# JiapengWu/TeMP

Measured on AMD Instinct MI355X. Metric: edges/sec (fwd+bwd) RGCN+GRU seq_len=15, higher is better.
Workload: dtype f32

## Files before the change

include/temp_amd.h:

```cpp
#ifndef TEMP_AMD_H
#define TEMP_AMD_H

#include <stddef.h>
#include <stdint.h>

#ifdef __cplusplus
extern "C" {
#endif

#define TEMP_ABI_VERSION 2

enum {
  TEMP_OK = 0,
  TEMP_E_BADARG = 1,
  TEMP_E_UNSUPPORTED = 2,
  TEMP_E_WORKSPACE = 3,
  TEMP_E_LAUNCH = 4
};

enum { TEMP_ACT_NONE = 0, TEMP_ACT_RELU = 1 };
enum { TEMP_GRU_TORCH = 0,
       TEMP_GRU_TYPE1 = 1 };

int temp_abi_version(void);
// ... 31 lines not shown
  int32_t n_seg;
  int32_t n_edges;
  const int32_t* a;
  const int32_t* b;
  int32_t n_chunks;
  const int32_t* chunk_seg;
  const int32_t* chunk_beg;
  const int32_t* chunk_end;
  const int32_t* chunk_slot;
  int32_t n_partial;
  int32_t n_fix;
  const int32_t* fix_seg;
  const int32_t* fix_slot;
  const int32_t* fix_cnt;
} TempEdgeView;

typedef struct TempMembers {
  int32_t n_members;
  int32_t max_nodes;
  int32_t max_edges;
  int32_t max_chunks[3];
  const int32_t* node_off;
  const int32_t* edge_off;
  const int32_t* chunk_off;
  const int32_t* fix_off;
} TempMembers;

typedef struct TempGraph {
  int32_t n_nodes;
  int32_t n_edges;
  const float* nnorm;
  const int32_t* in_deg;
  const int32_t* out_deg;
  TempEdgeView by_dst;
  TempEdgeView by_src;
  TempEdgeView by_rel;
  TempMembers members;
} TempGraph;

size_t temp_rgcn_fwd_workspace(const TempGraph* g, int d_out);
int temp_rgcn_fwd(const TempGraph* g, const float* h, const int32_t* h_ids ,
                  int d_in, int d_out, int num_bases, int n_rel_rows,
                  const float* weight, const float* loop_w, const float* bias , int act,
                  float* out, void* workspace, size_t workspace_bytes, const TempDropout* drop, void* stream);

size_t temp_rgcn_bwd_workspace(const TempGraph* g, int d_in, int d_out, int num_bases, int n_rel_rows);
int temp_rgcn_bwd(const TempGraph* g, const float* h, const float* out, const float* d_out_grad,
                  int d_in, int d_out, int num_bases, int n_rel_rows,
                  const float* weight, const float* loop_w, int has_bias, int act,
                  float* d_h, float* d_weight, float* d_loop_w, float* d_bias ,
                  void* workspace, size_t workspace_bytes, const TempDropout* drop, void* stream);

int temp_rgcn_bwd_dh(const TempGraph* g, const float* out , const float* d_out_grad, int d_in, int d_out, int num_bases,
                     int n_rel_rows, const float* weight, const float* loop_w, int act, float* d_h, float* dz_out ,
                     float* dzm_out , void* workspace, size_t workspace_bytes, const TempDropout* drop, void* stream);
int temp_rgcn_bwd_weights(const TempGraph* g, const float* h, const float* dz, const float* dzm , int d_in, int d_out, int num_bases,
                          int n_rel_rows, int has_bias, float* d_weight, float* d_loop_w, float* d_bias , void* workspace,
                          size_t workspace_bytes, void* stream);

size_t temp_rgcn_table_fwd_workspace(const TempGraph* g, int n_table, int d_out);
int temp_rgcn_table_fwd(const TempGraph* g, const float* table, const int32_t* ids, int n_table, int d_in, int d_out, int num_bases,
                        int n_rel_rows, const float* weight, const float* loop_w, const float* bias, int act, float* out, void* workspace,
                        size_t workspace_bytes, const TempDropout* drop, void* stream);
size_t temp_rgcn_table_bwd_workspace(const TempGraph* g, int n_table, int d_in, int d_out, int num_bases);
int temp_rgcn_table_bwd(const TempGraph* g, const float* table, const int32_t* ids, const int32_t* inv_ptr, const int32_t* inv_order, int n_table,
                        const float* out, const float* d_out_grad, int d_in, int d_out, int num_bases, int n_rel_rows, const float* weight,
                        const float* loop_w, int has_bias, int act, float* d_table, float* d_weight, float* d_loop_w, float* d_bias,
                        void* workspace, size_t workspace_bytes, const TempDropout* drop, void* stream);

int temp_rgcn_isolated_fwd(int n, int d, const float* e, const float* loop_w, const float* bias ,
                           int act, float* out, const TempDropout* drop, void* stream);
size_t temp_rgcn_isolated_bwd_workspace(int n, int d);
int temp_rgcn_isolated_bwd(int n, int d, const float* e, const float* out, const float* d_out_grad,
                           const float* loop_w, int has_bias, int act,
                           float* d_e, float* d_loop_w, float* d_bias ,
                           void* workspace, size_t workspace_bytes, const TempDropout* drop, void* stream);

int temp_gru_fwd(int n, int d, int variant,
                 const float* x, const float* prev, const int32_t* prev_idx , const float* dt,
                 float lambda, const float* decay_wb ,
                 const float* w_ih, const float* w_hh, const float* b_ih, const float* b_hh,
                 float* h_out, float* saved, void* stream);

size_t temp_gru_bwd_workspace(int n, int d, int variant);
int temp_gru_bwd(int n, int d, int variant,
                 const float* x, const float* prev, const int32_t* prev_idx , const float* dt,
                 float lambda, const float* decay_wb ,
                 const float* w_ih, const float* w_hh,
                 const float* saved, const float* d_h_out,
                 float* d_x, float* d_prev, float* d_w_ih, float* d_w_hh, float* d_b_ih, float* d_b_hh,
                 float* d_decay_wb ,
                 void* workspace, size_t workspace_bytes, void* stream);

int temp_decay_rows(int n, int d, const float* x, const float* dt, float lambda, float* out, void* stream);

int temp_gru_input_gates(int n, int d, int variant, const float* x, const float* w_ih, const float* b_ih, float* gi, void* stream);
int temp_gru_input_gates_multi(int count, const int* ns, int d, int variant, const float* const* xs, const float* const* w_ihs,
                               const float* const* b_ihs, float* const* gis, void* stream);
int temp_gru_input_gates_gather_multi(int count, const int* ns, int d, int variant, const float* const* xs, const int32_t* const* x_idx,
                                      const float* const* w_ihs, const float* const* b_ihs, float* const* gis, void* stream);
int temp_gru_cell_fwd(int n, int d, int variant, const float* gi, const float* prev, const int32_t* prev_idx ,
                      const float* dt, float lambda, const float* w_hh, const float* b_hh,
                      float* h_out, float* saved, size_t saved_plane, void* stream);
int temp_gru_cell_bwd(int n, int d, int variant, const float* saved, size_t saved_plane,
                      const float* dh_up , const float* d_prev_next , const int32_t* next_idx ,
                      const float* dt, float lambda, const float* w_hh,
                      float* dgi, float* dgh, float* decv, float* d_prev, void* stream);
typedef struct TempGruCellFwd {
  int32_t n; const float* gi; const float* prev ;
  const int32_t* prev_idx ; const float* dt;
  const float* w_hh; const float* b_hh; float* h_out; float* saved ;
} TempGruCellFwd;
typedef struct TempGruCellBwd {
  int32_t n; const float* saved; const float* dh_up ; const float* d_prev_next ;
  const int32_t* next_idx ; const float* dt; const float* w_hh;
  float* dgi; float* dgh; float* decv; float* d_prev;
  int32_t no_prev;
} TempGruCellBwd;
int temp_gru_cell_fwd_multi(int count, const TempGruCellFwd* cells, int d, int variant, float lambda, size_t saved_plane, void* stream);
int temp_gru_cell_bwd_multi(int count, const TempGruCellBwd* cells, int d, int variant, float lambda, size_t saved_plane, void* stream);
size_t temp_gru_weight_grads_workspace(int n, int d, int variant);
int temp_gru_weight_grads(int n, int d, int variant, const float* x, const float* hdec, const float* dgi, const float* dgh,
                          const float* w_ih, float* d_x , float* d_w_ih, float* d_w_hh, float* d_b_ih, float* d_b_hh,
                          void* workspace, size_t workspace_bytes, void* stream);
size_t temp_gru_weight_grads_multi_workspace(int count, const int* ns, int d, int variant);
int temp_gru_weight_grads_multi(int count, const int* ns, int d, int variant, const float* const* xs, const float* const* hdecs,
                                const float* const* dgis, const float* const* dghs, const float* const* w_ihs, float* const* d_xs,
                                float* d_w, float* d_b, void* workspace, size_t workspace_bytes, void* stream);

size_t temp_gru_grads_g4_workspace(int count, const int* ns, int d);
int temp_gru_grads_g4(int count, const int* ns, int d, const float* const* xs, const float* const* hdecs, const float* const* g4s,
                      const float* const* w_ihs, float* const* d_xs, float* d_w, float* d_b, void* workspace, size_t workspace_bytes,
                      void* stream);
int temp_gru_grads_g4_keys(int count, const int* ns, int d, const float* const* xs, const float* const* hdecs, const float* const* g4s,
                           const float* const* w_ihs, float* const* d_xs, float* d_w, float* d_b, const uint32_t* const* g4_row_keys,
                           const uint32_t* const* g4_col_keys, const uint32_t* const* x_col_keys ,
                           void* workspace, size_t workspace_bytes, void* stream);

#define TEMP_CHAIN_HAS_PREV (1 << 30)
#define TEMP_CHAIN_TRACKS 32
#define TEMP_CHAIN_MAX_RNN 4
#define TEMP_CHAIN_MAX_UP 8
typedef struct TempGruChain {
  int32_t d, variant, n_panels, n_steps;
  int32_t max_steps;
  const int32_t* panel; const int32_t* rows; const int32_t* sinfo;
  const float* dt;
  float lambda;
  size_t saved_plane;
  int32_t n_rnn;
  const float* packed[TEMP_CHAIN_MAX_RNN];
  const float* b_hh[TEMP_CHAIN_MAX_RNN];
  const int32_t* gi_index;
} TempGruChain;
int temp_gru_chain_supported(int d);
size_t temp_gru_chain_pack_floats(int d);
int temp_gru_chain_pack(int d, const float* w_hh, float* packed, void* stream);
int temp_gru_chain_pack_multi(int count, int d, const float* const* w_hh, float* const* packed, void* stream);
int temp_gru_chain_fwd(const TempGruChain* c, const float* gi, float* h_out, float* saved, void* stream);
int temp_gru_chain_bwd(const TempGruChain* c, const float* saved, int n_up, const float* const* up ,
                       float* dgi, float* dgh, void* stream);
int temp_gru_chain_bwd_g4(const TempGruChain* c, const float* saved, int n_up, const float* const* up ,
                          float* g4, void* stream);
int temp_gru_chain_keys_supported(int d);
int temp_gru_chain_bwd_g4_keys(const TempGruChain* c, const float* saved, int n_up, const float* const* up, float* g4,
                               uint32_t* row_keys, uint32_t* col_keys, void* stream);

int temp_gather_rows(int n, int d, const float* table, const int32_t* idx, float* out, void* stream);
size_t temp_keys_cols_size(int d);
int temp_absmax_keys(int n, int d, const float* x, int ldx, uint32_t* row_keys, uint32_t* col_keys, void* stream);
int temp_gather_rows_keys(int n, int d, const float* table, const int32_t* idx, float* out, uint32_t* row_keys, uint32_t* col_keys, void* stream);
int temp_linear_keys(int M, int N, int K, const float* A, int lda, const uint32_t* a_keys, const float* B, int ldb, int trans_b, float* C, int ldc,
                     void* stream);
int temp_gru_input_gates_gather_multi_keys(int count, const int* ns, int d, int variant, const float* const* xs, const int32_t* const* x_idx,
                                           const uint32_t* const* x_keys, const float* const* w_ihs, const float* const* b_ihs, float* const* gis,
                                           void* stream);
int temp_scatter_add_rows(int n, int d, const float* src, const int32_t* idx, float* table, void* stream);
size_t temp_segment_sum_rows_workspace(int n_seg, int n_rows, int d);
int temp_segment_sum_rows(int n_seg, int n_rows, int d, const int32_t* seg_ptr, const int32_t* order, const float* src, float* out,
                          void* workspace, size_t workspace_bytes, void* stream);
int temp_segment_sum_rows_relu(int n_seg, int n_rows, int d, const int32_t* seg_ptr, const int32_t* order, const float* src, const float* relu_of,
                               float* out, void* workspace, size_t workspace_bytes, void* stream);

int temp_linear(int M, int N, int K, const float* A, int lda, const float* B, int ldb, int trans_b, float* C, int ldc, void* stream);
int temp_linear_t(int M, int N, int K, const float* A, int lda, const float* B, int ldb, int trans_b, float* Ct, int ldct, void* stream);
typedef struct TempLinearProblem { int M; const float* A; const float* B; float* C; } TempLinearProblem;
int temp_linear_multi(int count, const TempLinearProblem* probs, int N, int K, int lda, int ldb, int trans_b, int ldc, void* stream);
size_t temp_linear_tn_workspace(int M, int Ka, int Nb);
int temp_linear_tn(int M, int Ka, int Nb, const float* A, int lda, const float* B, int ldb, float* out, int ldo,
                   void* workspace, size_t workspace_bytes, void* stream);
size_t temp_linear_tn_multi_workspace(int count, int max_m, int Ka, int Nb);
int temp_linear_tn_multi(int count, const TempLinearProblem* probs, int Ka, int Nb, int lda, int ldb, int ldc, void* workspace,
                         size_t workspace_bytes, void* stream);

int temp_gather_ce_fwd(int P, int C, int N, const float* scores, const int32_t* cand, float* loss_rows, float* lse_rows, void* stream);
int temp_gather_ce_bwd(int P, int C, int N, const float* scores, const int32_t* cand, const float* lse_rows, const float* scale,
                       float inv_rows, const float* row_scale , float* d_scores, void* stream);

#define TEMP_SCORE_DISTMULT 0
#define TEMP_SCORE_COMPLEX 1
int temp_bilinear_query_fwd(int P, int d, int kind, const float* ent_rows, const int32_t* known_idx, const float* rel, const int32_t* rel_idx,
                            const int32_t* is_tail, float* q, void* stream);
int temp_bilinear_query_bwd(int P, int d, int kind, const float* ent_rows, const int32_t* known_idx, const float* rel, const int32_t* rel_idx,
                            const int32_t* is_tail, const float* d_q, float* d_known_rows, float* d_rel_rows, void* stream);

#define TEMP_ASSEMBLE_PIECE 4096
typedef struct TempCopyDesc { const int32_t* src; const int32_t* aux; int32_t dst_off; int32_t len; int32_t add; int32_t mode; } TempCopyDesc;
int temp_assemble_views(int n_pieces, const int32_t* piece_desc, const int32_t* piece_start, const TempCopyDesc* descs, const int32_t* table,
                        int32_t* out, void* stream);

typedef struct TempSubsampleJob {
  int32_t n_nodes, n_edges, keep;
  uint64_t seed;
  const int32_t* parent; int32_t* child; const int32_t* eid;
  int32_t off_a[3], off_b[3], off_chunk_beg[3], off_chunk_end[3], off_chunk_seg[3], n_chunks[3];
  int32_t off_in_deg, off_out_deg, off_nnorm;
  uint8_t* keep_mask; void* scratch;
} TempSubsampleJob;
int temp_subsample_views(int n_jobs, const TempSubsampleJob* jobs, void* stream);

int temp_corrupt_sample(int R, int K, int N, uint64_t seed, const int32_t* truth, const int32_t* lo, const int32_t* hi, const int32_t* ids,
                        int32_t* cand, void* stream);

int temp_filtered_rank(int P, int N, int ld, const float* scores, const int32_t* target, const int32_t* filt_ptr,
                       const int32_t* filt_ids, int32_t* ranks, void* stream);

typedef struct TempAttn {
  int32_t n, D, heads, T;
  const float* q;  int32_t ldq;
  const float* kh; const float* vh; int32_t ldh;
  const float* kc; const float* vc; int32_t ldc;
  const int32_t* idx;
  const float* decay;
} TempAttn;
int temp_sa_attn_fwd(const TempAttn* p, float* out, float* score, float* lse, void* stream);
int temp_sa_attn_bwd(const TempAttn* p, const float* out, const float* score, const float* lse, const float* d_out,
                     float* d_q, int ld_dq, float* d_kh, float* d_vh, int ld_dh, float* d_kc, float* d_vc, int ld_dc,
                     float* d_decay, int n_table, const int32_t* inv_ptr, const int32_t* inv_ref, float* ds_ws, void* stream);

int temp_copy_probe(const void* src, void* dst, size_t bytes, void* stream);

int temp_trace_begin(int capacity);
int temp_trace_end(int* kernel_ids , float* ms , int capacity, int* n_out );
const char* temp_trace_kernel_name(int kernel_id);

#ifdef __cplusplus
}
#endif
#endif
```

temp_amd/_lib.py:

```python
import ctypes
import threading
import os

_HERE = os.path.dirname(os.path.abspath(__file__))
LIB_PATH = os.path.join(_HERE, "libtemp_amd.so")

c_i32p = ctypes.POINTER(ctypes.c_int32)
c_f32p = ctypes.POINTER(ctypes.c_float)
c_vp = ctypes.c_void_p

ACT_NONE, ACT_RELU = 0, 1
GRU_TORCH, GRU_TYPE1 = 0, 1
CHUNK = 64
CHUNK_REL = 128


class TempEdgeView(ctypes.Structure):
    _fields_ = [("n_seg", ctypes.c_int32), ("n_edges", ctypes.c_int32), ("a", c_vp), ("b", c_vp),
                ("n_chunks", ctypes.c_int32), ("chunk_seg", c_vp), ("chunk_beg", c_vp), ("chunk_end", c_vp),
                ("chunk_slot", c_vp), ("n_partial", ctypes.c_int32), ("n_fix", ctypes.c_int32),
                ("fix_seg", c_vp), ("fix_slot", c_vp), ("fix_cnt", c_vp)]


class TempMembers(ctypes.Structure):
    _fields_ = [("n_members", ctypes.c_int32), ("max_nodes", ctypes.c_int32), ("max_edges", ctypes.c_int32),
                ("max_chunks", ctypes.c_int32 * 3), ("node_off", c_vp), ("edge_off", c_vp), ("chunk_off", c_vp), ("fix_off", c_vp)]


class TempGraph(ctypes.Structure):
    _fields_ = [("n_nodes", ctypes.c_int32), ("n_edges", ctypes.c_int32), ("nnorm", c_vp), ("in_deg", c_vp),
                ("out_deg", c_vp), ("by_dst", TempEdgeView), ("by_src", TempEdgeView), ("by_rel", TempEdgeView),
                ("members", TempMembers)]


ABI_VERSION = 2
OPT_MFMA_BF16X3, OPT_TN_SPLIT, OPT_RGCN_SCALAR, OPT_GEMM_STREAM, OPT_GRU_STREAM, OPT_RGCN_TILE, OPT_DEBUG, OPT_OVERLAP, OPT_GEMM_RESIDENT, OPT_MFMA_F16X2 = range(10)


class TempGruCellFwd(ctypes.Structure):
    _fields_ = [("n", ctypes.c_int32), ("gi", c_vp), ("prev", c_vp), ("prev_idx", c_vp), ("dt", c_vp), ("w_hh", c_vp),
                ("b_hh", c_vp), ("h_out", c_vp), ("saved", c_vp)]


class TempGruCellBwd(ctypes.Structure):
    _fields_ = [("n", ctypes.c_int32), ("saved", c_vp), ("dh_up", c_vp), ("d_prev_next", c_vp), ("next_idx", c_vp), ("dt", c_vp),
                ("w_hh", c_vp), ("dgi", c_vp), ("dgh", c_vp), ("decv", c_vp), ("d_prev", c_vp), ("no_prev", ctypes.c_int32)]


CHAIN_HAS_PREV = 1 << 30
CHAIN_TRACKS = 32
CHAIN_MAX_RNN = 4
CHAIN_MAX_UP = 8
CHAIN_MAX_STEPS = 64


class TempGruChain(ctypes.Structure):
    _fields_ = [("d", ctypes.c_int32), ("variant", ctypes.c_int32), ("n_panels", ctypes.c_int32), ("n_steps", ctypes.c_int32),
                ("max_steps", ctypes.c_int32), ("panel", c_vp), ("rows", c_vp), ("sinfo", c_vp), ("dt", c_vp), ("lambda_", ctypes.c_float),
                ("saved_plane", ctypes.c_size_t), ("n_rnn", ctypes.c_int32), ("packed", c_vp * CHAIN_MAX_RNN), ("b_hh", c_vp * CHAIN_MAX_RNN),
                ("gi_index", c_vp)]


class TempSubsampleJob(ctypes.Structure):
    _fields_ = [("n_nodes", ctypes.c_int32), ("n_edges", ctypes.c_int32), ("keep", ctypes.c_int32), ("seed", ctypes.c_uint64),
                ("parent", c_vp), ("child", c_vp), ("eid", c_vp),
                ("off_a", ctypes.c_int32 * 3), ("off_b", ctypes.c_int32 * 3), ("off_chunk_beg", ctypes.c_int32 * 3),
                ("off_chunk_end", ctypes.c_int32 * 3), ("off_chunk_seg", ctypes.c_int32 * 3), ("n_chunks", ctypes.c_int32 * 3),
                ("off_in_deg", ctypes.c_int32), ("off_out_deg", ctypes.c_int32), ("off_nnorm", ctypes.c_int32),
                ("keep_mask", c_vp), ("scratch", c_vp)]


class TempDropout(ctypes.Structure):
    _fields_ = [("p", ctypes.c_float), ("seed", ctypes.c_uint64)]


class TempAttn(ctypes.Structure):
    _fields_ = [("n", ctypes.c_int32), ("D", ctypes.c_int32), ("heads", ctypes.c_int32), ("T", ctypes.c_int32),
                ("q", c_vp), ("ldq", ctypes.c_int32), ("kh", c_vp), ("vh", c_vp), ("ldh", ctypes.c_int32),
                ("kc", c_vp), ("vc", c_vp), ("ldc", ctypes.c_int32), ("idx", c_vp), ("decay", c_vp)]


class TempLinearProblem(ctypes.Structure):
    _fields_ = [("M", ctypes.c_int32), ("A", c_vp), ("B", c_vp), ("C", c_vp)]


ASSEMBLE_PIECE = 4096
SCORE_KINDS = {"distmult": 0, "complex": 1}

_G = ctypes.POINTER(TempGraph)
_I, _F, _SZ = ctypes.c_int, ctypes.c_float, ctypes.c_size_t
SYMBOLS = {
    "temp_abi_version": (_I, []),
    "temp_error_string": (ctypes.c_char_p, [_I]),
    "temp_set_option": (_I, [_I, _I]),
    "temp_get_option": (_I, [_I]),
    "temp_scratch_refused": (ctypes.c_longlong, []),
    "temp_f16_launches": (ctypes.c_longlong, []),
    "temp_tile_launches": (ctypes.c_longlong, []),
    "temp_set_debug_buffer": (None, [c_vp, _SZ]),
    "temp_rgcn_fwd_workspace": (_SZ, [_G, _I]),
    "temp_rgcn_fwd": (_I, [_G, c_vp, c_vp, _I, _I, _I, _I, c_vp, c_vp, c_vp, _I, c_vp, c_vp, _SZ, c_vp, c_vp]),
    "temp_rgcn_bwd_workspace": (_SZ, [_G, _I, _I, _I, _I]),
    "temp_rgcn_bwd": (_I, [_G, c_vp, c_vp, c_vp, _I, _I, _I, _I, c_vp, c_vp, _I, _I, c_vp, c_vp, c_vp, c_vp, c_vp, _SZ, c_vp, c_vp]),
    "temp_rgcn_bwd_dh": (_I, [_G, c_vp, c_vp, _I, _I, _I, _I, c_vp, c_vp, _I, c_vp, c_vp, c_vp, c_vp, _SZ, c_vp, c_vp]),
    "temp_rgcn_bwd_weights": (_I, [_G, c_vp, c_vp, c_vp, _I, _I, _I, _I, _I, c_vp, c_vp, c_vp, c_vp, _SZ, c_vp]),
    "temp_rgcn_table_fwd_workspace": (_SZ, [_G, _I, _I]),
    "temp_rgcn_table_fwd": (_I, [_G, c_vp, c_vp, _I, _I, _I, _I, _I, c_vp, c_vp, c_vp, _I, c_vp, c_vp, _SZ, c_vp, c_vp]),
    "temp_rgcn_table_bwd_workspace": (_SZ, [_G, _I, _I, _I, _I]),
    "temp_rgcn_table_bwd": (_I, [_G, c_vp, c_vp, c_vp, c_vp, _I, c_vp, c_vp, _I, _I, _I, _I, c_vp, c_vp, _I, _I, c_vp, c_vp, c_vp, c_vp,
                                 c_vp, _SZ, c_vp, c_vp]),
    "temp_rgcn_isolated_fwd": (_I, [_I, _I, c_vp, c_vp, c_vp, _I, c_vp, c_vp, c_vp]),
    "temp_rgcn_isolated_bwd_workspace": (_SZ, [_I, _I]),
    "temp_rgcn_isolated_bwd": (_I, [_I, _I, c_vp, c_vp, c_vp, c_vp, _I, _I, c_vp, c_vp, c_vp, c_vp, _SZ, c_vp, c_vp]),
    "temp_gru_fwd": (_I, [_I, _I, _I, c_vp, c_vp, c_vp, c_vp, _F, c_vp, c_vp, c_vp, c_vp, c_vp, c_vp, c_vp, c_vp]),
    "temp_gru_bwd_workspace": (_SZ, [_I, _I, _I]),
    "temp_gru_bwd": (_I, [_I, _I, _I, c_vp, c_vp, c_vp, c_vp, _F, c_vp, c_vp, c_vp, c_vp, c_vp,
                          c_vp, c_vp, c_vp, c_vp, c_vp, c_vp, c_vp, c_vp, _SZ, c_vp]),
    "temp_decay_rows": (_I, [_I, _I, c_vp, c_vp, _F, c_vp, c_vp]),
    "temp_gru_input_gates": (_I, [_I, _I, _I, c_vp, c_vp, c_vp, c_vp, c_vp]),
    "temp_gru_input_gates_multi": (_I, [_I, c_vp, _I, _I, c_vp, c_vp, c_vp, c_vp, c_vp]),
    "temp_gru_input_gates_gather_multi": (_I, [_I, c_vp, _I, _I, c_vp, c_vp, c_vp, c_vp, c_vp, c_vp]),
    "temp_gru_cell_fwd": (_I, [_I, _I, _I, c_vp, c_vp, c_vp, c_vp, _F, c_vp, c_vp, c_vp, c_vp, _SZ, c_vp]),
    "temp_gru_cell_bwd": (_I, [_I, _I, _I, c_vp, _SZ, c_vp, c_vp, c_vp, c_vp, _F, c_vp, c_vp, c_vp, c_vp, c_vp, c_vp]),
    "temp_gru_cell_fwd_multi": (_I, [_I, ctypes.POINTER(TempGruCellFwd), _I, _I, _F, _SZ, c_vp]),
    "temp_gru_cell_bwd_multi": (_I, [_I, ctypes.POINTER(TempGruCellBwd), _I, _I, _F, _SZ, c_vp]),
    "temp_gru_weight_grads_workspace": (_SZ, [_I, _I, _I]),
    "temp_gru_weight_grads": (_I, [_I, _I, _I, c_vp, c_vp, c_vp, c_vp, c_vp, c_vp, c_vp, c_vp, c_vp, c_vp, c_vp, _SZ, c_vp]),
    "temp_gru_weight_grads_multi_workspace": (ctypes.c_size_t, [_I, c_vp, _I, _I]),
    "temp_gru_weight_grads_multi": (_I, [_I, c_vp, _I, _I, c_vp, c_vp, c_vp, c_vp, c_vp, c_vp, c_vp, c_vp, c_vp, ctypes.c_size_t, c_vp]),
    "temp_gru_chain_supported": (_I, [_I]),
    "temp_gru_chain_pack_floats": (_SZ, [_I]),
    "temp_gru_chain_pack": (_I, [_I, c_vp, c_vp, c_vp]),
    "temp_gru_chain_pack_multi": (_I, [_I, _I, ctypes.POINTER(c_vp), ctypes.POINTER(c_vp), c_vp]),
    "temp_gru_chain_fwd": (_I, [ctypes.POINTER(TempGruChain), c_vp, c_vp, c_vp, c_vp]),
    "temp_gru_chain_bwd": (_I, [ctypes.POINTER(TempGruChain), c_vp, _I, ctypes.POINTER(c_vp), c_vp, c_vp, c_vp]),
    "temp_gru_chain_bwd_g4": (_I, [ctypes.POINTER(TempGruChain), c_vp, _I, ctypes.POINTER(c_vp), c_vp, c_vp]),
    "temp_gru_chain_keys_supported": (_I, [_I]),
    "temp_gru_chain_bwd_g4_keys": (_I, [ctypes.POINTER(TempGruChain), c_vp, _I, ctypes.POINTER(c_vp), c_vp, c_vp, c_vp, c_vp]),
    "temp_gru_grads_g4_keys": (_I, [_I, c_vp, _I, c_vp, c_vp, c_vp, c_vp, c_vp, c_vp, c_vp, c_vp, c_vp, c_vp, c_vp, ctypes.c_size_t, c_vp]),
    "temp_gru_grads_g4_workspace": (ctypes.c_size_t, [_I, c_vp, _I]),
    "temp_gru_grads_g4": (_I, [_I, c_vp, _I, c_vp, c_vp, c_vp, c_vp, c_vp, c_vp, c_vp, c_vp, ctypes.c_size_t, c_vp]),
    "temp_gather_rows": (_I, [_I, _I, c_vp, c_vp, c_vp, c_vp]),
    "temp_keys_cols_size": (_SZ, [_I]),
    "temp_absmax_keys": (_I, [_I, _I, c_vp, _I, c_vp, c_vp, c_vp]),
    "temp_gather_rows_keys": (_I, [_I, _I, c_vp, c_vp, c_vp, c_vp, c_vp, c_vp]),
    "temp_linear_keys": (_I, [_I, _I, _I, c_vp, _I, c_vp, c_vp, _I, _I, c_vp, _I, c_vp]),
    "temp_gru_input_gates_gather_multi_keys": (_I, [_I, c_vp, _I, _I, c_vp, c_vp, c_vp, c_vp, c_vp, c_vp, c_vp]),
    "temp_scatter_add_rows": (_I, [_I, _I, c_vp, c_vp, c_vp, c_vp]),
    "temp_segment_sum_rows_workspace": (_SZ, [_I, _I, _I]),
    "temp_segment_sum_rows": (_I, [_I, _I, _I, c_vp, c_vp, c_vp, c_vp, c_vp, _SZ, c_vp]),
    "temp_segment_sum_rows_relu": (_I, [_I, _I, _I, c_vp, c_vp, c_vp, c_vp, c_vp, c_vp, _SZ, c_vp]),
    "temp_linear": (_I, [_I, _I, _I, c_vp, _I, c_vp, _I, _I, c_vp, _I, c_vp]),
    "temp_linear_t": (_I, [_I, _I, _I, c_vp, _I, c_vp, _I, _I, c_vp, _I, c_vp]),
    "temp_linear_multi": (_I, [_I, ctypes.POINTER(TempLinearProblem), _I, _I, _I, _I, _I, _I, c_vp]),
    "temp_linear_tn_workspace": (_SZ, [_I, _I, _I]),
    "temp_linear_tn_multi_workspace": (_SZ, [_I, _I, _I, _I]),
    "temp_linear_tn_multi": (_I, [_I, ctypes.POINTER(TempLinearProblem), _I, _I, _I, _I, _I, c_vp, _SZ, c_vp]),
    "temp_linear_tn": (_I, [_I, _I, _I, c_vp, _I, c_vp, _I, c_vp, _I, c_vp, _SZ, c_vp]),
    "temp_gather_ce_fwd": (_I, [_I, _I, _I, c_vp, c_vp, c_vp, c_vp, c_vp]),
    "temp_gather_ce_bwd": (_I, [_I, _I, _I, c_vp, c_vp, c_vp, c_vp, _F, c_vp, c_vp, c_vp]),
    "temp_bilinear_query_fwd": (_I, [_I, _I, _I, c_vp, c_vp, c_vp, c_vp, c_vp, c_vp, c_vp]),
    "temp_bilinear_query_bwd": (_I, [_I, _I, _I, c_vp, c_vp, c_vp, c_vp, c_vp, c_vp, c_vp, c_vp, c_vp]),
    "temp_assemble_views": (_I, [_I, c_vp, c_vp, c_vp, c_vp, c_vp, c_vp]),
    "temp_subsample_views": (_I, [_I, ctypes.POINTER(TempSubsampleJob), c_vp]),
    "temp_corrupt_sample": (_I, [_I, _I, _I, ctypes.c_uint64, c_vp, c_vp, c_vp, c_vp, c_vp, c_vp]),
    "temp_filtered_rank": (_I, [_I, _I, _I, c_vp, c_vp, c_vp, c_vp, c_vp, c_vp]),
    "temp_sa_attn_fwd": (_I, [ctypes.POINTER(TempAttn), c_vp, c_vp, c_vp, c_vp]),
    "temp_sa_attn_bwd": (_I, [ctypes.POINTER(TempAttn), c_vp, c_vp, c_vp, c_vp, c_vp, _I, c_vp, c_vp, _I, c_vp, c_vp, _I, c_vp, _I, c_vp, c_vp, c_vp, c_vp]),
    "temp_copy_probe": (_I, [c_vp, c_vp, _SZ, c_vp]),
    "temp_trace_begin": (_I, [_I]),
    "temp_trace_end": (_I, [c_i32p, c_f32p, _I, c_i32p]),
    "temp_trace_kernel_name": (ctypes.c_char_p, [_I]),
}

_lib = None


class TempAmdError(RuntimeError):
    pass


def load():
    global _lib
    if _lib is not None:
        return _lib
    if not os.path.exists(LIB_PATH):
        raise TempAmdError("libtemp_amd.so not found at %s -- run `python -m temp_amd.build` "
                           "(hipcc --offload-arch=gfx950); there is no CPU fallback" % LIB_PATH)
    lib = ctypes.CDLL(LIB_PATH) if os.environ.get("TEMP_PYDLL", "1") == "0" else ctypes.PyDLL(LIB_PATH)
    for name, (res, args) in SYMBOLS.items():
        fn = getattr(lib, name)
        fn.restype = res
        fn.argtypes = args
    if lib.temp_abi_version() != ABI_VERSION:
        raise TempAmdError("libtemp_amd.so ABI version %d != %d (stale .so or stale Python package)" % (lib.temp_abi_version(), ABI_VERSION))
    _lib = lib
    return lib


def check(rc, what):
    if rc != 0:
        msg = load().temp_error_string(rc).decode()
        raise TempAmdError("%s failed: %s (code %d)" % (what, msg, rc))


class _CreateLock:

    def __init__(self):
        self._l = threading.RLock()

    def __enter__(self):
        if not self._l.acquire(blocking=False):
            held = getattr(_coop, "held", False)
            if held:
                _py_token.release()
            self._l.acquire()
            if held:
                _py_token.acquire()
        return self

    def __exit__(self, *exc):
        self._l.release()
        return False


create_lock = _CreateLock()


def publish(device):
    import torch as _torch
    device = _torch.device(device)
    if device.type == "cuda":
        _torch.cuda.current_stream(device).synchronize()


_coop = threading.local()
_py_token = threading.Lock()


def coop_begin(gate):
    _coop.gate = gate
    _py_token.acquire()
    _coop.held = True


def coop_end():
    if getattr(_coop, "held", False):
        _coop.held = False
        _py_token.release()
    _coop.gate = None


def pause_point():
    g = getattr(_coop, "gate", None)
    if g is not None and not g.is_set():
        held = getattr(_coop, "held", False)
        if held:
            _py_token.release()
        g.wait()
        if held:
            _py_token.acquire()


def outside_token(fn):
    def call(*args):
        if getattr(_coop, "held", False):
            _py_token.release()
            try:
                return fn(*args)
            finally:
                _py_token.acquire()
        return fn(*args)
    return call


_STAGE_BYTES = 32 << 20
_stage = threading.local()


def to_device(host, device):
    import numpy as _np
    import torch as _torch
    t = _torch.from_numpy(_np.ascontiguousarray(host)) if isinstance(host, _np.ndarray) else host
    device = _torch.device(device)
    nbytes = t.numel() * t.element_size()
    if device.type != "cuda" or nbytes == 0 or t.is_cuda or nbytes > _STAGE_BYTES // 4 or not t.is_contiguous():
        return t.to(device)
# ... 31 lines not shown
```

temp_amd/backend.py:

```python
import ctypes

import torch

from . import _lib

_backend = None


def set_backend(b):
    global _backend
    _backend = b


def get_backend():
    global _backend
    if _backend is None:
        _backend = HipBackend()
    return _backend


def _ptr(t):
    return ctypes.c_void_p(t.data_ptr()) if t is not None else None


# ... 137 lines not shown
        e, out, g, loop_w = _f32(e, "e"), _f32(out, "out"), _f32(d_out_grad, "d_out"), _f32(loop_w, "loop_weight")
        n, d = e.shape
        d_e = torch.empty_like(e)
        d_loop = torch.empty_like(loop_w)
        d_bias = torch.empty(d, dtype=torch.float32, device=e.device) if has_bias else None
        ws = self._ws(self.lib.temp_rgcn_isolated_bwd_workspace(n, d), e.device)
        rc = self.lib.temp_rgcn_isolated_bwd(n, d, _ptr(e), _ptr(out), _ptr(g), _ptr(loop_w), int(has_bias), act, _ptr(d_e),
                                             _ptr(d_loop), _ptr(d_bias), _ptr(ws), ws.numel(), _drop(drop), _stream())
        _lib.check(rc, "temp_rgcn_isolated_bwd")
        return d_e, d_loop, d_bias

    def gru_fwd(self, x, prev, prev_idx, dt, lam, decay_wb, w_ih, w_hh, b_ih, b_hh, variant):
        x, prev, dt = _f32(x, "x"), _f32(prev, "prev"), _f32(dt, "dt")
        w_ih, w_hh, b_ih, b_hh = _f32(w_ih, "w_ih"), _f32(w_hh, "w_hh"), _f32(b_ih, "b_ih"), _f32(b_hh, "b_hh")
        decay_wb, prev_idx = _f32(decay_wb, "decay_wb"), _i32(prev_idx, "prev_idx")
        n, d = x.shape
        h_out = torch.empty_like(x)
        saved = torch.empty(5, n, d, dtype=torch.float32, device=x.device)
        rc = self.lib.temp_gru_fwd(n, d, variant, _ptr(x), _ptr(prev), _ptr(prev_idx), _ptr(dt), float(lam), _ptr(decay_wb),
                                   _ptr(w_ih), _ptr(w_hh), _ptr(b_ih), _ptr(b_hh), _ptr(h_out), _ptr(saved), _stream())
        _lib.check(rc, "temp_gru_fwd")
        return h_out, saved

    def gru_bwd(self, x, prev, prev_idx, dt, lam, decay_wb, w_ih, w_hh, saved, d_h, variant):
        x, prev, dt, d_h = _f32(x, "x"), _f32(prev, "prev"), _f32(dt, "dt"), _f32(d_h, "d_h")
        w_ih, w_hh, saved = _f32(w_ih, "w_ih"), _f32(w_hh, "w_hh"), _f32(saved, "saved")
        decay_wb, prev_idx = _f32(decay_wb, "decay_wb"), _i32(prev_idx, "prev_idx")
        n, d = x.shape
        dev = x.device
        d_x = torch.empty_like(x)
        d_prev = torch.empty_like(x)
        d_w_ih, d_w_hh = torch.empty_like(w_ih), torch.empty_like(w_hh)
        d_b_ih = torch.empty(w_ih.shape[0], dtype=torch.float32, device=dev)
        d_b_hh = torch.empty(w_hh.shape[0], dtype=torch.float32, device=dev)
        d_wb = torch.empty(2, dtype=torch.float32, device=dev) if decay_wb is not None else None
        ws = self._ws(self.lib.temp_gru_bwd_workspace(n, d, variant), dev)
        rc = self.lib.temp_gru_bwd(n, d, variant, _ptr(x), _ptr(prev), _ptr(prev_idx), _ptr(dt), float(lam), _ptr(decay_wb),
                                   _ptr(w_ih), _ptr(w_hh), _ptr(saved), _ptr(d_h), _ptr(d_x), _ptr(d_prev), _ptr(d_w_ih),
                                   _ptr(d_w_hh), _ptr(d_b_ih), _ptr(d_b_hh), _ptr(d_wb), _ptr(ws), ws.numel(), _stream())
        _lib.check(rc, "temp_gru_bwd")
        return d_x, d_prev, d_w_ih, d_w_hh, d_b_ih, d_b_hh, d_wb

    def gru_input_gates(self, x, w_ih, b_ih, variant, out):
        x, w_ih, b_ih = _f32(x, "x"), _f32(w_ih, "w_ih"), _f32(b_ih, "b_ih")
        assert out.is_contiguous() and out.shape == (x.shape[0], w_ih.shape[0])
        rc = self.lib.temp_gru_input_gates(x.shape[0], x.shape[1], variant, _ptr(x), _ptr(w_ih), _ptr(b_ih), _ptr(out), _stream())
        _lib.check(rc, "temp_gru_input_gates")

    def gru_input_gates_multi(self, xs, w_ihs, b_ihs, variant, outs, x_idx=None, x_keys=None):
        k = len(xs)
        xs = [_f32(x, "x") for x in xs]
        w_ihs, b_ihs = [_f32(w, "w_ih") for w in w_ihs], [_f32(b, "b_ih") for b in b_ihs]
        d = xs[0].shape[1]
        idx = [None] * k if x_idx is None else [None if t is None else _i32(t, "x_idx") for t in x_idx]
        rows = [x.shape[0] if t is None else t.shape[0] for x, t in zip(xs, idx)]
        for x, w, o, n in zip(xs, w_ihs, outs, rows):
            assert x.shape[1] == d and o.is_contiguous() and o.shape == (n, w.shape[0]) and w.shape == w_ihs[0].shape
        arr = lambda ts: (ctypes.c_void_p * k)(*[t.data_ptr() for t in ts])
        ns = (ctypes.c_int * k)(*rows)
        if x_idx is None and x_keys is None:
            rc = self.lib.temp_gru_input_gates_multi(k, ns, d, variant, arr(xs), arr(w_ihs), arr(b_ihs), arr(outs), _stream())
            _lib.check(rc, "temp_gru_input_gates_multi")
            return
        ia = (ctypes.c_void_p * k)(*[None if t is None else t.data_ptr() for t in idx])
        if x_keys is not None:
            for x, t in zip(xs, x_keys):
                assert t.dtype == torch.int32 and t.is_contiguous() and t.numel() == x.shape[0]
            ka = (ctypes.c_void_p * k)(*[t.data_ptr() for t in x_keys])
            rc = self.lib.temp_gru_input_gates_gather_multi_keys(k, ns, d, variant, arr(xs), ia if x_idx is not None else None, ka, arr(w_ihs),
                                                                 arr(b_ihs), arr(outs), _stream())
            _lib.check(rc, "temp_gru_input_gates_gather_multi_keys")
            return
        rc = self.lib.temp_gru_input_gates_gather_multi(k, ns, d, variant, arr(xs), ia, arr(w_ihs), arr(b_ihs), arr(outs), _stream())
        _lib.check(rc, "temp_gru_input_gates_gather_multi")

    def gru_cell_fwd(self, gi, prev, prev_idx, dt, lam, w_hh, b_hh, variant, h_out, saved_all, row0):
        n, d = h_out.shape
        plane = saved_all.shape[1] * d
        sp = ctypes.c_void_p(saved_all.data_ptr() + 4 * row0 * d)
        rc = self.lib.temp_gru_cell_fwd(n, d, variant, _ptr(gi), _ptr(_f32(prev, "prev")), _ptr(_i32(prev_idx, "prev_idx")),
                                        _ptr(_f32(dt, "dt")), float(lam), _ptr(_f32(w_hh, "w_hh")), _ptr(_f32(b_hh, "b_hh")),
                                        _ptr(h_out), sp, plane, _stream())
        _lib.check(rc, "temp_gru_cell_fwd")

    def gru_cell_bwd(self, saved_all, row0, n, dh_up, d_prev_next, next_idx, dt, lam, w_hh, variant, dgi, dgh, decv, d_prev):
        d = saved_all.shape[2]
        plane = saved_all.shape[1] * d
        sp = ctypes.c_void_p(saved_all.data_ptr() + 4 * row0 * d)
        rc = self.lib.temp_gru_cell_bwd(n, d, variant, sp, plane, _ptr(dh_up), _ptr(d_prev_next), _ptr(_i32(next_idx, "next_idx")),
                                        _ptr(_f32(dt, "dt")), float(lam), _ptr(_f32(w_hh, "w_hh")), _ptr(dgi), _ptr(dgh), _ptr(decv),
                                        _ptr(d_prev), _stream())
        _lib.check(rc, "temp_gru_cell_bwd")

    def gru_cell_fwd_multi(self, cells, lam, variant, saved_all):
        d = saved_all.shape[2]
        arr = (_lib.TempGruCellFwd * len(cells))()
        keep = []
        for a, c in zip(arr, cells):
            prev, pidx, dt = _f32(c["prev"], "prev"), _i32(c["prev_idx"], "prev_idx"), _f32(c["dt"], "dt")
            w_hh, b_hh = _f32(c["w_hh"], "w_hh"), _f32(c["b_hh"], "b_hh")
            keep += [prev, pidx, dt, w_hh, b_hh]
            a.n = c["h_out"].shape[0]
            a.gi, a.prev = c["gi"].data_ptr(), (prev.data_ptr() if prev is not None else None)
            a.prev_idx, a.dt = (pidx.data_ptr() if pidx is not None else None), dt.data_ptr()
            a.w_hh, a.b_hh, a.h_out = w_hh.data_ptr(), b_hh.data_ptr(), c["h_out"].data_ptr()
            a.saved = saved_all.data_ptr() + 4 * c["row0"] * d
        rc = self.lib.temp_gru_cell_fwd_multi(len(cells), arr, d, variant, float(lam), saved_all.shape[1] * d, _stream())
        _lib.check(rc, "temp_gru_cell_fwd_multi")

    def gru_cell_bwd_multi(self, cells, lam, variant, saved_all):
        d = saved_all.shape[2]
        arr = (_lib.TempGruCellBwd * len(cells))()
        keep = []
        opt = lambda t: t.data_ptr() if t is not None else None
        for a, c in zip(arr, cells):
            dt, w_hh, nidx = _f32(c["dt"], "dt"), _f32(c["w_hh"], "w_hh"), _i32(c["next_idx"], "next_idx")
            keep += [dt, w_hh, nidx]
            a.n = c["n"]
            a.saved = saved_all.data_ptr() + 4 * c["row0"] * d
            a.dh_up, a.d_prev_next, a.next_idx = opt(c["dh_up"]), opt(c["d_prev_next"]), opt(nidx)
            a.dt, a.w_hh = dt.data_ptr(), w_hh.data_ptr()
            a.dgi, a.dgh, a.decv, a.d_prev = c["dgi"].data_ptr(), c["dgh"].data_ptr(), c["decv"].data_ptr(), c["d_prev"].data_ptr()
            a.no_prev = 1 if c.get("no_prev") else 0
        rc = self.lib.temp_gru_cell_bwd_multi(len(cells), arr, d, variant, float(lam), saved_all.shape[1] * d, _stream())
        _lib.check(rc, "temp_gru_cell_bwd_multi")

    def subsample_views(self, jobs):
        arr = (_lib.TempSubsampleJob * len(jobs))()
        for a, j in zip(arr, jobs):
            a.n_nodes, a.n_edges, a.keep, a.seed = j["n_nodes"], j["n_edges"], j["keep"], int(j["seed"]) & 0xFFFFFFFFFFFFFFFF
            a.parent, a.child = _i32(j["parent"], "parent").data_ptr(), _i32(j["child"], "child").data_ptr()
            a.eid = _i32(j["eid"], "eid").data_ptr() if j["n_edges"] else None
            for fld in ("off_a", "off_b", "off_chunk_beg", "off_chunk_end", "off_chunk_seg", "n_chunks"):
                for v in range(3):
                    getattr(a, fld)[v] = int(j[fld][v])
            a.off_in_deg, a.off_out_deg, a.off_nnorm = int(j["off_in_deg"]), int(j["off_out_deg"]), int(j["off_nnorm"])
            a.keep_mask = j["keep_mask"].data_ptr() if j.get("keep_mask") is not None else None
            a.scratch = j["scratch"].data_ptr()
        _lib.check(self.lib.temp_subsample_views(len(jobs), arr, _stream()), "temp_subsample_views")

    def decay_rows(self, x, dt, lam):
        x, dt = _f32(x, "x"), _f32(dt, "dt")
        out = torch.empty_like(x)
        _lib.check(self.lib.temp_decay_rows(x.shape[0], x.shape[1], _ptr(x), _ptr(dt), float(lam), _ptr(out), _stream()), "temp_decay_rows")
        return out

    def gru_chain_supported(self, d):
        return bool(self.lib.temp_gru_chain_supported(int(d)))

    def gru_chain_pack(self, w_hh):
        w_hh = _f32(w_hh, "w_hh")
        d = w_hh.shape[1]
        out = torch.empty(self.lib.temp_gru_chain_pack_floats(d), dtype=torch.float32, device=w_hh.device)
        _lib.check(self.lib.temp_gru_chain_pack(d, _ptr(w_hh), _ptr(out), _stream()), "temp_gru_chain_pack")
        return out

    def gru_chain_pack_multi(self, w_hhs):
        w_hhs = [_f32(w, "w_hh") for w in w_hhs]
        d = w_hhs[0].shape[1]
        n = self.lib.temp_gru_chain_pack_floats(d)
        buf = torch.empty(len(w_hhs), n, dtype=torch.float32, device=w_hhs[0].device)
        src = (ctypes.c_void_p * len(w_hhs))(*[w.data_ptr() for w in w_hhs])
        dst = (ctypes.c_void_p * len(w_hhs))(*[buf[i].data_ptr() for i in range(len(w_hhs))])
        _lib.check(self.lib.temp_gru_chain_pack_multi(len(w_hhs), d, src, dst, _stream()), "temp_gru_chain_pack_multi")
        return [buf[i] for i in range(len(w_hhs))]

    def _chain_desc(self, tabs, d, variant, lam, plane, packs, b_hhs):
        c = _lib.TempGruChain()
        c.d, c.variant, c.n_panels, c.n_steps, c.max_steps = d, variant, tabs["n_panels"], tabs["n_steps"], tabs["max_steps"]
        c.panel, c.rows, c.sinfo, c.dt = (_i32(tabs[k], k).data_ptr() for k in ("panel", "rows", "sinfo", "dt_bits"))
        c.lambda_, c.saved_plane, c.n_rnn = float(lam), plane, len(packs)
        keep = []
        for i, (pk, b) in enumerate(zip(packs, b_hhs)):
            pk, b = _f32(pk, "packed"), _f32(b, "b_hh")
            keep += [pk, b]
            c.packed[i], c.b_hh[i] = pk.data_ptr(), b.data_ptr()
        return c, keep

    def gru_chain_fwd(self, tabs, gi, lam, variant, packs, b_hhs, h_out, saved_all, gi_index=None):
        d = saved_all.shape[2]
        c, keep = self._chain_desc(tabs, d, variant, lam, saved_all.shape[1] * d, packs, b_hhs)
        if gi_index is not None:
            assert gi_index.shape[0] == saved_all.shape[1]
            c.gi_index = _i32(gi_index, "gi_index").data_ptr()
        rc = self.lib.temp_gru_chain_fwd(ctypes.byref(c), _ptr(_f32(gi, "gi")), _ptr(h_out), _ptr(saved_all), _stream())
        _lib.check(rc, "temp_gru_chain_fwd")

    def gru_chain_bwd(self, tabs, saved_all, ups, lam, variant, packs, b_hhs, dgi, dgh):
        d = saved_all.shape[2]
        c, keep = self._chain_desc(tabs, d, variant, lam, saved_all.shape[1] * d, packs, b_hhs)
        ups = [_f32(u, "upstream") if u is not None else None for u in ups]
        arr = (ctypes.c_void_p * max(len(ups), 1))(*[u.data_ptr() if u is not None else None for u in ups])
        rc = self.lib.temp_gru_chain_bwd(ctypes.byref(c), _ptr(saved_all), len(ups), arr, _ptr(dgi), _ptr(dgh), _stream())
        _lib.check(rc, "temp_gru_chain_bwd")

    def gru_chain_keys_supported(self, d):
        return bool(self.lib.temp_gru_chain_keys_supported(int(d)))

    def gru_chain_bwd_g4(self, tabs, saved_all, ups, lam, variant, packs, b_hhs, g4, keys=None):
        d = saved_all.shape[2]
        c, keep = self._chain_desc(tabs, d, variant, lam, saved_all.shape[1] * d, packs, b_hhs)
        ups = [_f32(u, "upstream") if u is not None else None for u in ups]
        arr = (ctypes.c_void_p * max(len(ups), 1))(*[u.data_ptr() if u is not None else None for u in ups])
        if keys is not None:
            row_keys, col_keys = keys
            assert row_keys.dtype == torch.int32 and col_keys.dtype == torch.int32 and col_keys.is_contiguous()
            assert row_keys.numel() == saved_all.shape[1] and col_keys.numel() == (len(packs) + tabs["n_panels"]) * 4 * d
            rc = self.lib.temp_gru_chain_bwd_g4_keys(ctypes.byref(c), _ptr(saved_all), len(ups), arr, _ptr(g4), _ptr(row_keys), _ptr(col_keys),
                                                     _stream())
            _lib.check(rc, "temp_gru_chain_bwd_g4_keys")
            return
        rc = self.lib.temp_gru_chain_bwd_g4(ctypes.byref(c), _ptr(saved_all), len(ups), arr, _ptr(g4), _stream())
        _lib.check(rc, "temp_gru_chain_bwd_g4")

    def gru_grads_g4_supported(self, ns, d, variant):
        k = len(ns)
        if k < 1 or k > 4 or variant != _lib.GRU_TORCH:
            return False
        return self.lib.temp_gru_grads_g4_workspace(k, (ctypes.c_int * k)(*[int(n) for n in ns]), int(d)) > 0

    def gru_grads_g4(self, xs, hdecs, g4s, w_ihs, d_xs, row_keys=None, col_keys=None, x_col_keys=None):
        k = len(xs)
        d = xs[0].shape[1]
        dev = xs[0].device
        ns = (ctypes.c_int * k)(*[x.shape[0] for x in xs])
        nb = self.lib.temp_gru_grads_g4_workspace(k, ns, d)
        if nb == 0:
            raise ValueError("temp_gru_grads_g4: unsupported shape (check gru_grads_g4_supported first)")
        keep = [[_f32(t, "operand") for t in ts] for ts in (xs, hdecs, w_ihs)]
        for g in g4s:
            assert g.dtype == torch.float32 and g.is_contiguous() and g.shape[1] == 4 * d
        arr = lambda ts: (ctypes.c_void_p * k)(*[t.data_ptr() for t in ts])
        dx = (ctypes.c_void_p * k)(*[None if t is None else t.data_ptr() for t in d_xs])
        d_w = torch.empty(2 * k, 3 * d, d, dtype=torch.float32, device=dev)
        d_b = torch.empty(2 * k, 3 * d, dtype=torch.float32, device=dev)
        ws = self._ws(nb, dev)
        if row_keys is not None and col_keys is not None:
            for rk, ck, x in zip(row_keys, col_keys, xs):
                assert rk.dtype == torch.int32 and ck.dtype == torch.int32 and rk.is_contiguous() and ck.is_contiguous()
                assert rk.numel() == x.shape[0] and ck.numel() == 4 * d
            xk = None
            if x_col_keys is not None:
                for t in x_col_keys:
                    assert t.dtype == torch.int32 and t.is_contiguous() and t.numel() == d
                xk = arr(x_col_keys)
            rc = self.lib.temp_gru_grads_g4_keys(k, ns, d, arr(keep[0]), arr(keep[1]), arr(g4s), arr(keep[2]), dx, _ptr(d_w), _ptr(d_b),
                                                 arr(row_keys), arr(col_keys), xk, _ptr(ws), ws.numel(), _stream())
            _lib.check(rc, "temp_gru_grads_g4_keys")
            return [(d_w[2 * i], d_w[2 * i + 1], d_b[2 * i], d_b[2 * i + 1]) for i in range(k)]
        rc = self.lib.temp_gru_grads_g4(k, ns, d, arr(keep[0]), arr(keep[1]), arr(g4s), arr(keep[2]), dx, _ptr(d_w), _ptr(d_b), _ptr(ws),
                                        ws.numel(), _stream())
        _lib.check(rc, "temp_gru_grads_g4")
        return [(d_w[2 * i], d_w[2 * i + 1], d_b[2 * i], d_b[2 * i + 1]) for i in range(k)]

    def gru_weight_grads(self, x, hdec, dgi, dgh, w_ih, variant, d_x):
        n, d = x.shape
        w_ih = _f32(w_ih, "w_ih")
        dev = x.device
        d_w_ih = torch.empty_like(w_ih)
        d_w_hh = torch.empty(3 * d, d, dtype=torch.float32, device=dev)
        d_b_ih = torch.empty(w_ih.shape[0], dtype=torch.float32, device=dev)
        d_b_hh = torch.empty(3 * d, dtype=torch.float32, device=dev)
        ws = self._ws(self.lib.temp_gru_weight_grads_workspace(n, d, variant), dev)
        rc = self.lib.temp_gru_weight_grads(n, d, variant, _ptr(x), _ptr(hdec), _ptr(dgi), _ptr(dgh), _ptr(w_ih), _ptr(d_x),
                                            _ptr(d_w_ih), _ptr(d_w_hh), _ptr(d_b_ih), _ptr(d_b_hh), _ptr(ws), ws.numel(), _stream())
        _lib.check(rc, "temp_gru_weight_grads")
        return d_w_ih, d_w_hh, d_b_ih, d_b_hh

    def gru_weight_grads_multi(self, xs, hdecs, dgis, dghs, w_ihs, variant, d_xs):
        k = len(xs)
        if k < 1 or k > 4 or variant != _lib.GRU_TORCH or any(h is None for h in hdecs):
            return None
        d = xs[0].shape[1]
        dev = xs[0].device
        ns = (ctypes.c_int * k)(*[x.shape[0] for x in xs])
        nb = self.lib.temp_gru_weight_grads_multi_workspace(k, ns, d, variant)
        if nb == 0:
            return None
        keep = [[_f32(t, "operand") for t in ts] for ts in (xs, hdecs, dgis, dghs, w_ihs)]
        arr = lambda ts: (ctypes.c_void_p * k)(*[t.data_ptr() for t in ts])
        dx = (ctypes.c_void_p * k)(*[None if t is None else t.data_ptr() for t in d_xs])
        d_w = torch.empty(2 * k, 3 * d, d, dtype=torch.float32, device=dev)
        d_b = torch.empty(2 * k, 3 * d, dtype=torch.float32, device=dev)
        ws = self._ws(nb, dev)
        rc = self.lib.temp_gru_weight_grads_multi(k, ns, d, variant, arr(keep[0]), arr(keep[1]), arr(keep[2]), arr(keep[3]), arr(keep[4]), dx,
                                                  _ptr(d_w), _ptr(d_b), _ptr(ws), ws.numel(), _stream())
        if rc == 2:
            return None
        _lib.check(rc, "temp_gru_weight_grads_multi")
        return [(d_w[2 * i], d_w[2 * i + 1], d_b[2 * i], d_b[2 * i + 1]) for i in range(k)]

    def linear(self, a, b, trans_b, out=None, a_keys=None):
        a, b = _f32(a, "a"), _f32(b, "b")
        M, K = a.shape
        N = b.shape[0] if trans_b else b.shape[1]
        c = out if out is not None else torch.empty(M, N, dtype=torch.float32, device=a.device)
        assert c.shape == (M, N) and c.is_contiguous() and c.dtype == torch.float32
        if a_keys is not None:
            assert a_keys.dtype == torch.int32 and a_keys.is_contiguous() and a_keys.numel() == M
            rc = self.lib.temp_linear_keys(M, N, K, _ptr(a), K, _ptr(a_keys), _ptr(b), b.shape[1], int(trans_b), _ptr(c), N, _stream())
            _lib.check(rc, "temp_linear_keys")
            return c
        rc = self.lib.temp_linear(M, N, K, _ptr(a), K, _ptr(b), b.shape[1], int(trans_b), _ptr(c), N, _stream())
        _lib.check(rc, "temp_linear")
        return c

    def absmax_keys(self, x, rows=True, cols=True):
        x = _f32(x, "x")
        n, d = x.shape
        rk = torch.empty(n, dtype=torch.int32, device=x.device) if rows else None
        ck = torch.empty(self.lib.temp_keys_cols_size(d), dtype=torch.int32, device=x.device) if cols else None
        _lib.check(self.lib.temp_absmax_keys(n, d, _ptr(x), d, _ptr(rk), _ptr(ck), _stream()), "temp_absmax_keys")
        return rk, (ck[:d] if cols else None)

    def linear_t(self, a, b, trans_b, out_t):
        a, b = _f32(a, "a"), _f32(b, "b")
        M, K = a.shape
        N = b.shape[0] if trans_b else b.shape[1]
        if out_t.shape != (N, M) or not out_t.is_contiguous() or out_t.dtype != torch.float32:
            raise ValueError("linear_t: out_t must be a contiguous float32 (N, M) matrix")
        rc = self.lib.temp_linear_t(M, N, K, _ptr(a), K, _ptr(b), b.shape[1], int(trans_b), _ptr(out_t), M, _stream())
        _lib.check(rc, "temp_linear_t")
        return out_t

    def linear_multi(self, a_list, b_list, trans_b, out):
        K = a_list[0].shape[1]
        N = out.shape[1]
        arr = (_lib.TempLinearProblem * len(a_list))()
        row, keep = 0, []
        for i, (a, b) in enumerate(zip(a_list, b_list)):
            a, b = _f32(a, "a"), _f32(b, "b")
            keep.append((a, b))
            if a.shape[1] != K or b.shape != ((N, K) if trans_b else (K, N)):
                raise ValueError("linear_multi: problems must share N, K and the layout of b")
            arr[i].M, arr[i].A, arr[i].B = a.shape[0], a.data_ptr(), b.data_ptr()
            arr[i].C = out.data_ptr() + row * N * 4
            row += a.shape[0]
        if row != out.shape[0] or not out.is_contiguous():
            raise ValueError("linear_multi: out must be a contiguous (sum M_i, N) matrix")
# ... 202 lines not shown
```

temp_amd/csrc/gru_chain.hip:

```cpp
#include "common.hpp"
#include "gru_math.hpp"
#include "gemm_bx.hpp"

namespace temp {

#define CH_SLOTS TEMP_CHAIN_TRACKS
#define CH_HAS_PREV TEMP_CHAIN_HAS_PREV
#define CH_ROW_MASK (TEMP_CHAIN_HAS_PREV - 1)
#define CH_LDS_LIMIT (160 * 1024)

struct ChainRnn { const float4* wf; const float4* wb; const float* b_hh; const unsigned* kf; const unsigned* kb; };
struct ChainArgs {
  int D, n_panels, max_steps, dbg;
  int n_rnn_keys;
  const int32_t* panel; const int32_t* rows; const int32_t* sinfo;
  const float* dt;
  const int32_t* gi_index;
  float lambda;
  size_t plane;
  ChainRnn rnn[TEMP_CHAIN_MAX_RNN];
};
struct ChainUps { const float* p[TEMP_CHAIN_MAX_UP]; };

struct ChainGeom {
  int NT, NQ;
  int NTb, NQb;
  int lda, ldh;
  int ldA, ldz;
};
__host__ __device__ inline ChainGeom chain_geom(int D) {
  ChainGeom g;
  g.NT = (3 * D + 31) >> 5; g.NQ = ((D + 15) >> 4) << 1;
  g.NTb = (D + 31) >> 5; g.NQb = ((3 * D + 31) >> 5) << 2;
  g.lda = g.NT * 32 + 4; g.ldh = g.NQ * 8 + 4;
  g.ldA = g.NQb * 8 + 4; g.ldz = g.NTb * 32 + 4;
  return g;
}
#define CH_MAX_STEPS 64
inline size_t chain_lds_fwd(int D, int ms) { ChainGeom g = chain_geom(D); return ((size_t)CH_SLOTS * g.lda + 2 * CH_SLOTS * g.ldh + (2 * CH_SLOTS + 1) * (size_t)ms) * 4; }
inline size_t chain_lds_bwd(int D, int ms) { ChainGeom g = chain_geom(D); return ((size_t)CH_SLOTS * g.ldA + 2 * CH_SLOTS * g.ldz + (2 * CH_SLOTS + 3) * (size_t)ms) * 4; }

}
#include "gru_chain_hx.hpp"
namespace temp {

__global__ void __launch_bounds__(256) k_gru_chain_pack(int D, const float* __restrict__ W, float4* __restrict__ out) {
  const ChainGeom g = chain_geom(D);
  const int nf = g.NT * g.NQ * 64, nb = g.NTb * g.NQb * 64;
  for (int i = blockIdx.x * blockDim.x + threadIdx.x; i < nf + nb; i += gridDim.x * blockDim.x) {
    const bool fwd = i < nf;
    const int j = fwd ? i : i - nf;
    const int lane = j & 63, rest = j >> 6;
    const int nq = fwd ? g.NQ : g.NQb;
    const int tile = rest / nq, q = rest - tile * nq;
    const int n = tile * 32 + (lane & 31), k = 8 * q + 4 * (lane >> 5);
    float v[4];
#pragma unroll
    for (int e = 0; e < 4; ++e) {
      if (fwd) v[e] = (n < 3 * D && k + e < D) ? W[(size_t)n * D + k + e] : 0.f;
      else v[e] = (n < D && k + e < 3 * D) ? W[(size_t)(k + e) * D + n] : 0.f;
    }
    out[i] = make_float4(v[0], v[1], v[2], v[3]);
  }
}

template <int VARIANT, int TPW, int MW, int BX>
__global__ void __launch_bounds__(256 + 64 * MW) k_gru_chain_fwd(ChainArgs a, const float* __restrict__ gi, float* __restrict__ H,
                                                                  float* __restrict__ saved) {
  extern __shared__ __attribute__((aligned(16))) float lds[];
  constexpr int PASSES = CH_SLOTS / MW;
  const int D = a.D, D4 = D >> 2;
  const int G = (VARIANT == TEMP_GRU_TORCH) ? 3 * D : D;
  const ChainGeom g = chain_geom(D);
  const int NT = g.NT, NQ = g.NQ, lda = g.lda, ldh = g.ldh;
  float* accb = lds;
  float* hb = accb + CH_SLOTS * lda;
  int* tabb = (int*)(hb + 2 * CH_SLOTS * ldh);
  float* decb = (float*)(tabb + CH_SLOTS * a.max_steps);
  int* flagb = (int*)(decb + CH_SLOTS * a.max_steps);
  const int tid = threadIdx.x, wave = tid >> 6, lane = tid & 63;
  const size_t plane = a.plane;

  for (int p = blockIdx.x; p < a.n_panels; p += gridDim.x) {
    const int rnn_id = a.panel[4 * p], s0 = a.panel[4 * p + 1], ns = a.panel[4 * p + 2];
    const ChainRnn R = a.rnn[rnn_id];
    for (int i = tid; i < 2 * CH_SLOTS * ldh; i += blockDim.x) hb[i] = 0.f;
    for (int i = tid; i < ns * CH_SLOTS; i += blockDim.x) {
      const int e = a.rows[(size_t)s0 * CH_SLOTS + i];
      tabb[i] = e;
      decb[i] = e >= 0 ? expf(-a.dt[e & CH_ROW_MASK] * a.lambda) : 0.f;
    }
    if (tid < ns) flagb[tid] = a.sinfo[4 * (size_t)(s0 + tid)];
    __syncthreads();

    if (wave < 4) {
      const int li = lane & 31, hh = lane >> 5;
      bool tval[TPW];
      int tidx[TPW];
#pragma unroll
      for (int j = 0; j < TPW; ++j) { tidx[j] = wave + 4 * j; tval[j] = tidx[j] < NT; if (!tval[j]) tidx[j] = NT - 1; }
      f32x16 acc[TPW];
#pragma unroll
      for (int j = 0; j < TPW; ++j)
#pragma unroll
        for (int r = 0; r < 16; ++r) acc[j][r] = 0.f;
      if constexpr (BX) {
        const bx_u32x4* wp = reinterpret_cast<const bx_u32x4*>(R.wf);
        const int NS = NQ >> 1;
        bx_u32x4 wh[TPW] = {}, wm[TPW] = {}, wl[TPW] = {};
        const bool dup_loads = (a.dbg & 128) != 0;
        auto wload = [&](bx_u32x4 (&w)[TPW], int sl, int pl) {
#pragma unroll
          for (int j = 0; j < TPW; ++j)
            if (tval[j] || dup_loads) w[j] = wp[((size_t)(sl * NT + tidx[j]) * 3 + pl) * 64 + lane];
        };
        const int rot = (a.dbg & 64) ? 0 : (int)(blockIdx.x >> 3) % NS;
        wload(wh, rot, 0); wload(wm, rot, 1); wload(wl, rot, 2);
        for (int s = 0; s < ns; ++s) {
          const int cur = s & 1;
          const int flags = flagb[s];
          if (flags & 1) {
            const int e = tabb[s * CH_SLOTS + li];
            const float decm = (e >= 0 && (e & CH_HAS_PREV)) ? decb[s * CH_SLOTS + li] : 0.f;
            const float* hrow = hb + (size_t)cur * CH_SLOTS * ldh + li * ldh + 8 * hh;
            bx_u32x4 AH, AM, AL, NH, NM, NL;
            {
              const float4 r0 = scale4(ld4(hrow + 16 * rot), decm), r1 = scale4(ld4(hrow + 16 * rot + 4), decm);
              unsigned h_, m_, l_;
              bx_split_pair(r0.x, r0.y, h_, m_, l_); AH[0] = h_; AM[0] = m_; AL[0] = l_;
              bx_split_pair(r0.z, r0.w, h_, m_, l_); AH[1] = h_; AM[1] = m_; AL[1] = l_;
              bx_split_pair(r1.x, r1.y, h_, m_, l_); AH[2] = h_; AM[2] = m_; AL[2] = l_;
              bx_split_pair(r1.z, r1.w, h_, m_, l_); AH[3] = h_; AM[3] = m_; AL[3] = l_;
            }
            for (int j = 0, sl = rot; j < NS; ++j) {
              const int sn = sl + 1 < NS ? sl + 1 : 0;
              const float4 n0 = scale4(ld4(hrow + 16 * sn), decm), n1 = scale4(ld4(hrow + 16 * sn + 4), decm);
              const bx_bf16x8 ah = bx_frag(AH), am = bx_frag(AM), al = bx_frag(AL);
              unsigned h_, m_, l_;
              __builtin_amdgcn_sched_barrier(0);
#pragma unroll
              for (int j = 0; j < TPW; ++j) acc[j] = __builtin_amdgcn_mfma_f32_32x32x16_bf16(bx_frag(wl[j]), ah, acc[j], 0, 0, 0);
              __builtin_amdgcn_sched_barrier(0);
              wload(wl, sn, 2);
              bx_split_pair(n0.x, n0.y, h_, m_, l_); NH[0] = h_; NM[0] = m_; NL[0] = l_;
              __builtin_amdgcn_sched_barrier(0);
#pragma unroll
              for (int j = 0; j < TPW; ++j) acc[j] = __builtin_amdgcn_mfma_f32_32x32x16_bf16(bx_frag(wm[j]), am, acc[j], 0, 0, 0);
              __builtin_amdgcn_sched_barrier(0);
              bx_split_pair(n0.z, n0.w, h_, m_, l_); NH[1] = h_; NM[1] = m_; NL[1] = l_;
              __builtin_amdgcn_sched_barrier(0);
#pragma unroll
              for (int j = 0; j < TPW; ++j) acc[j] = __builtin_amdgcn_mfma_f32_32x32x16_bf16(bx_frag(wm[j]), ah, acc[j], 0, 0, 0);
              __builtin_amdgcn_sched_barrier(0);
              wload(wm, sn, 1);
              bx_split_pair(n1.x, n1.y, h_, m_, l_); NH[2] = h_; NM[2] = m_; NL[2] = l_;
              __builtin_amdgcn_sched_barrier(0);
#pragma unroll
              for (int j = 0; j < TPW; ++j) acc[j] = __builtin_amdgcn_mfma_f32_32x32x16_bf16(bx_frag(wh[j]), al, acc[j], 0, 0, 0);
              __builtin_amdgcn_sched_barrier(0);
              bx_split_pair(n1.z, n1.w, h_, m_, l_); NH[3] = h_; NM[3] = m_; NL[3] = l_;
              __builtin_amdgcn_sched_barrier(0);
#pragma unroll
              for (int j = 0; j < TPW; ++j) acc[j] = __builtin_amdgcn_mfma_f32_32x32x16_bf16(bx_frag(wh[j]), am, acc[j], 0, 0, 0);
#pragma unroll
              for (int j = 0; j < TPW; ++j) acc[j] = __builtin_amdgcn_mfma_f32_32x32x16_bf16(bx_frag(wh[j]), ah, acc[j], 0, 0, 0);
              __builtin_amdgcn_sched_barrier(0);
// ... 256 lines not shown
            }
          const float dec = decb[s * CH_SLOTS + li];
#pragma unroll
          for (int j = 0; j < TPWB; ++j) {
            if (!tval[j]) continue;
#pragma unroll
            for (int qq = 0; qq < 4; ++qq) {
              const int c = tidx[j] * 32 + 8 * qq + 4 * hh;
              const float4 gz = ld4(gzb + (size_t)li * ldz + c);
              st4(dpb + (size_t)li * ldz + c, make_float4((acc[j][4 * qq] + gz.x) * dec, (acc[j][4 * qq + 1] + gz.y) * dec,
                                                           (acc[j][4 * qq + 2] + gz.z) * dec, (acc[j][4 * qq + 3] + gz.w) * dec));
              acc[j][4 * qq] = 0.f; acc[j][4 * qq + 1] = 0.f; acc[j][4 * qq + 2] = 0.f; acc[j][4 * qq + 3] = 0.f;
            }
          }
          }
          __syncthreads();
        }
      } else {
      float4 w0[TPWB], w1[TPWB], w2[TPWB], w3[TPWB];
      auto wload = [&](float4 (&w)[TPWB], int q) {
#pragma unroll
        for (int j = 0; j < TPWB; ++j) w[j] = R.wb[((size_t)tidx[j] * NQb + q) * 64 + lane];
      };
      wload(w0, 0); wload(w1, 1); wload(w2, 2);
      for (int s = ns - 1; s >= 0; --s) {
        const int cur = s & 1;
        const int flags = flagb[s];
        __syncthreads();
        if (flags & 1) {
          const float* arow = ab + (size_t)li * ldA + 4 * hh;
          auto stage = [&](const float4 (&w)[TPWB], const float4 d4) {
#pragma unroll
            for (int j = 0; j < TPWB; ++j) acc[j] = __builtin_amdgcn_mfma_f32_32x32x2f32(w[j].x, d4.x, acc[j], 0, 0, 0);
#pragma unroll
            for (int j = 0; j < TPWB; ++j) acc[j] = __builtin_amdgcn_mfma_f32_32x32x2f32(w[j].y, d4.y, acc[j], 0, 0, 0);
#pragma unroll
            for (int j = 0; j < TPWB; ++j) acc[j] = __builtin_amdgcn_mfma_f32_32x32x2f32(w[j].z, d4.z, acc[j], 0, 0, 0);
#pragma unroll
            for (int j = 0; j < TPWB; ++j) acc[j] = __builtin_amdgcn_mfma_f32_32x32x2f32(w[j].w, d4.w, acc[j], 0, 0, 0);
          };
          float4 dA = ld4(arow), dB;
          for (int q = 0; q < NQb; q += 4) {
            const int qa = q + 4 < NQb ? q + 4 : 0, qb = q + 5 < NQb ? q + 5 : 1, qc = q + 6 < NQb ? q + 6 : 2;
            wload(w3, q + 3);
            dB = ld4(arow + 8 * (q + 1));
            __builtin_amdgcn_sched_barrier(0);
            stage(w0, dA);
            __builtin_amdgcn_sched_barrier(0);
            wload(w0, qa);
            dA = ld4(arow + 8 * (q + 2));
            __builtin_amdgcn_sched_barrier(0);
            stage(w1, dB);
            __builtin_amdgcn_sched_barrier(0);
            wload(w1, qb);
            dB = ld4(arow + 8 * (q + 3));
            __builtin_amdgcn_sched_barrier(0);
            stage(w2, dA);
            __builtin_amdgcn_sched_barrier(0);
            wload(w2, qc);
            dA = ld4(arow + 8 * (q + 4 < NQb ? q + 4 : 0));
            __builtin_amdgcn_sched_barrier(0);
            stage(w3, dB);
            __builtin_amdgcn_sched_barrier(0);
          }
          const float dec = decb[s * CH_SLOTS + li];
#pragma unroll
          for (int j = 0; j < TPWB; ++j) {
            if (!tval[j]) continue;
#pragma unroll
            for (int qq = 0; qq < 4; ++qq) {
              const int c = tidx[j] * 32 + 8 * qq + 4 * hh;
              const float4 gz = ld4(gzb + (size_t)li * ldz + c);
              st4(dpb + (size_t)li * ldz + c, make_float4((acc[j][4 * qq] + gz.x) * dec, (acc[j][4 * qq + 1] + gz.y) * dec,
                                                           (acc[j][4 * qq + 2] + gz.z) * dec, (acc[j][4 * qq + 3] + gz.w) * dec));
              acc[j][4 * qq] = 0.f; acc[j][4 * qq + 1] = 0.f; acc[j][4 * qq + 2] = 0.f; acc[j][4 * qq + 3] = 0.f;
            }
          }
        }
        __syncthreads();
      }
      }
    } else {
      const int mw = wave - 4, c4 = lane, col = 4 * c4;
      const bool cact = c4 < D4;
      int erow[PASSES];
      bool nxt[PASSES];
      float4 sr[PASSES], sz[PASSES], sn[PASSES], shn[PASSES], shd[PASSES];
      auto prefetch = [&](int s) {
#pragma unroll
        for (int ps = 0; ps < PASSES; ++ps) {
          const int slot = ps * MW + mw;
          const int e = tabb[s * CH_SLOTS + slot];
          erow[ps] = e;
          int en = -1;
          if (s + 1 < ns) en = tabb[(s + 1) * CH_SLOTS + slot];
          nxt[ps] = en >= 0 && (en & CH_HAS_PREV);
          const bool ok = e >= 0 && cact;
          const size_t row = ok ? (size_t)(e & CH_ROW_MASK) : 0;
          const float* src = saved + row * D + (ok ? col : 0);
          sr[ps] = ld4(src); sz[ps] = ld4(src + plane); sn[ps] = ld4(src + 2 * plane); shn[ps] = ld4(src + 3 * plane);
          shd[ps] = ld4(src + 4 * plane);
        }
      };
      prefetch(ns - 1);
      for (int s = ns - 1; s >= 0; --s) {
        const int cur = s & 1;
        const int up_sel = upb[2 * s], up_row0 = upb[2 * s + 1];
        const float* upp = up_sel >= 0 ? ups.p[up_sel] : nullptr;
#pragma unroll
        for (int ps = 0; ps < PASSES; ++ps) {
          const int slot = ps * MW + mw;
          const int e = erow[ps];
          if (!cact) continue;
          if (e < 0) continue;
          const size_t row = (size_t)(e & CH_ROW_MASK);
          float4 gd = upp ? ld4(upp + (row - (size_t)up_row0) * D + col) : zero4();
          if (nxt[ps]) gd = add4(gd, ld4(dpb + (size_t)slot * ldz + col));
          const float4 rg = sr[ps], zg = sz[ps], ng = sn[ps], hn = shn[ps], hd = shd[ps];
          float4 dr_pre, dz_pre, dn_pre, dhn, gz;
#define TEMP_GATE(c)                                          \
          {                                                   \
            const float dn = gd.c * (1.f - zg.c);             \
            const float dz = gd.c * (hd.c - ng.c);            \
            dn_pre.c = dn * (1.f - ng.c * ng.c);              \
            dr_pre.c = dn_pre.c * hn.c * rg.c * (1.f - rg.c); \
            dz_pre.c = dz * zg.c * (1.f - zg.c);              \
            dhn.c = dn_pre.c * rg.c;                          \
            gz.c = gd.c * zg.c;                               \
          }
          TEMP_GATE(x) TEMP_GATE(y) TEMP_GATE(z) TEMP_GATE(w)
#undef TEMP_GATE
          float* arow = ab + (size_t)slot * ldA + col;
          st4(arow, dr_pre); st4(arow + D, dz_pre); st4(arow + 2 * D, dhn);
          st4(gzb + (size_t)slot * ldz + col, gz);
          if constexpr (G4) {
            const size_t b4 = row * 4 * D + col;
            st4(dgi + b4, dr_pre); st4(dgi + b4 + D, dz_pre); st4(dgi + b4 + 2 * D, dn_pre); st4(dgi + b4 + 3 * D, dhn);
          } else {
          const size_t b3 = row * 3 * D + col;
          if (VARIANT == TEMP_GRU_TORCH) { st4(dgi + b3, dr_pre); st4(dgi + b3 + D, dz_pre); st4(dgi + b3 + 2 * D, dn_pre); }
          else st4(dgi + row * D + col, dn_pre);
          st4(dgh + b3, dr_pre); st4(dgh + b3 + D, dz_pre); st4(dgh + b3 + 2 * D, dhn);
          }
        }
        __syncthreads();
        if (s > 0) prefetch(s - 1);
        __syncthreads();
      }
    }
    __syncthreads();
  }
}

static int chain_check(const TempGruChain* c) {
  if (!c || c->d <= 0 || c->n_panels < 0 || c->n_steps < 0 || c->n_rnn <= 0 || c->n_rnn > TEMP_CHAIN_MAX_RNN) return TEMP_E_BADARG;
  if (c->variant != TEMP_GRU_TORCH && c->variant != TEMP_GRU_TYPE1) return TEMP_E_BADARG;
  if (c->n_panels > 0 && (!c->panel || !c->rows || !c->sinfo || !c->dt)) return TEMP_E_BADARG;
  for (int i = 0; i < c->n_rnn; ++i) if (!c->packed[i] || !c->b_hh[i]) return TEMP_E_BADARG;
  if (c->max_steps <= 0 || c->max_steps > CH_MAX_STEPS) return TEMP_E_BADARG;
  if (!temp_gru_chain_supported(c->d)) return TEMP_E_UNSUPPORTED;
  return TEMP_OK;
}

static bool chain_bx(int d) { return bx_enabled() && d % 8 == 0; }
static bool chain_hx(int d) {
  if (!chain_bx(d) || !hx_enabled()) return false;
  const ChainGeomHx g = chain_geom_hx(d);
  return chain_lds_fwd_hx(d, CH_MAX_STEPS) <= CH_LDS_LIMIT && chain_lds_bwd_hx(d, CH_MAX_STEPS) <= CH_LDS_LIMIT && g.NT <= 20 && g.NTb <= 8;
}

static ChainArgs chain_args(const TempGruChain* c) {
  ChainArgs a = {};
  const ChainGeom g = chain_geom(c->d);
  a.D = c->d; a.n_panels = c->n_panels; a.max_steps = c->max_steps; a.panel = c->panel; a.rows = c->rows; a.sinfo = c->sinfo; a.dt = c->dt;
  a.n_rnn_keys = c->n_rnn; a.lambda = c->lambda; a.plane = c->saved_plane; a.gi_index = c->gi_index; a.dbg = option(TEMP_OPT_DEBUG) >> 8;
  for (int i = 0; i < c->n_rnn; ++i) {
    a.rnn[i].wf = (const float4*)c->packed[i];
    a.rnn[i].wb = (const float4*)c->packed[i] + (chain_bx(c->d) ? (size_t)(g.NQ >> 1) * g.NT * 192 : (size_t)g.NT * g.NQ * 64);
    a.rnn[i].b_hh = c->b_hh[i];
    a.rnn[i].kf = a.rnn[i].kb = nullptr;
    if (chain_hx(c->d)) {
      const ChainGeomHx gx = chain_geom_hx(c->d);
      a.rnn[i].wb = (const float4*)c->packed[i] + chain_hx_fwd_items(c->d);
      a.rnn[i].kf = (const unsigned*)((const float4*)c->packed[i] + chain_hx_fwd_items(c->d) + chain_hx_bwd_items(c->d));
      a.rnn[i].kb = a.rnn[i].kf + gx.NT * 32;
    }
  }
  return a;
}

template <class K>
static int chain_lds_attr(K kernel, size_t bytes, bool* done) {
  if (*done) return TEMP_OK;
  if (hipFuncSetAttribute((const void*)kernel, hipFuncAttributeMaxDynamicSharedMemorySize, CH_LDS_LIMIT) != hipSuccess) return TEMP_E_LAUNCH;
  (void)bytes;
  *done = true;
  return TEMP_OK;
}

template <int VARIANT, int TPW>
static int launch_chain_fwd(const ChainArgs& a, const float* gi, float* h, float* saved, hipStream_t st) {
  static bool attr = false;
  static bool attr_bx = false;
  static bool attr_hx = false;
  if (chain_hx(a.D)) {
    const size_t lds_hx = chain_lds_fwd_hx(a.D, a.max_steps);
    constexpr int TPW8 = (TPW * 4 + 7) / 8 < 1 ? 1 : (TPW * 4 + 7) / 8;
    const int cfg = (a.dbg >> 4) & 3;
    if (cfg == 1) {
      auto kernel = k_gru_chain_fwd_hx<VARIANT, TPW, 4, 4>;
      int rc = chain_lds_attr(kernel, lds_hx, &attr_hx);
      if (rc) return rc;
      TEMP_LAUNCH(K_GRU_CHAIN_FWD, kernel, dim3(a.n_panels), dim3(512), lds_hx, st, a, gi, h, saved);
    } else if (cfg == 2) {
      static bool attr_48 = false;
      auto kernel = k_gru_chain_fwd_hx<VARIANT, TPW, 8, 4>;
      int rc = chain_lds_attr(kernel, lds_hx, &attr_48);
      if (rc) return rc;
      TEMP_LAUNCH(K_GRU_CHAIN_FWD, kernel, dim3(a.n_panels), dim3(768), lds_hx, st, a, gi, h, saved);
    } else if (cfg == 3) {
      static bool attr_882 = false;
      auto kernel = k_gru_chain_fwd_hx<VARIANT, TPW8, 8, 8, 1>;
      int rc = chain_lds_attr(kernel, lds_hx, &attr_882);
      if (rc) return rc;
      TEMP_LAUNCH(K_GRU_CHAIN_FWD, kernel, dim3(a.n_panels), dim3(1024), lds_hx, st, a, gi, h, saved);
    } else {
      static bool attr_88 = false;
      auto kernel = k_gru_chain_fwd_hx<VARIANT, TPW8, 8, 8>;
      int rc = chain_lds_attr(kernel, lds_hx, &attr_88);
      if (rc) return rc;
      TEMP_LAUNCH(K_GRU_CHAIN_FWD, kernel, dim3(a.n_panels), dim3(1024), lds_hx, st, a, gi, h, saved);
    }
    hx_count();
    return launch_status();
  }
  const size_t lds = chain_lds_fwd(a.D, a.max_steps);
  if (chain_bx(a.D)) {
    auto kernel = k_gru_chain_fwd<VARIANT, TPW, 4, 1>;
    int rc = chain_lds_attr(kernel, lds, &attr_bx);
    if (rc) return rc;
    TEMP_LAUNCH(K_GRU_CHAIN_FWD, kernel, dim3(a.n_panels), dim3(512), lds, st, a, gi, h, saved);
    return launch_status();
  }
  auto kernel = k_gru_chain_fwd<VARIANT, TPW, 4, 0>;
  int rc = chain_lds_attr(kernel, lds, &attr);
  if (rc) return rc;
  TEMP_LAUNCH(K_GRU_CHAIN_FWD, kernel, dim3(a.n_panels), dim3(512), lds, st, a, gi, h, saved);
  return launch_status();
}

template <int VARIANT, int TPWB, int G4 = 0>
static int launch_chain_bwd(const ChainArgs& a, const ChainUps& ups, const float* saved, float* dgi, float* dgh, hipStream_t st,
                            unsigned* row_keys = nullptr, unsigned* col_keys = nullptr) {
  static bool attr = false;
  static bool attr_bx = false;
  static bool attr_hx = false;
  if (chain_hx(a.D)) {
    const size_t lds_hx = chain_lds_bwd_hx(a.D, a.max_steps);
    constexpr int TPWB8 = (TPWB * 4 + 7) / 8 < 1 ? 1 : (TPWB * 4 + 7) / 8;
    const int cfg = (a.dbg >> 4) & 3;
    if (cfg == 3) {
      static bool attr_5 = false;
      auto kernel = k_gru_chain_bwd_hx<VARIANT, TPWB, 8, G4, 4, 5>;
      int rc = chain_lds_attr(kernel, lds_hx, &attr_5);
      if (rc) return rc;
      TEMP_LAUNCH(K_GRU_CHAIN_BWD, kernel, dim3(a.n_panels), dim3(768), lds_hx, st, a, ups, saved, dgi, dgh, row_keys, col_keys);
    } else if (cfg != 2) {
      auto kernel = k_gru_chain_bwd_hx<VARIANT, TPWB, 8, G4, 4, 4>;
      int rc = chain_lds_attr(kernel, lds_hx, &attr_hx);
      if (rc) return rc;
      TEMP_LAUNCH(K_GRU_CHAIN_BWD, kernel, dim3(a.n_panels), dim3(768), lds_hx, st, a, ups, saved, dgi, dgh, row_keys, col_keys);
    } else {
      static bool attr_88 = false;
      auto kernel = k_gru_chain_bwd_hx<VARIANT, TPWB8, 8, G4, 8, 8>;
      int rc = chain_lds_attr(kernel, lds_hx, &attr_88);
      if (rc) return rc;
      TEMP_LAUNCH(K_GRU_CHAIN_BWD, kernel, dim3(a.n_panels), dim3(1024), lds_hx, st, a, ups, saved, dgi, dgh, row_keys, col_keys);
    }
    hx_count();
    if (col_keys) TEMP_LAUNCH(K_GRU_CHAIN_PACK, k_keys_reduce, dim3(ceil_div(4 * a.D, 32), a.n_rnn_keys), dim3(1024), 0, st, a.n_panels, 4 * a.D, col_keys + (size_t)a.n_rnn_keys * 4 * a.D, col_keys, a.panel, 4);
    return launch_status();
  }
  if (row_keys || col_keys) return TEMP_E_UNSUPPORTED;
  const size_t lds = chain_lds_bwd(a.D, a.max_steps);
  if (chain_bx(a.D)) {
    auto kernel = k_gru_chain_bwd<VARIANT, TPWB, 8, 1, G4>;
    int rc = chain_lds_attr(kernel, lds, &attr_bx);
    if (rc) return rc;
    TEMP_LAUNCH(K_GRU_CHAIN_BWD, kernel, dim3(a.n_panels), dim3(768), lds, st, a, ups, saved, dgi, dgh);
    return launch_status();
  }
  auto kernel = k_gru_chain_bwd<VARIANT, TPWB, 8, 0, G4>;
  int rc = chain_lds_attr(kernel, lds, &attr);
  if (rc) return rc;
  TEMP_LAUNCH(K_GRU_CHAIN_BWD, kernel, dim3(a.n_panels), dim3(768), lds, st, a, ups, saved, dgi, dgh);
  return launch_status();
}

}

using namespace temp;

extern "C" {

int temp_gru_chain_supported(int d) {
  if (d <= 0 || d % 4) return 0;
  return chain_lds_fwd(d, CH_MAX_STEPS) <= CH_LDS_LIMIT && chain_lds_bwd(d, CH_MAX_STEPS) <= CH_LDS_LIMIT && chain_geom(d).NT <= 24 && chain_geom(d).NTb <= 8;
}

size_t temp_gru_chain_pack_floats(int d) {
  if (d <= 0) return 0;
  const ChainGeom g = chain_geom(d);
  const size_t f32 = ((size_t)g.NT * g.NQ + (size_t)g.NTb * g.NQb) * 64 * 4;
  const size_t bx = ((size_t)(g.NQ >> 1) * g.NT + (size_t)(g.NQb >> 1) * g.NTb) * 192 * 4;
  const size_t hx = chain_hx_pack_floats(d);
  const size_t m = f32 > bx ? f32 : bx;
  return m > hx ? m : hx;
}

int temp_gru_chain_pack(int d, const float* w_hh, float* packed, void* stream) {
  if (d <= 0 || !w_hh || !packed) return TEMP_E_BADARG;
  if (d % 4) return TEMP_E_UNSUPPORTED;
  const ChainGeom g = chain_geom(d);
  if (chain_hx(d)) return temp_gru_chain_pack_multi(1, d, &w_hh, &packed, stream);
  if (chain_bx(d)) {
    const int nsf = g.NQ >> 1, nsb = g.NQb >> 1;
    bx_u32x4* pf = reinterpret_cast<bx_u32x4*>(packed);
    bx_u32x4* pb = pf + (size_t)nsf * g.NT * 192;
    TEMP_LAUNCH(K_GRU_CHAIN_PACK, (k_bx_pack<1>), dim3(ceil_div((long long)nsf * g.NT, 4)), dim3(256), 0, (hipStream_t)stream, d, 3 * d, g.NT, nsf,
                w_hh, d, pf);
    TEMP_LAUNCH(K_GRU_CHAIN_PACK, (k_bx_pack<0>), dim3(ceil_div((long long)nsb * g.NTb, 4)), dim3(256), 0, (hipStream_t)stream, 3 * d, d, g.NTb, nsb,
                w_hh, d, pb);
    return launch_status();
  }
  const size_t n4 = ((size_t)g.NT * g.NQ + (size_t)g.NTb * g.NQb) * 64;
  int gx = ceil_div((long long)n4, 256);
  if (gx > 1024) gx = 1024;
  TEMP_LAUNCH(K_GRU_CHAIN_PACK, k_gru_chain_pack, dim3(gx), dim3(256), 0, (hipStream_t)stream, d, w_hh, (float4*)packed);
  return launch_status();
}

int temp_gru_chain_pack_multi(int count, int d, const float* const* w_hh, float* const* packed, void* stream) {
  if (count <= 0 || count > TEMP_CHAIN_MAX_RNN || d <= 0 || !w_hh || !packed) return TEMP_E_BADARG;
  for (int i = 0; i < count; ++i) if (!w_hh[i] || !packed[i]) return TEMP_E_BADARG;
  if (d % 4) return TEMP_E_UNSUPPORTED;
  if (chain_hx(d)) {
    const ChainGeomHx gx = chain_geom_hx(d);
    HxPackJobs jobs = {};
    for (int i = 0; i < count; ++i) {
      hx_u32x4* pf = reinterpret_cast<hx_u32x4*>(packed[i]);
      hx_u32x4* pb = pf + chain_hx_fwd_items(d);
      unsigned* kf = reinterpret_cast<unsigned*>(pb + chain_hx_bwd_items(d));
      if (jobs.count + 2 > HX_PACK_JOBS) { hx_pack_launch(jobs, K_GRU_CHAIN_PACK, (hipStream_t)stream); jobs = HxPackJobs{}; }
      hx_pack_jobs_add(jobs, w_hh[i], pf, kf, d, 3 * d, d, 1);
      hx_pack_jobs_add(jobs, w_hh[i], pb, kf + gx.NT * 32, 3 * d, d, d, 0, gx.NSb);
    }
    hx_pack_launch(jobs, K_GRU_CHAIN_PACK, (hipStream_t)stream);
    return launch_status();
  }
  if (!chain_bx(d) || 2 * count > BX_PACK_JOBS) {
    for (int i = 0; i < count; ++i) { const int rc = temp_gru_chain_pack(d, w_hh[i], packed[i], stream); if (rc) return rc; }
    return TEMP_OK;
  }
  const ChainGeom g = chain_geom(d);
  BxPackJobs jobs = {};
  for (int i = 0; i < count; ++i) {
    bx_u32x4* pf = reinterpret_cast<bx_u32x4*>(packed[i]);
    bx_pack_jobs_add(jobs, w_hh[i], pf, d, 3 * d, d, 1);
    bx_pack_jobs_add(jobs, w_hh[i], pf + (size_t)(g.NQ >> 1) * g.NT * 192, 3 * d, d, d, 0);
  }
  TEMP_LAUNCH(K_GRU_CHAIN_PACK, k_bx_pack_multi, dim3(ceil_div(jobs.total_units, 4)), dim3(256), 0, (hipStream_t)stream, jobs);
  return launch_status();
}

int temp_gru_chain_fwd(const TempGruChain* c, const float* gi, float* h_out, float* saved, void* stream) {
  int rc = chain_check(c);
  if (rc) return rc;
  if (c->n_panels == 0) return TEMP_OK;
  if (!gi || !h_out || !saved) return TEMP_E_BADARG;
  const ChainArgs a = chain_args(c);
  hipStream_t st = (hipStream_t)stream;
  const int tpw = ceil_div(chain_geom(c->d).NT, 4);
#define TEMP_CHAIN_FWD(V)                                                            \
  switch (tpw) {                                                                     \
    case 1: return launch_chain_fwd<V, 1>(a, gi, h_out, saved, st);                  \
    case 2: return launch_chain_fwd<V, 2>(a, gi, h_out, saved, st);                  \
    case 3: return launch_chain_fwd<V, 3>(a, gi, h_out, saved, st);                  \
    case 4: return launch_chain_fwd<V, 4>(a, gi, h_out, saved, st);                  \
    case 5: return launch_chain_fwd<V, 5>(a, gi, h_out, saved, st);                  \
    case 6: return launch_chain_fwd<V, 6>(a, gi, h_out, saved, st);                  \
    default: return TEMP_E_UNSUPPORTED;                                              \
  }
  if (c->variant == TEMP_GRU_TORCH) { TEMP_CHAIN_FWD(TEMP_GRU_TORCH) }
  TEMP_CHAIN_FWD(TEMP_GRU_TYPE1)
#undef TEMP_CHAIN_FWD
}

int temp_gru_chain_bwd_g4(const TempGruChain* c, const float* saved, int n_up, const float* const* up, float* g4, void* stream) {
  int rc = chain_check(c);
  if (rc) return rc;
  if (n_up < 0 || n_up > TEMP_CHAIN_MAX_UP || (n_up > 0 && !up)) return TEMP_E_BADARG;
  if (c->variant != TEMP_GRU_TORCH) return TEMP_E_UNSUPPORTED;
  if (c->n_panels == 0) return TEMP_OK;
  if (!saved || !g4) return TEMP_E_BADARG;
  const ChainArgs a = chain_args(c);
  ChainUps ups = {};
  for (int i = 0; i < n_up; ++i) ups.p[i] = up[i];
  hipStream_t st = (hipStream_t)stream;
  const int tpw = ceil_div(chain_geom(c->d).NTb, 4);
  if (tpw == 1) return launch_chain_bwd<TEMP_GRU_TORCH, 1, 1>(a, ups, saved, g4, nullptr, st);
  if (tpw == 2) return launch_chain_bwd<TEMP_GRU_TORCH, 2, 1>(a, ups, saved, g4, nullptr, st);
  return TEMP_E_UNSUPPORTED;
}

int temp_gru_chain_keys_supported(int d) { return d > 0 && chain_hx(d) ? 1 : 0; }

int temp_gru_chain_bwd_g4_keys(const TempGruChain* c, const float* saved, int n_up, const float* const* up, float* g4, uint32_t* row_keys,
                               uint32_t* col_keys, void* stream) {
  int rc = chain_check(c);
  if (rc) return rc;
  if (n_up < 0 || n_up > TEMP_CHAIN_MAX_UP || (n_up > 0 && !up)) return TEMP_E_BADARG;
  if (c->variant != TEMP_GRU_TORCH || !chain_hx(c->d)) return TEMP_E_UNSUPPORTED;
  if (c->n_panels == 0) return TEMP_OK;
  if (!saved || !g4) return TEMP_E_BADARG;
  const ChainArgs a = chain_args(c);
  ChainUps ups = {};
  for (int i = 0; i < n_up; ++i) ups.p[i] = up[i];
  hipStream_t st = (hipStream_t)stream;
  const int tpw = ceil_div(chain_geom(c->d).NTb, 4);
  if (tpw == 1) return launch_chain_bwd<TEMP_GRU_TORCH, 1, 1>(a, ups, saved, g4, nullptr, st, row_keys, col_keys);
  if (tpw == 2) return launch_chain_bwd<TEMP_GRU_TORCH, 2, 1>(a, ups, saved, g4, nullptr, st, row_keys, col_keys);
  return TEMP_E_UNSUPPORTED;
}

int temp_gru_chain_bwd(const TempGruChain* c, const float* saved, int n_up, const float* const* up, float* dgi, float* dgh, void* stream) {
  int rc = chain_check(c);
  if (rc) return rc;
  if (n_up < 0 || n_up > TEMP_CHAIN_MAX_UP || (n_up > 0 && !up)) return TEMP_E_BADARG;
  if (c->n_panels == 0) return TEMP_OK;
  if (!saved || !dgi || !dgh) return TEMP_E_BADARG;
  const ChainArgs a = chain_args(c);
  ChainUps ups = {};
  for (int i = 0; i < n_up; ++i) ups.p[i] = up[i];
  hipStream_t st = (hipStream_t)stream;
  const int tpw = ceil_div(chain_geom(c->d).NTb, 4);
  if (c->variant == TEMP_GRU_TORCH) {
    if (tpw == 1) return launch_chain_bwd<TEMP_GRU_TORCH, 1>(a, ups, saved, dgi, dgh, st);
    if (tpw == 2) return launch_chain_bwd<TEMP_GRU_TORCH, 2>(a, ups, saved, dgi, dgh, st);
  } else {
    if (tpw == 1) return launch_chain_bwd<TEMP_GRU_TYPE1, 1>(a, ups, saved, dgi, dgh, st);
    if (tpw == 2) return launch_chain_bwd<TEMP_GRU_TYPE1, 2>(a, ups, saved, dgi, dgh, st);
  }
  return TEMP_E_UNSUPPORTED;
}

}
```

temp_amd/csrc/gru_chain_hx.hpp:

```cpp
#pragma once
#include "hx_pack.hpp"

namespace temp {

#define CHX_STATE_SCALE 16384.f
#define CHX_STATE_INV (1.f / 16384.f)

struct ChainGeomHx {
  int NT, NS;
  int NTb, NSb;
  int lda, ldz;
  int ldp, ldpa;
  int ldh;
};
__host__ __device__ inline ChainGeomHx chain_geom_hx(int D) {
  ChainGeomHx g;
  g.NT = (3 * D + 31) >> 5; g.NS = (D + 15) >> 4;
  g.NTb = (D + 31) >> 5; g.NSb = (((3 * D + 15) >> 4) + 7) & ~7;
  g.lda = g.NT * 32 + 4; g.ldz = g.NTb * 32 + 4;
  g.ldp = g.NS * 32 + 16; g.ldpa = g.NSb * 32 + 16;
  g.ldh = g.NS * 16 + 4;
  return g;
}
inline size_t chain_lds_fwd_hx(int D, int ms) {
// ... 56 lines not shown
#pragma unroll
        for (int r = 0; r < 16; ++r) acc[j][r] = 0.f;
      const hx_u32x4* wp = reinterpret_cast<const hx_u32x4*>(R.wf);
      constexpr bool ONESET = NMW > 4 && !TWOSETS;
      constexpr bool PREF = !(NMW > 4 && TWOSETS);
      hx_u32x4 w[ONESET ? 1 : 2][2][TPW] = {};
      auto wload = [&](hx_u32x4 (&wr)[TPW], int sl, int pl) {
#pragma unroll
        for (int j = 0; j < TPW; ++j)
          if (tval[j]) wr[j] = wp[((size_t)(sl * NT + tidx[j]) * 2 + pl) * 64 + lane];
      };
      const int rot = (a.dbg & 64) ? 0 : (int)(blockIdx.x >> 3) % NS;
      wload(w[0][0], rot, 0); wload(w[0][1], rot, 1);
      if constexpr (!ONESET) { wload(w[1][0], rot + 1 < NS ? rot + 1 : 0, 0); wload(w[1][1], rot + 1 < NS ? rot + 1 : 0, 1); }
      const char* hrow = hpl + (size_t)li * ldp + 16 * hh;
      const int pl1 = CH_SLOTS * ldp;
      for (int s = 0; s < ns; ++s) {
        const int flags = flagb[s];
        if ((flags & 1) && !(a.dbg & 1)) {
          hx_u32x4 FH = *reinterpret_cast<const hx_u32x4*>(hrow + 32 * rot), FL = *reinterpret_cast<const hx_u32x4*>(hrow + pl1 + 32 * rot), NH, NL;
          int sl_cur = rot;
          auto slab = [&](auto set_c, int sl1, int sl2) {
            constexpr int SET = decltype(set_c)::value;
            if constexpr (PREF) {
              NH = *reinterpret_cast<const hx_u32x4*>(hrow + 32 * sl1);
              NL = *reinterpret_cast<const hx_u32x4*>(hrow + pl1 + 32 * sl1);
            } else {
              FH = *reinterpret_cast<const hx_u32x4*>(hrow + 32 * sl_cur);
              FL = *reinterpret_cast<const hx_u32x4*>(hrow + pl1 + 32 * sl_cur);
              sl_cur = sl1;
            }
            const hx_f16x8 ah = hx_frag(FH), al = hx_frag(FL);
            __builtin_amdgcn_sched_barrier(0);
#pragma unroll
            for (int j = 0; j < TPW; ++j) acc[j] = __builtin_amdgcn_mfma_f32_32x32x16_f16(hx_frag(w[SET][1][j]), ah, acc[j], 0, 0, 0);
            __builtin_amdgcn_sched_barrier(0);
            wload(w[SET][1], sl2, 1);
            __builtin_amdgcn_sched_barrier(0);
#pragma unroll
            for (int j = 0; j < TPW; ++j) acc[j] = __builtin_amdgcn_mfma_f32_32x32x16_f16(hx_frag(w[SET][0][j]), al, acc[j], 0, 0, 0);
#pragma unroll
            for (int j = 0; j < TPW; ++j) acc[j] = __builtin_amdgcn_mfma_f32_32x32x16_f16(hx_frag(w[SET][0][j]), ah, acc[j], 0, 0, 0);
            __builtin_amdgcn_sched_barrier(0);
            wload(w[SET][0], sl2, 0);
            if constexpr (PREF) { FH = NH; FL = NL; }
          };
          auto at = [&](int j) { const int v = rot + j; return v < NS ? v : v - NS; };
          if constexpr (ONESET) {
            for (int j = 0; j < NS; ++j) slab(std::integral_constant<int, 0>(), at(j + 1 < NS ? j + 1 : 0), at(j + 1 < NS ? j + 1 : 0));
          } else {
          int j = 0;
          for (; j + 1 < NS; j += 2) {
            slab(std::integral_constant<int, 0>(), at(j + 1), at(j + 2 < NS ? j + 2 : 0));
            slab(std::integral_constant<int, 1>(), at(j + 2 < NS ? j + 2 : 0), at(j + 3 < NS ? j + 3 : 1));
          }
          if (j < NS) slab(std::integral_constant<int, 0>(), at(0), at(0));
          }
#pragma unroll
          for (int j = 0; j < TPW; ++j) {
            if (!tval[j]) continue;
            float* dst = accb + (size_t)li * lda + tidx[j] * 32 + 4 * hh;
#pragma unroll
            for (int qq = 0; qq < 4; ++qq) {
              st4(dst + 8 * qq, make_float4(acc[j][4 * qq], acc[j][4 * qq + 1], acc[j][4 * qq + 2], acc[j][4 * qq + 3]));
              acc[j][4 * qq] = 0.f; acc[j][4 * qq + 1] = 0.f; acc[j][4 * qq + 2] = 0.f; acc[j][4 * qq + 3] = 0.f;
            }
          }
        }
        __syncthreads();
        __syncthreads();
      }
    } else {
      const int mw = wave - NMW, c4 = lane, col = 4 * c4;
      const bool cact = c4 < D4;
      const int colc = cact ? col : 0;
      const float4 bhr = ld4(R.b_hh + colc), bhz = ld4(R.b_hh + D + colc), bhn = ld4(R.b_hh + 2 * D + colc);
      int erow[PASSES];
      float4 g0[PASSES], g1[PASSES], g2[PASSES];
      auto prefetch = [&](int s) {
#pragma unroll
        for (int ps = 0; ps < PASSES; ++ps) {
          const int e = tabb[s * CH_SLOTS + ps * MW + mw];
          erow[ps] = e;
          const bool ok = e >= 0 && cact && !(a.dbg & 4);
          const int er = e & CH_ROW_MASK;
          const float* src = gi + (ok ? (size_t)(a.gi_index ? a.gi_index[er] : er) * G + col : 0);
          if (VARIANT == TEMP_GRU_TORCH) { g0[ps] = ld4(src); g1[ps] = ld4(src + (ok ? D : 0)); g2[ps] = ld4(src + (ok ? 2 * D : 0)); }
          else { g0[ps] = zero4(); g1[ps] = zero4(); g2[ps] = ld4(src); }
        }
      };
      prefetch(0);
      for (int s = 0; s < ns; ++s) {
        const int flags = flagb[s];
        __syncthreads();
#pragma unroll
        for (int ps = 0; ps < PASSES; ++ps) {
          const int slot = ps * MW + mw;
          const int e = erow[ps];
          if (e < 0 || !cact) continue;
          const size_t row = (size_t)(e & CH_ROW_MASK);
          const bool hp = (e & CH_HAS_PREV) != 0;
          float4 ar = zero4(), az = zero4(), an = zero4(), hd = zero4();
          if (hp) {
            const float* ab = accb + (size_t)slot * lda + col;
            const float dec = decb[s * CH_SLOTS + slot];
            const float4 pr = ld4(ab), pz = ld4(ab + D), pn = ld4(ab + 2 * D);
            const float4 ivr = ld4(ivt + col), ivz = ld4(ivt + D + col), ivn = ld4(ivt + 2 * D + col);
            ar = make_float4(pr.x * (ivr.x * dec), pr.y * (ivr.y * dec), pr.z * (ivr.z * dec), pr.w * (ivr.w * dec));
            az = make_float4(pz.x * (ivz.x * dec), pz.y * (ivz.y * dec), pz.z * (ivz.z * dec), pz.w * (ivz.w * dec));
            an = make_float4(pn.x * (ivn.x * dec), pn.y * (ivn.y * dec), pn.z * (ivn.z * dec), pn.w * (ivn.w * dec));
            hd = scale4(ld4(hb + (size_t)slot * ldh + col), dec);
          }
          float o_h[4], o_r[4], o_z[4], o_n[4], o_hn[4];
          const float arv[4] = {ar.x, ar.y, ar.z, ar.w}, azv[4] = {az.x, az.y, az.z, az.w}, anv[4] = {an.x, an.y, an.z, an.w};
          const float hdv[4] = {hd.x, hd.y, hd.z, hd.w};
          const float g0v[4] = {g0[ps].x, g0[ps].y, g0[ps].z, g0[ps].w}, g1v[4] = {g1[ps].x, g1[ps].y, g1[ps].z, g1[ps].w};
          const float g2v[4] = {g2[ps].x, g2[ps].y, g2[ps].z, g2[ps].w};
          const float brv[4] = {bhr.x, bhr.y, bhr.z, bhr.w}, bzv[4] = {bhz.x, bhz.y, bhz.z, bhz.w}, bnv[4] = {bhn.x, bhn.y, bhn.z, bhn.w};
#pragma unroll
          for (int k = 0; k < 4; ++k) {
            float xr = arv[k], xz = azv[k];
            if (VARIANT == TEMP_GRU_TORCH) { xr += g0v[k]; xz += g1v[k]; }
            const float rg = gate_sigmoid(xr + brv[k]);
            const float zg = gate_sigmoid(xz + bzv[k]);
            const float hn = anv[k] + bnv[k];
            const float ng = gate_tanh(g2v[k] + rg * hn);
            o_h[k] = (VARIANT == TEMP_GRU_TORCH) ? ((1.f - zg) * ng + zg * hdv[k]) : (ng + zg * (hdv[k] - ng));
            o_r[k] = rg; o_z[k] = zg; o_n[k] = ng; o_hn[k] = hn;
          }
          const float4 h4 = make_float4(o_h[0], o_h[1], o_h[2], o_h[3]);
          st4(hb + (size_t)slot * ldh + col, h4);
          hx_u32x2 SH, SL;
          hx_split4(h4, CHX_STATE_SCALE, SH, SL);
          char* hdst = hpl + (size_t)slot * ldp + 2 * col;
          *reinterpret_cast<hx_u32x2*>(hdst) = SH;
          *reinterpret_cast<hx_u32x2*>(hdst + CH_SLOTS * ldp) = SL;
          const size_t o = row * D + col;
          if (a.dbg & 2) continue;
          if (flags & 2) st4(H + o, h4);
          st4(saved + o, make_float4(o_r[0], o_r[1], o_r[2], o_r[3]));
          st4(saved + plane + o, make_float4(o_z[0], o_z[1], o_z[2], o_z[3]));
          st4(saved + 2 * plane + o, make_float4(o_n[0], o_n[1], o_n[2], o_n[3]));
          st4(saved + 3 * plane + o, make_float4(o_hn[0], o_hn[1], o_hn[2], o_hn[3]));
          st4(saved + 4 * plane + o, hd);
        }
        __syncthreads();
        if (s + 1 < ns) prefetch(s + 1);
      }
    }
    __syncthreads();
  }
}

template <int VARIANT, int TPWB, int MW, int G4, int NMW = 4, int RING = 4>
__global__ void __launch_bounds__(64 * (NMW + MW)) k_gru_chain_bwd_hx(ChainArgs a, ChainUps ups, const float* __restrict__ saved,
                                                                     float* __restrict__ dgi, float* __restrict__ dgh,
                                                                     unsigned* __restrict__ row_keys, unsigned* __restrict__ col_keys) {
  extern __shared__ __attribute__((aligned(16))) float lds[];
  constexpr int PASSES = CH_SLOTS / MW;
  const int D = a.D, D4 = D >> 2;
  const ChainGeomHx g = chain_geom_hx(D);
  const int NTb = g.NTb, NSb = g.NSb, ldpa = g.ldpa, ldz = g.ldz;
  char* apl = (char*)lds;
  float* gzb = (float*)(apl + 2 * CH_SLOTS * ldpa);
  float* dpb = gzb + CH_SLOTS * ldz;
  int* tabb = (int*)(dpb + CH_SLOTS * ldz);
  float* decb = (float*)(tabb + CH_SLOTS * a.max_steps);
  int* flagb = (int*)(decb + CH_SLOTS * a.max_steps);
  int* upb = flagb + a.max_steps;
  float* rinv = (float*)(upb + 2 * a.max_steps);
  unsigned* ckey = (unsigned*)(rinv + CH_SLOTS);
  const int tid = threadIdx.x, wave = __builtin_amdgcn_readfirstlane(tid >> 6), lane = tid & 63;
  const size_t plane = a.plane;

  for (int p = blockIdx.x; p < a.n_panels; p += gridDim.x) {
    const int rnn_id = a.panel[4 * p], s0 = a.panel[4 * p + 1], ns = a.panel[4 * p + 2];
    const ChainRnn R = a.rnn[rnn_id];
    for (int i = tid; i < 2 * CH_SLOTS * ldpa / 16; i += blockDim.x) reinterpret_cast<hx_u32x4*>(apl)[i] = hx_u32x4{0u, 0u, 0u, 0u};
    for (int i = tid; i < 4 * D; i += blockDim.x) ckey[i] = 0u;
    if (tid < ns) { upb[2 * tid] = a.sinfo[4 * (size_t)(s0 + tid) + 1]; upb[2 * tid + 1] = a.sinfo[4 * (size_t)(s0 + tid) + 2]; }
    for (int i = tid; i < ns * CH_SLOTS; i += blockDim.x) {
      const int e = a.rows[(size_t)s0 * CH_SLOTS + i];
      tabb[i] = e;
      decb[i] = e >= 0 ? expf(-a.dt[e & CH_ROW_MASK] * a.lambda) : 0.f;
    }
    if (tid < ns) flagb[tid] = a.sinfo[4 * (size_t)(s0 + tid)];
    __syncthreads();

    if (wave < NMW) {
      const int li = lane & 31, hh = lane >> 5;
      bool tval[TPWB];
      int tidx[TPWB];
#pragma unroll
      for (int j = 0; j < TPWB; ++j) { tidx[j] = wave + NMW * j; tval[j] = tidx[j] < NTb; if (!tval[j]) tidx[j] = NTb - 1; }
      f32x16 acc[TPWB];
#pragma unroll
      for (int j = 0; j < TPWB; ++j)
#pragma unroll
        for (int r = 0; r < 16; ++r) acc[j][r] = 0.f;
      const hx_u32x4* wp = reinterpret_cast<const hx_u32x4*>(R.wb);
      hx_u32x4 wh[RING][TPWB] = {}, wl[RING][TPWB] = {};
      auto wload = [&](hx_u32x4 (&w)[TPWB], int sl, int pl) {
#pragma unroll
        for (int j = 0; j < TPWB; ++j)
          if (tval[j]) w[j] = wp[((size_t)(sl * NTb + tidx[j]) * 2 + pl) * 64 + lane];
      };
      const int rot = (a.dbg & 64) ? 0 : RING * ((int)(blockIdx.x >> 3) % (NSb / RING));
#pragma unroll
      for (int q = 0; q < RING; ++q) { wload(wh[q], rot + q, 0); wload(wl[q], rot + q, 1); }
      const char* arow = apl + (size_t)li * ldpa + 16 * hh;
      const int pl1 = CH_SLOTS * ldpa;
      for (int s = ns - 1; s >= 0; --s) {
        const int flags = flagb[s];
        __syncthreads();
        if ((flags & 1) && !(a.dbg & 1)) {
          hx_u32x4 FH = *reinterpret_cast<const hx_u32x4*>(arow + 32 * rot), FL = *reinterpret_cast<const hx_u32x4*>(arow + pl1 + 32 * rot), NH, NL;
          for (int j = 0, sl = rot; j < NSb; j += RING) {
            const int base2 = sl + RING < NSb ? sl + RING : 0;
#pragma unroll
            for (int q = 0; q < RING; ++q) {
              const int sn = (q < RING - 1) ? sl + q + 1 : base2;
              NH = *reinterpret_cast<const hx_u32x4*>(arow + 32 * sn);
              NL = *reinterpret_cast<const hx_u32x4*>(arow + pl1 + 32 * sn);
              const hx_f16x8 ah = hx_frag(FH), al = hx_frag(FL);
              __builtin_amdgcn_sched_barrier(0);
#pragma unroll
              for (int t = 0; t < TPWB; ++t) acc[t] = __builtin_amdgcn_mfma_f32_32x32x16_f16(hx_frag(wl[q][t]), ah, acc[t], 0, 0, 0);
              __builtin_amdgcn_sched_barrier(0);
              wload(wl[q], base2 + q, 1);
              __builtin_amdgcn_sched_barrier(0);
#pragma unroll
              for (int t = 0; t < TPWB; ++t) acc[t] = __builtin_amdgcn_mfma_f32_32x32x16_f16(hx_frag(wh[q][t]), al, acc[t], 0, 0, 0);
#pragma unroll
              for (int t = 0; t < TPWB; ++t) acc[t] = __builtin_amdgcn_mfma_f32_32x32x16_f16(hx_frag(wh[q][t]), ah, acc[t], 0, 0, 0);
              __builtin_amdgcn_sched_barrier(0);
              wload(wh[q], base2 + q, 0);
              FH = NH; FL = NL;
            }
            sl = base2;
          }
          const float dec = decb[s * CH_SLOTS + li], ri = rinv[li];
#pragma unroll
          for (int j = 0; j < TPWB; ++j) {
            if (!tval[j]) continue;
#pragma unroll
            for (int qq = 0; qq < 4; ++qq) {
              const int c = tidx[j] * 32 + 8 * qq + 4 * hh;
              const float4 gz = ld4(gzb + (size_t)li * ldz + c);
              const float i0 = hx_inv_scale(R.kb[c]) * ri, i1 = hx_inv_scale(R.kb[c + 1]) * ri, i2 = hx_inv_scale(R.kb[c + 2]) * ri, i3 = hx_inv_scale(R.kb[c + 3]) * ri;
              st4(dpb + (size_t)li * ldz + c, make_float4((acc[j][4 * qq] * i0 + gz.x) * dec, (acc[j][4 * qq + 1] * i1 + gz.y) * dec,
                                                           (acc[j][4 * qq + 2] * i2 + gz.z) * dec, (acc[j][4 * qq + 3] * i3 + gz.w) * dec));
              acc[j][4 * qq] = 0.f; acc[j][4 * qq + 1] = 0.f; acc[j][4 * qq + 2] = 0.f; acc[j][4 * qq + 3] = 0.f;
            }
          }
        }
        __syncthreads();
      }
    } else {
      const int mw = wave - NMW, c4 = lane, col = 4 * c4;
      const bool cact = c4 < D4;
      const int colc = cact ? col : 0;
      int erow[PASSES];
      bool nxt[PASSES];
      float4 sr[PASSES], sz[PASSES], sn[PASSES], shn[PASSES], shd[PASSES];
      unsigned ck[4][4] = {};
      auto prefetch = [&](int s) {
#pragma unroll
        for (int ps = 0; ps < PASSES; ++ps) {
          const int slot = ps * MW + mw;
          const int e = tabb[s * CH_SLOTS + slot];
          erow[ps] = e;
          int en = -1;
          if (s + 1 < ns) en = tabb[(s + 1) * CH_SLOTS + slot];
          nxt[ps] = en >= 0 && (en & CH_HAS_PREV);
          const bool ok = e >= 0 && cact && !(a.dbg & 4);
          const size_t row = ok ? (size_t)(e & CH_ROW_MASK) : 0;
          const float* src = saved + row * D + (ok ? col : 0);
          sr[ps] = ld4(src); sz[ps] = ld4(src + plane); sn[ps] = ld4(src + 2 * plane); shn[ps] = ld4(src + 3 * plane);
          shd[ps] = ld4(src + 4 * plane);
        }
      };
      prefetch(ns - 1);
      for (int s = ns - 1; s >= 0; --s) {
        const int up_sel = upb[2 * s], up_row0 = upb[2 * s + 1];
        const float* upp = up_sel >= 0 ? ups.p[up_sel] : nullptr;
#pragma unroll
        for (int ps = 0; ps < PASSES; ++ps) {
          const int slot = ps * MW + mw;
          const int e = erow[ps];
          if (e < 0) continue;
          const size_t row = (size_t)(e & CH_ROW_MASK);
          float4 gd = (upp && cact) ? ld4(upp + (row - (size_t)up_row0) * D + col) : zero4();
          if (nxt[ps] && cact) gd = add4(gd, ld4(dpb + (size_t)slot * ldz + col));
          const float4 rg = sr[ps], zg = sz[ps], ng = sn[ps], hn = shn[ps], hd = shd[ps];
          float4 dr_pre, dz_pre, dn_pre, dhn, gz;
#define TEMP_GATE(c)                                          \
          {                                                   \
            const float dn = gd.c * (1.f - zg.c);             \
            const float dz = gd.c * (hd.c - ng.c);            \
            dn_pre.c = dn * (1.f - ng.c * ng.c);              \
            dr_pre.c = dn_pre.c * hn.c * rg.c * (1.f - rg.c); \
            dz_pre.c = dz * zg.c * (1.f - zg.c);              \
            dhn.c = dn_pre.c * rg.c;                          \
            gz.c = gd.c * zg.c;                               \
          }
          TEMP_GATE(x) TEMP_GATE(y) TEMP_GATE(z) TEMP_GATE(w)
// ... 64 lines not shown
```

temp_amd/csrc/hx_pack.hpp:

```cpp
#pragma once
#include "common.hpp"
#include "split_f16.hpp"

namespace temp {

#define HX_PACK_JOBS 8
struct HxPackJob { const float* B; hx_u32x4* out; unsigned* keys; int K, N, n_tiles, n_slabs, ldb, trans, unit0, kblock0; };
struct HxPackJobs { HxPackJob j[HX_PACK_JOBS]; int count, total_units, total_kblocks; };

inline size_t hx_packed_items(int N, int K) { return (size_t)ceil_div(K, 16) * ceil_div(N, 32) * 128; }

inline void hx_pack_jobs_add(HxPackJobs& jobs, const float* B, hx_u32x4* out, unsigned* keys, int K, int N, int ldb, int trans, int n_slabs = 0) {
  HxPackJob& j = jobs.j[jobs.count++];
  j.B = B; j.out = out; j.keys = keys; j.K = K; j.N = N; j.n_tiles = ceil_div(N, 32); j.n_slabs = n_slabs > 0 ? n_slabs : ceil_div(K, 16); j.ldb = ldb; j.trans = trans;
  j.unit0 = jobs.total_units; j.kblock0 = jobs.total_kblocks;
  jobs.total_units += j.n_tiles * j.n_slabs;
  jobs.total_kblocks += j.n_tiles;
}

__device__ __forceinline__ const HxPackJob& hx_job_of(const HxPackJobs& jobs, int idx, bool by_kblock, int& local) {
  int ji = 0;
#pragma unroll
  for (int i = 1; i < HX_PACK_JOBS; ++i)
    if (i < jobs.count && idx >= (by_kblock ? jobs.j[i].kblock0 : jobs.j[i].unit0)) ji = i;
  local = idx - (by_kblock ? jobs.j[ji].kblock0 : jobs.j[ji].unit0);
  return jobs.j[ji];
}

static __global__ void __launch_bounds__(1024) k_hx_keys_pack(HxPackJobs jobs) {
  __shared__ unsigned sm[32][33];
  __shared__ float scale_l[32];
  int t;
  const HxPackJob& jb = hx_job_of(jobs, blockIdx.x, true, t);
  const int K = jb.K, N = jb.N, ldb = jb.ldb;
  const float* __restrict__ B = jb.B;
  unsigned key = 0;
  int c, g;
  if (jb.trans) {
    c = threadIdx.x >> 5; g = threadIdx.x & 31;
    const int n = 32 * t + c;
    if (n < N) {
      const float* p = B + (size_t)n * ldb;
      if ((K & 3) == 0 && (ldb & 3) == 0) {
        for (int q0 = g; q0 < (K >> 2); q0 += 128) {
          float4 v[4];
#pragma unroll
          for (int i = 0; i < 4; ++i) { const int q = q0 + 32 * i; v[i] = q < (K >> 2) ? ld4(p + 4 * q) : zero4(); }
#pragma unroll
          for (int i = 0; i < 4; ++i) key = max(key, hx_abs_bits4(v[i]));
        }
      } else {
        for (int k = g; k < K; k += 32) key = max(key, hx_abs_bits(p[k]));
      }
    }
  } else {
    g = threadIdx.x >> 5; c = threadIdx.x & 31;
    const int n = 32 * t + c;
    if (n < N) {
      const float* p = B + n;
      for (int k0 = g; k0 < K; k0 += 256) {
        float v[8];
#pragma unroll
        for (int i = 0; i < 8; ++i) { const int k = k0 + 32 * i; v[i] = k < K ? p[(size_t)k * ldb] : 0.f; }
#pragma unroll
        for (int i = 0; i < 8; ++i) key = max(key, hx_abs_bits(v[i]));
      }
    }
  }
  sm[g][c] = key;
  __syncthreads();
  if (threadIdx.x < 32) {
    key = 0;
#pragma unroll
    for (int i = 0; i < 32; ++i) key = max(key, sm[i][threadIdx.x]);
    jb.keys[32 * t + threadIdx.x] = key;
    scale_l[threadIdx.x] = hx_scale(key);
  }
  __syncthreads();
  const int lane = threadIdx.x & 63, hh = lane >> 5, li = lane & 31, wave = threadIdx.x >> 6;
  const int n = 32 * t + li;
  const float sc = scale_l[li];
  for (int s0 = wave; s0 < jb.n_slabs; s0 += 16) {
    const int k = 16 * s0 + 8 * hh;
    float4 v0 = zero4(), v1 = zero4();
    if (n < N && k < K) {
      const bool full = k + 4 < K;
      if (jb.trans) {
        const float* p = B + (size_t)n * ldb + k;
        v0 = ld4(p);
        if (full) v1 = ld4(p + 4);
      } else {
        const float* p = B + (size_t)k * ldb + n;
        const size_t l = (size_t)ldb;
        v0 = make_float4(p[0], p[l], p[2 * l], p[3 * l]);
        if (full) v1 = make_float4(p[4 * l], p[5 * l], p[6 * l], p[7 * l]);
      }
    }
    hx_u32x4 H, L;
    hx_split8(v0, v1, sc, H, L);
    hx_u32x4* d = jb.out + ((size_t)s0 * jb.n_tiles + t) * 128 + lane;
    d[0] = H; d[64] = L;
  }
}

inline void hx_pack_launch(const HxPackJobs& jobs, int kid, hipStream_t st) {
  if (!jobs.count) return;
  TEMP_LAUNCH(kid, k_hx_keys_pack, dim3(jobs.total_kblocks), dim3(1024), 0, st, jobs);
}

__device__ __forceinline__ unsigned hx_wave_max(unsigned v) {
  v = max(v, (unsigned)__builtin_amdgcn_update_dpp(0, (int)v, 0xB1, 0xf, 0xf, true));
  v = max(v, (unsigned)__builtin_amdgcn_update_dpp(0, (int)v, 0x4E, 0xf, 0xf, true));
  v = max(v, (unsigned)__builtin_amdgcn_update_dpp(0, (int)v, 0x141, 0xf, 0xf, true));
  v = max(v, (unsigned)__builtin_amdgcn_update_dpp(0, (int)v, 0x140, 0xf, 0xf, true));
  const unsigned a = __builtin_amdgcn_readlane((int)v, 0), b = __builtin_amdgcn_readlane((int)v, 16);
  const unsigned c = __builtin_amdgcn_readlane((int)v, 32), d = __builtin_amdgcn_readlane((int)v, 48);
  return max(max(a, b), max(c, d));
}

static __global__ void __launch_bounds__(1024) k_keys_reduce(int n_part, int cols, const unsigned* __restrict__ part, unsigned* __restrict__ out,
                                                             const int32_t* __restrict__ owner, int owner_stride) {
  __shared__ unsigned sm[32][33];
  const int cl = threadIdx.x & 31, pg = threadIdx.x >> 5, c = blockIdx.x * 32 + cl, r = blockIdx.y;
  unsigned key = 0;
  if (c < cols) {
    for (int p0 = pg; p0 < n_part; p0 += 256) {
      unsigned v[8];
#pragma unroll
      for (int u = 0; u < 8; ++u) {
        const int p = p0 + 32 * u;
        v[u] = (p < n_part && (!owner || owner[(size_t)owner_stride * p] == r)) ? part[(size_t)p * cols + c] : 0u;
      }
#pragma unroll
      for (int u = 0; u < 8; ++u) key = max(key, v[u]);
    }
  }
  sm[pg][cl] = key;
  __syncthreads();
  if (threadIdx.x < 32 && blockIdx.x * 32 + threadIdx.x < cols) {
    key = 0;
#pragma unroll
    for (int i = 0; i < 32; ++i) key = max(key, sm[i][threadIdx.x]);
    out[(size_t)r * cols + blockIdx.x * 32 + threadIdx.x] = key;
  }
}

#define ABSMAX_BLOCKS 1024
#define ABSMAX_WAVES 16
template <bool GATHER>
__global__ void __launch_bounds__(64 * ABSMAX_WAVES) k_absmax_keys(int n_rows, int d, const float* __restrict__ X, int ldx, const int32_t* __restrict__ idx,
                                                     float* __restrict__ out, unsigned* __restrict__ row_keys, unsigned* __restrict__ col_part) {
  __shared__ hx_u32x4 sm[ABSMAX_WAVES][64];
  const int lane = threadIdx.x & 63, wave = threadIdx.x >> 6;
  const int d4 = d >> 2;
  const bool act = lane < d4;
  const int gw = blockIdx.x * ABSMAX_WAVES + wave, nw = gridDim.x * ABSMAX_WAVES;
  const float* xp = X + (act ? 4 * lane : 0);
  unsigned ck[4] = {0u, 0u, 0u, 0u};
  for (int r0 = gw; r0 < n_rows; r0 += 4 * nw) {
    float4 v[4];
    int src[4];
#pragma unroll
    for (int u = 0; u < 4; ++u) { const int r = r0 + u * nw; const int rr = r < n_rows ? r : r0; src[u] = GATHER ? idx[rr] : rr; }
#pragma unroll
    for (int u = 0; u < 4; ++u) { v[u] = ld4(xp + (size_t)(src[u] >= 0 ? src[u] : 0) * ldx); if (GATHER && src[u] < 0) v[u] = zero4(); }
#pragma unroll
    for (int u = 0; u < 4; ++u) {
      const int r = r0 + u * nw;
      const unsigned k = act ? hx_abs_bits4(v[u]) : 0u;
      if (r < n_rows) {
        if (GATHER && act) st4(out + (size_t)r * d + 4 * lane, v[u]);
        if (act) { ck[0] = max(ck[0], hx_abs_bits(v[u].x)); ck[1] = max(ck[1], hx_abs_bits(v[u].y)); ck[2] = max(ck[2], hx_abs_bits(v[u].z)); ck[3] = max(ck[3], hx_abs_bits(v[u].w)); }
        if (row_keys) { const unsigned rk = hx_wave_max(k); if (lane == 0) row_keys[r] = rk; }
      }
    }
  }
  if (!col_part) return;
  sm[wave][lane] = hx_u32x4{ck[0], ck[1], ck[2], ck[3]};
  __syncthreads();
  if (wave == 0 && act) {
    hx_u32x4 m = sm[0][lane];
#pragma unroll
    for (int w = 1; w < ABSMAX_WAVES; ++w) { const hx_u32x4 o = sm[w][lane]; m[0] = max(m[0], o[0]); m[1] = max(m[1], o[1]); m[2] = max(m[2], o[2]); m[3] = max(m[3], o[3]); }
    *reinterpret_cast<hx_u32x4*>(col_part + (size_t)blockIdx.x * d + 4 * lane) = m;
  }
}
inline int absmax_blocks(int n_rows) { const int b = ceil_div(n_rows, 8 * ABSMAX_WAVES); return b < 1 ? 1 : (b > ABSMAX_BLOCKS / 4 ? ABSMAX_BLOCKS / 4 : b); }
static inline void launch_absmax_keys(int n_rows, int d, const float* X, int ldx, unsigned* row_keys, unsigned* col_keys, unsigned* col_part, hipStream_t st) {
  const int blocks = absmax_blocks(n_rows);
  TEMP_LAUNCH(K_KEYS, (k_absmax_keys<false>), dim3(blocks), dim3(64 * ABSMAX_WAVES), 0, st, n_rows, d, X, ldx, (const int32_t*)nullptr, (float*)nullptr, row_keys, col_keys ? col_part : nullptr);
  if (col_keys) TEMP_LAUNCH(K_KEYS, k_keys_reduce, dim3(ceil_div(d, 32), 1), dim3(1024), 0, st, blocks, d, col_part, col_keys, (const int32_t*)nullptr, 0);
}

static inline void launch_gather_rows_keys(int n, int d, const float* table, const int32_t* idx, float* out, unsigned* row_keys, unsigned* col_keys,
                                           unsigned* col_part, hipStream_t st) {
  const int blocks = absmax_blocks(n);
  TEMP_LAUNCH(K_GATHER_ROWS, (k_absmax_keys<true>), dim3(blocks), dim3(64 * ABSMAX_WAVES), 0, st, n, d, table, d, idx, out, row_keys, col_keys ? col_part : nullptr);
  if (col_keys) TEMP_LAUNCH(K_GATHER_ROWS, k_keys_reduce, dim3(ceil_div(d, 32), 1), dim3(1024), 0, st, blocks, d, col_part, col_keys, (const int32_t*)nullptr, 0);
}

}
```

temp_amd/gru_chain.py:

```python
import numpy as np
import torch

from . import _hostlib, _lib
from .backend import get_backend


CHAIN_KERNELS = True
WEIGHT_GRADS_MULTI = True
KEYED_GRADS = True
GATE_GRADS_ONCE = True


class GruInstance:
    __slots__ = ("n", "x0", "h0", "rnn", "prev", "next", "prev_idx", "next_idx", "dt", "group")

    def __init__(self, n, x0, rnn, prev, prev_idx_np, dt_np, next_idx_np=None):
        self.n, self.x0, self.rnn, self.prev = int(n), int(x0), rnn, prev
        self.h0 = 0
        self.next = -1
        self.prev_idx = prev_idx_np
        self.next_idx = next_idx_np
        self.dt = dt_np
        self.group = -1


class GruProgram:
    def __init__(self, instances):
        self.inst = instances
        off = 0
        for it in instances:
            it.h0 = off
            off += it.n
        self.n_total = off
        for i, it in enumerate(instances):
            if it.prev >= 0:
                p = instances[it.prev]
                assert p.next == -1, "an instance feeds at most one successor"
                p.next = i
                if p.next_idx is None:
                    inv = np.full(p.n, -1, dtype=np.int32)
                    ok = it.prev_idx >= 0
                    inv[it.prev_idx[ok]] = np.nonzero(ok)[0].astype(np.int32)
                    p.next_idx = inv
        self.groups = []
        for i, it in enumerate(instances):
            g = self.groups[-1] if self.groups else None
            if g is not None and g["rnn"] == it.rnn and g["x1"] == it.x0 and g["h1"] == it.h0:
                g["x1"] += it.n
                g["h1"] += it.n
            else:
                self.groups.append(dict(rnn=it.rnn, x0=it.x0, x1=it.x0 + it.n, h0=it.h0, h1=it.h0 + it.n))
            it.group = len(self.groups) - 1
        depth = []
        for it in instances:
            depth.append(0 if it.prev < 0 else depth[it.prev] + 1)
        self.levels = []
        for lv in range(max(depth) + 1 if depth else 0):
            idx = [i for i, dp in enumerate(depth) if dp == lv and instances[i].n > 0]
            for k in range(0, len(idx), 4):
                self.levels.append(idx[k:k + 4])
        self.dev = None

    def chain_plan(self):
        if getattr(self, "_chain_plan", False) is not False:
            return self._chain_plan
        self._chain_plan = self._chain_plan_host()
        return self._chain_plan

    def _chain_plan_host(self):
        inst = self.inst
        if not any(it.prev >= 0 and it.n > 0 for it in inst):
            return None
        chains = []
        for head, it0 in enumerate(inst):
            if it0.prev >= 0:
                continue
            chain = [head]
            while inst[chain[-1]].next >= 0:
                chain.append(inst[chain[-1]].next)
            chains.append(chain)
        res = _hostlib.chain_tracks(chains, [it.n for it in inst], [it.h0 for it in inst], [it.rnn for it in inst],
                                    [getattr(it, "prev_idx", None) if it.prev >= 0 else None for it in inst], _lib.CHAIN_TRACKS, _lib.CHAIN_MAX_STEPS)
        if res is None:
            return None
        panel, rows, anyp, sinst = res
        return dict(panel=panel, rows=rows, any_prev=anyp, step_inst=sinst)

    def _chain_plan_numpy(self):
        inst = self.inst
        T = _lib.CHAIN_TRACKS
        panel, rows_tab, any_prev, step_inst = [], [], [], []
        s_base = 0
        plan = None
        ok = any(it.prev >= 0 and it.n > 0 for it in inst)
        for head, it0 in enumerate(inst):
            if not ok:
                break
            if it0.prev >= 0:
                continue
            chain = [head]
            while inst[chain[-1]].next >= 0:
                chain.append(inst[chain[-1]].next)
            chain = [i for i in chain]
            if any(inst[i].rnn != it0.rnn for i in chain):
                ok = False
                break
            n_tracks, prev_tr, steps = 0, None, []
            for k, i in enumerate(chain):
                it = inst[i]
                tr = np.full(it.n, -1, dtype=np.int64)
                has = np.zeros(it.n, dtype=bool)
                if k > 0 and it.n:
                    pi = np.asarray(it.prev_idx, dtype=np.int64)
                    has = pi >= 0
                    tr[has] = prev_tr[pi[has]]
                new = np.nonzero(~has)[0]
                if new.size:
                    used = np.zeros(n_tracks, dtype=bool)
                    used[tr[has]] = True
                    free = np.nonzero(~used)[0]
                    take = min(free.size, new.size)
                    tr[new[:take]] = free[:take]
                    extra = new.size - take
                    if extra:
                        tr[new[take:]] = n_tracks + np.arange(extra)
                        n_tracks += extra
                steps.append((i, tr, has))
                prev_tr = tr
            if n_tracks == 0:
                continue
            n_pan = (n_tracks + T - 1) // T
            tab = np.full((len(chain), n_pan * T), -1, dtype=np.int64)
            for k, (i, tr, has) in enumerate(steps):
                if tr.size:
                    tab[k, tr] = (inst[i].h0 + np.arange(tr.size)) | (has.astype(np.int64) << 30)
            tab = tab.reshape(len(chain), n_pan, T)
            active = (tab >= 0).any(axis=2)
            anyp = ((tab >= 0) & ((tab >> 30) & 1).astype(bool)).any(axis=2)
            act_t = active.T
            counts = act_t.sum(axis=1)
            if counts.max() > _lib.CHAIN_MAX_STEPS:
                ok = False
                break
            first = s_base + np.concatenate([[0], np.cumsum(counts)[:-1]])
            panel.append(np.stack([np.full(n_pan, it0.rnn), first, counts, np.zeros(n_pan, dtype=np.int64)], axis=1))
            rows_tab.append(tab.transpose(1, 0, 2)[act_t])
            any_prev.append(anyp.T[act_t])
            step_inst.append(np.broadcast_to(np.asarray(chain)[None, :], act_t.shape)[act_t])
            s_base += int(counts.sum())
        if ok and panel:
            pn = np.concatenate(panel)
            pn = pn[pn[:, 2] > 0]
            plan = dict(panel=pn.astype(np.int32), rows=np.concatenate(rows_tab).astype(np.int32),
                        any_prev=np.concatenate(any_prev), step_inst=np.concatenate(step_inst).astype(np.int64))
        return plan

    def chain_tables(self, device, want):
        plan = self.chain_plan()
        _lib.pause_point()
        if plan is None or (want is not None and len(want) > _lib.CHAIN_MAX_UP):
            return None
        cache = self.__dict__.setdefault("_chain_tabs", {})
        key = (str(device), want)
        tabs = cache.get(key)
        if tabs is None:
            S = plan["rows"].shape[0]
            sinfo = np.zeros((S, 4), dtype=np.int32)
            si = plan["step_inst"]
            if want is None:
                sinfo[:, 0] = plan["any_prev"].astype(np.int32) | 2
            else:
                sel = np.full(len(self.inst), -1, dtype=np.int32)
                sel[list(want)] = np.arange(len(want), dtype=np.int32)
                h0 = np.array([it.h0 for it in self.inst], dtype=np.int32)
                sinfo[:, 0] = plan["any_prev"].astype(np.int32) | np.where(sel[si] >= 0, 2, 0)
                sinfo[:, 1] = sel[si]
                sinfo[:, 2] = np.where(sel[si] >= 0, h0[si], 0)
            dt = np.zeros(self.n_total, dtype=np.float32)
            for it in self.inst:
                if it.n:
                    dt[it.h0:it.h0 + it.n] = np.asarray(it.dt, dtype=np.float32).reshape(-1)
            _lib.pause_point()
            parts = [plan["panel"].reshape(-1), plan["rows"].reshape(-1), sinfo.reshape(-1), dt.view(np.int32)]
            buf = _lib.to_device(np.concatenate(parts), device)
            cuts = np.cumsum([0] + [p.size for p in parts])
            tabs = cache[key] = dict(n_panels=int(plan["panel"].shape[0]), n_steps=int(S), max_steps=int(plan["panel"][:, 2].max()), panel=buf[cuts[0]:cuts[1]], rows=buf[cuts[1]:cuts[2]],
                                     sinfo=buf[cuts[2]:cuts[3]], dt_bits=buf[cuts[3]:cuts[4]])
        return tabs

    def gi_shared(self, device):
        src = getattr(self, "x_src", None)
        if src is None:
            return None
        c = getattr(self, "_gi_shared", None)
        if c is not None and c[0] == str(device):
            return c[1]
        src = np.asarray(src)
        reps, g0, index, total = [], [], np.zeros(self.n_total, dtype=np.int32), 0
        n_labels = int(src.max()) + 1 if src.size else 0
        for g in self.groups:
            assert g["x1"] - g["x0"] == g["h1"] - g["h0"]
            first, inv = _hostlib.unique_labels(src[g["x0"]:g["x1"]], n_labels)
            reps.append(first)
            g0.append(total)
            index[g["h0"]:g["h1"]] = total + inv.reshape(-1)
            total += first.size
        res = None
        if total * 8 <= self.n_total * 7:
            buf = _lib.to_device(np.concatenate(reps + [index]), device)
            cuts = np.cumsum([0] + [r.size for r in reps])
            res = dict(rep=[buf[cuts[i]:cuts[i + 1]] for i in range(len(reps))], g0=g0, rows=int(total), gi_index=buf[cuts[-1]:])
        self._gi_shared = (str(device), res)
        return res

    def constants(self, device, d):
        key = (str(device), int(d))
        c = getattr(self, "_const", None)
        if c is None or c[0] != key:
            n0 = max([it.n for it in self.inst if it.prev < 0] + [1])
            c = self._const = (key, torch.zeros(1, d, dtype=torch.float32, device=device), torch.full((n0,), -1, dtype=torch.int32, device=device))
        return c[1], c[2]

    def upload(self, device):
        if self.dev is not None and self.dev[0] == str(device):
            return self.dev[1]
        parts, spans, off = [], [], 0
        for it in self.inst:
            span = []
            for arr in (it.prev_idx.astype(np.int32) if it.prev >= 0 else None, it.next_idx,
                        np.ascontiguousarray(it.dt, dtype=np.float32).view(np.int32)):
                if arr is None:
                    span.append(None)
                    continue
                parts.append(arr.reshape(-1))
                span.append((off, off + arr.size))
                off += arr.size
            spans.append(span)
        buf = _lib.to_device(np.concatenate(parts) if parts else np.zeros(0, np.int32), device)
        cut = lambda sp: buf[sp[0]:sp[1]] if sp is not None else None
        t = [(cut(a), cut(b), cut(c).view(torch.float32)) for a, b, c in spans]
        self.dev = (str(device), t)
        return t


class _GruChainFn(torch.autograd.Function):
    @staticmethod
    def forward(ctx, x_all, prog, lam, variant, n_rnn, want, x_keys, *weights):
        be = get_backend()
        dev = x_all.device
        d = x_all.shape[1]
        G = weights[0].shape[0]
        N = prog.n_total
        x_all = x_all.detach().contiguous()
        W = [tuple(w.detach().contiguous() for w in weights[4 * r:4 * r + 4]) for r in range(n_rnn)]
        tabs = None
        if CHAIN_KERNELS and hasattr(be, "gru_chain_fwd") and n_rnn <= _lib.CHAIN_MAX_RNN and be.gru_chain_supported(d):
            tabs = prog.chain_tables(dev, want)
        share = prog.gi_shared(dev) if tabs is not None else None
        ctx.x_keys = x_keys if (x_keys is not None and tabs is not None) else None
        gk = (lambda: dict(x_keys=[ctx.x_keys[0][g["x0"]:g["x1"]] for g in prog.groups])) if ctx.x_keys is not None else dict
        gi_index = None
        if share is not None:
            gi_index = share["gi_index"]
            gi = torch.empty(share["rows"], G, dtype=torch.float32, device=dev)
            cut = share["g0"] + [share["rows"]]
            be.gru_input_gates_multi([x_all[g["x0"]:g["x1"]] for g in prog.groups], [W[g["rnn"]][0] for g in prog.groups],
                                     [W[g["rnn"]][2] for g in prog.groups], variant, [gi[cut[i]:cut[i + 1]] for i in range(len(prog.groups))],
                                     x_idx=share["rep"], **gk())
        else:
            gi = torch.empty(N, G, dtype=torch.float32, device=dev)
        if share is not None:
            pass
        elif len(prog.groups) > 1 and hasattr(be, "gru_input_gates_multi"):
            be.gru_input_gates_multi([x_all[g["x0"]:g["x1"]] for g in prog.groups], [W[g["rnn"]][0] for g in prog.groups],
                                     [W[g["rnn"]][2] for g in prog.groups], variant, [gi[g["h0"]:g["h1"]] for g in prog.groups], **gk())
        else:
            for g in prog.groups:
                w_ih, _, b_ih, _ = W[g["rnn"]]
                be.gru_input_gates(x_all[g["x0"]:g["x1"]], w_ih, b_ih, variant, gi[g["h0"]:g["h1"]])
        H = torch.empty(N, d, dtype=torch.float32, device=dev)
        saved = torch.empty(5, N, d, dtype=torch.float32, device=dev)
        packs = None
        if tabs is not None:
            packs = be.gru_chain_pack_multi([W[r][1] for r in range(n_rnn)]) if hasattr(be, "gru_chain_pack_multi") else \
                [be.gru_chain_pack(W[r][1]) for r in range(n_rnn)]
            be.gru_chain_fwd(tabs, gi, lam, variant, packs, [W[r][3] for r in range(n_rnn)], H, saved, gi_index=gi_index)
        else:
            tens = prog.upload(dev)
            zero, none_idx = prog.constants(dev, d)
        for level in (prog.levels if tabs is None else ()):
            cells = []
            for i in level:
                it = prog.inst[i]
                pi, _, dt = tens[i]
                _, w_hh, _, b_hh = W[it.rnn]
                if it.prev >= 0:
                    p = prog.inst[it.prev]
                    prev, pidx = H[p.h0:p.h0 + p.n], pi
                else:
                    prev, pidx = None, none_idx[:it.n]
                cells.append(dict(gi=gi[it.h0:it.h0 + it.n], prev=prev, prev_idx=pidx, dt=dt, w_hh=w_hh, b_hh=b_hh,
                                  h_out=H[it.h0:it.h0 + it.n], row0=it.h0))
            be.gru_cell_fwd_multi(cells, lam, variant, saved)
        ctx.set_materialize_grads(False)
        ctx.save_for_backward(x_all, saved, *[w for ws in W for w in ws])
        ctx.prog, ctx.lam, ctx.variant, ctx.n_rnn, ctx.G, ctx.want = prog, lam, variant, n_rnn, G, want
        ctx.tabs, ctx.packs = tabs, packs
        if want is None:
            return H
        return tuple(H[prog.inst[i].h0:prog.inst[i].h0 + prog.inst[i].n] for i in want)

    @staticmethod
    def backward(ctx, *d_outs):
        be = get_backend()
        x_all, saved = ctx.saved_tensors[:2]
        flat = ctx.saved_tensors[2:]
        W = [flat[4 * r:4 * r + 4] for r in range(ctx.n_rnn)]
        prog, lam, variant, G = ctx.prog, ctx.lam, ctx.variant, ctx.G
        dev, d, N = x_all.device, x_all.shape[1], prog.n_total
        if ctx.want is None:
            dH = d_outs[0].contiguous() if d_outs[0] is not None else torch.zeros(N, d, dtype=torch.float32, device=dev)
            up = lambda i, it: dH[it.h0:it.h0 + it.n]
        else:
            given = {i: g.contiguous() for i, g in zip(ctx.want, d_outs) if g is not None}
            up = lambda i, it: given.get(i)
        groups = list(prog.groups)
        zero_state = [all(it.prev < 0 for it in prog.inst if it.group == gi) for gi in range(len(groups))]
        disjoint = all(groups[a]["x1"] <= groups[b]["x0"] or groups[b]["x1"] <= groups[a]["x0"] for a in range(len(groups)) for b in range(a))
        one_launch = bool(groups and disjoint and not any(zero_state) and len({g["rnn"] for g in groups}) == len(groups) and WEIGHT_GRADS_MULTI)
        once = bool(one_launch and GATE_GRADS_ONCE and ctx.tabs is not None and hasattr(be, "gru_grads_g4")
                    and be.gru_grads_g4_supported([g["h1"] - g["h0"] for g in groups], d, variant))
        if once:
            g4 = torch.empty(N, 4 * d, dtype=torch.float32, device=dev)
            ups = [dH] if ctx.want is None else [given.get(i) for i in ctx.want]
            keyed = bool(KEYED_GRADS and hasattr(be, "gru_chain_keys_supported") and be.gru_chain_keys_supported(d))
            keys = (torch.empty(N, dtype=torch.int32, device=dev), torch.empty(ctx.n_rnn + ctx.tabs["n_panels"], 4 * d, dtype=torch.int32, device=dev)) if keyed else None
            be.gru_chain_bwd_g4(ctx.tabs, saved, ups, lam, variant, ctx.packs, [W[r][3] for r in range(ctx.n_rnn)], g4, **({"keys": keys} if keyed else {}))
            d_x_all = torch.empty_like(x_all)
            xsl = [slice(g["x0"], g["x1"]) for g in groups]
            hsl = [slice(g["h0"], g["h1"]) for g in groups]
            kw = dict(row_keys=[keys[0][b] for b in hsl], col_keys=[keys[1][g["rnn"]] for g in groups]) if keyed else {}
            if keyed and ctx.x_keys is not None:
                kw["x_col_keys"] = [ctx.x_keys[1]] * len(groups)
            multi = be.gru_grads_g4([x_all[a] for a in xsl], [saved[4, b] for b in hsl], [g4[b] for b in hsl], [W[g["rnn"]][0] for g in groups],
                                    [d_x_all[a] for a in xsl], **kw)
            grads = [None] * (4 * ctx.n_rnn)
            covered = np.zeros(x_all.shape[0], dtype=bool)
            for g, gw in zip(groups, multi):
                covered[g["x0"]:g["x1"]] = True
                for k in range(4):
                    grads[4 * g["rnn"] + k] = gw[k]
            if not covered.all():
                d_x_all[torch.from_numpy(~covered).to(dev)] = 0
            return (d_x_all, None, None, None, None, None, None) + tuple(grads)
        dgi = torch.empty(N, G, dtype=torch.float32, device=dev)
        dgh = torch.empty(N, 3 * d, dtype=torch.float32, device=dev)
        if ctx.tabs is not None:
            ups = [dH] if ctx.want is None else [given.get(i) for i in ctx.want]
            be.gru_chain_bwd(ctx.tabs, saved, ups, lam, variant, ctx.packs, [W[r][3] for r in range(ctx.n_rnn)], dgi, dgh)
        else:
            tens = prog.upload(dev)
            decv = torch.empty(N, dtype=torch.float32, device=dev)
            d_prev = torch.empty(N, d, dtype=torch.float32, device=dev)
        for level in (reversed(prog.levels) if ctx.tabs is None else ()):
            cells = []
            for i in level:
                it = prog.inst[i]
                _, ni, dt = tens[i]
                nxt = prog.inst[it.next] if (it.next >= 0 and prog.inst[it.next].n > 0) else None
                sl = slice(it.h0, it.h0 + it.n)
                cells.append(dict(row0=it.h0, n=it.n, dh_up=up(i, it), d_prev_next=d_prev[nxt.h0:nxt.h0 + nxt.n] if nxt is not None else None,
                                  next_idx=ni if nxt is not None else None, dt=dt, w_hh=W[it.rnn][1], dgi=dgi[sl], dgh=dgh[sl],
                                  decv=decv[sl], d_prev=d_prev[sl], no_prev=it.prev < 0))
            be.gru_cell_bwd_multi(cells, lam, variant, saved)
        d_x_all = torch.empty_like(x_all)
        written = np.zeros(x_all.shape[0], dtype=bool)
        grads = [None] * (4 * ctx.n_rnn)
        multi = None
        if one_launch and hasattr(be, "gru_weight_grads_multi"):
            xsl = [slice(g["x0"], g["x1"]) for g in groups]
            hsl = [slice(g["h0"], g["h1"]) for g in groups]
            multi = be.gru_weight_grads_multi([x_all[a] for a in xsl], [saved[4, b] for b in hsl], [dgi[b] for b in hsl], [dgh[b] for b in hsl],
                                              [W[g["rnn"]][0] for g in groups], variant, [d_x_all[a] for a in xsl])
        if multi is not None:
            for g, gw in zip(groups, multi):
                written[g["x0"]:g["x1"]] = True
                for k in range(4):
                    grads[4 * g["rnn"] + k] = gw[k]
            groups = []
        for g in groups:
            gi_ = prog.groups.index(g)
            xs, hs = slice(g["x0"], g["x1"]), slice(g["h0"], g["h1"])
            first = not written[xs].any()
            assert first or written[xs].all()
            tgt = d_x_all[xs] if first else torch.empty(g["x1"] - g["x0"], d, dtype=torch.float32, device=dev)
            gw = be.gru_weight_grads(x_all[xs], None if zero_state[gi_] else saved[4, hs], dgi[hs], dgh[hs], W[g["rnn"]][0], variant, tgt)
            if not first:
                d_x_all[xs] += tgt
            written[xs] = True
            for k in range(4):
                j = 4 * g["rnn"] + k
                grads[j] = gw[k] if grads[j] is None else grads[j] + gw[k]
        if not written.all():
            d_x_all[torch.from_numpy(~written).to(dev)] = 0
        return (d_x_all, None, None, None, None, None, None) + tuple(grads)


def chain_kernels_usable(d, n_rnn=1):
    be = get_backend()
    return bool(CHAIN_KERNELS and hasattr(be, "gru_chain_fwd") and n_rnn <= _lib.CHAIN_MAX_RNN and be.gru_chain_supported(d))


def prepare_program(prog, device, d, n_rnn, want):
    if chain_kernels_usable(d, n_rnn) and prog.chain_tables(device, tuple(want) if want is not None else None) is not None:
        _lib.pause_point()
        prog.gi_shared(device)
        return
    prog.upload(device)


def zero_state_program(n):
    return GruProgram([GruInstance(n, 0, 0, -1, np.full(n, -1, dtype=np.int32), np.zeros(n, dtype=np.float32))])


def gru_chain(x_all, prog, rnns, lam, type1=False, want=None, x_keys=None):
    ws = []
    for r in rnns:
        if type1:
            ws += [r.weight_ih, r.weight_hh, r.bias_ih, r.bias_hh]
        else:
            ws += [r.weight_ih_l0, r.weight_hh_l0, r.bias_ih_l0, r.bias_hh_l0]
    return _GruChainFn.apply(x_all, prog, float(lam), _lib.GRU_TYPE1 if type1 else _lib.GRU_TORCH, len(rnns),
                             tuple(want) if want is not None else None, x_keys, *ws)
```

Baseline: 875.4 million.

## Fuse GRU input-gate GEMM into chain forward kernel with joint W_ih/W_hh packing

Adds a fused forward chain kernel that computes the input-gate projection x·W_ih inside the recurrent chain kernel, reading x through a row index, instead of materialising the gi tensor with a separate GEMM launch first. W_ih is packed alongside W_hh in the split hx format by a joint pack job, and pack-layout tags are threaded through the chain descriptor so forward and backward pick kernels by layout. This removes one GEMM launch and the gi write/read round trip. In exchange the chain kernel does more MFMA work per step on its serial path and uses more LDS.

```diff
diff --git a/include/temp_amd.h b/include/temp_amd.h
--- a/include/temp_amd.h
+++ b/include/temp_amd.h
@@ -207,12 +207,21 @@
   const float* packed[TEMP_CHAIN_MAX_RNN];
   const float* b_hh[TEMP_CHAIN_MAX_RNN];
   const int32_t* gi_index;
+  int32_t pack_layout;
 } TempGruChain;
+enum { TEMP_CHAIN_PACK_F32 = 1, TEMP_CHAIN_PACK_BX = 2, TEMP_CHAIN_PACK_HX = 3, TEMP_CHAIN_PACK_HX_X = 4 };
+int temp_gru_chain_pack_layout(int d);
 int temp_gru_chain_supported(int d);
 size_t temp_gru_chain_pack_floats(int d);
 int temp_gru_chain_pack(int d, const float* w_hh, float* packed, void* stream);
 int temp_gru_chain_pack_multi(int count, int d, const float* const* w_hh, float* const* packed, void* stream);
 int temp_gru_chain_fwd(const TempGruChain* c, const float* gi, float* h_out, float* saved, void* stream);
+int temp_gru_chain_fwd_x_supported(int d, int variant, int max_steps);
+size_t temp_gru_chain_pack_x_floats(int d);
+int temp_gru_chain_pack_x_multi(int count, int d, const float* const* w_hh, const float* const* w_ih, float* const* packed, void* stream);
+int temp_gru_chain_fwd_x(const TempGruChain* c, const float* x, const int32_t* x_index, const float* const* b_ih, float* h_out, float* saved,
+                         void* stream);
+long long temp_gru_chain_fwd_x_launches(void);
 int temp_gru_chain_bwd(const TempGruChain* c, const float* saved, int n_up, const float* const* up ,
                        float* dgi, float* dgh, void* stream);
 int temp_gru_chain_bwd_g4(const TempGruChain* c, const float* saved, int n_up, const float* const* up ,
diff --git a/temp_amd/_lib.py b/temp_amd/_lib.py
--- a/temp_amd/_lib.py
+++ b/temp_amd/_lib.py
@@ -52,13 +52,14 @@
 CHAIN_MAX_RNN = 4
 CHAIN_MAX_UP = 8
 CHAIN_MAX_STEPS = 64
+CHAIN_PACK_F32, CHAIN_PACK_BX, CHAIN_PACK_HX, CHAIN_PACK_HX_X = 1, 2, 3, 4
 
 
 class TempGruChain(ctypes.Structure):
     _fields_ = [("d", ctypes.c_int32), ("variant", ctypes.c_int32), ("n_panels", ctypes.c_int32), ("n_steps", ctypes.c_int32),
                 ("max_steps", ctypes.c_int32), ("panel", c_vp), ("rows", c_vp), ("sinfo", c_vp), ("dt", c_vp), ("lambda_", ctypes.c_float),
                 ("saved_plane", ctypes.c_size_t), ("n_rnn", ctypes.c_int32), ("packed", c_vp * CHAIN_MAX_RNN), ("b_hh", c_vp * CHAIN_MAX_RNN),
-                ("gi_index", c_vp)]
+                ("gi_index", c_vp), ("pack_layout", ctypes.c_int32)]
 
 
 class TempSubsampleJob(ctypes.Structure):
@@ -133,6 +134,12 @@
     "temp_gru_chain_pack": (_I, [_I, c_vp, c_vp, c_vp]),
     "temp_gru_chain_pack_multi": (_I, [_I, _I, ctypes.POINTER(c_vp), ctypes.POINTER(c_vp), c_vp]),
     "temp_gru_chain_fwd": (_I, [ctypes.POINTER(TempGruChain), c_vp, c_vp, c_vp, c_vp]),
+    "temp_gru_chain_pack_layout": (_I, [_I]),
+    "temp_gru_chain_fwd_x_supported": (_I, [_I, _I, _I]),
+    "temp_gru_chain_pack_x_floats": (_SZ, [_I]),
+    "temp_gru_chain_pack_x_multi": (_I, [_I, _I, ctypes.POINTER(c_vp), ctypes.POINTER(c_vp), ctypes.POINTER(c_vp), c_vp]),
+    "temp_gru_chain_fwd_x": (_I, [ctypes.POINTER(TempGruChain), c_vp, c_vp, ctypes.POINTER(c_vp), c_vp, c_vp, c_vp]),
+    "temp_gru_chain_fwd_x_launches": (ctypes.c_longlong, []),
     "temp_gru_chain_bwd": (_I, [ctypes.POINTER(TempGruChain), c_vp, _I, ctypes.POINTER(c_vp), c_vp, c_vp, c_vp]),
     "temp_gru_chain_bwd_g4": (_I, [ctypes.POINTER(TempGruChain), c_vp, _I, ctypes.POINTER(c_vp), c_vp, c_vp]),
     "temp_gru_chain_keys_supported": (_I, [_I]),
diff --git a/temp_amd/backend.py b/temp_amd/backend.py
--- a/temp_amd/backend.py
+++ b/temp_amd/backend.py
@@ -313,7 +313,9 @@
         w_hh = _f32(w_hh, "w_hh")
         d = w_hh.shape[1]
         out = torch.empty(self.lib.temp_gru_chain_pack_floats(d), dtype=torch.float32, device=w_hh.device)
+        layout = self.lib.temp_gru_chain_pack_layout(d)
         _lib.check(self.lib.temp_gru_chain_pack(d, _ptr(w_hh), _ptr(out), _stream()), "temp_gru_chain_pack")
+        out.chain_pack_layout = layout
         return out
 
     def gru_chain_pack_multi(self, w_hhs):
@@ -323,14 +325,24 @@
         buf = torch.empty(len(w_hhs), n, dtype=torch.float32, device=w_hhs[0].device)
         src = (ctypes.c_void_p * len(w_hhs))(*[w.data_ptr() for w in w_hhs])
         dst = (ctypes.c_void_p * len(w_hhs))(*[buf[i].data_ptr() for i in range(len(w_hhs))])
+        layout = self.lib.temp_gru_chain_pack_layout(d)
         _lib.check(self.lib.temp_gru_chain_pack_multi(len(w_hhs), d, src, dst, _stream()), "temp_gru_chain_pack_multi")
-        return [buf[i] for i in range(len(w_hhs))]
+        return self._tagged([buf[i] for i in range(len(w_hhs))], layout)
+
+    @staticmethod
+    def _tagged(packs, layout):
+        for pk in packs:
+            pk.chain_pack_layout = layout
+        return packs
 
     def _chain_desc(self, tabs, d, variant, lam, plane, packs, b_hhs):
         c = _lib.TempGruChain()
         c.d, c.variant, c.n_panels, c.n_steps, c.max_steps = d, variant, tabs["n_panels"], tabs["n_steps"], tabs["max_steps"]
         c.panel, c.rows, c.sinfo, c.dt = (_i32(tabs[k], k).data_ptr() for k in ("panel", "rows", "sinfo", "dt_bits"))
         c.lambda_, c.saved_plane, c.n_rnn = float(lam), plane, len(packs)
+        layouts = {getattr(pk, "chain_pack_layout", None) for pk in packs}
+        assert len(layouts) == 1 and None not in layouts, "chain packs without one common layout tag (gru_chain_pack*)"
+        c.pack_layout = layouts.pop()
         keep = []
         for i, (pk, b) in enumerate(zip(packs, b_hhs)):
             pk, b = _f32(pk, "packed"), _f32(b, "b_hh")
@@ -346,6 +358,30 @@
             c.gi_index = _i32(gi_index, "gi_index").data_ptr()
         rc = self.lib.temp_gru_chain_fwd(ctypes.byref(c), _ptr(_f32(gi, "gi")), _ptr(h_out), _ptr(saved_all), _stream())
         _lib.check(rc, "temp_gru_chain_fwd")
+
+    def gru_chain_fwd_x_supported(self, d, variant, max_steps):
+        return bool(self.lib.temp_gru_chain_fwd_x_supported(int(d), int(variant), int(max_steps)))
+
+    def gru_chain_pack_x_multi(self, w_hhs, w_ihs):
+        w_hhs, w_ihs = [_f32(w, "w_hh") for w in w_hhs], [_f32(w, "w_ih") for w in w_ihs]
+        d = w_hhs[0].shape[1]
+        k = len(w_hhs)
+        n = self.lib.temp_gru_chain_pack_x_floats(d)
+        buf = torch.empty(k, n, dtype=torch.float32, device=w_hhs[0].device)
+        arr = lambda ts: (ctypes.c_void_p * k)(*[t.data_ptr() for t in ts])
+        _lib.check(self.lib.temp_gru_chain_pack_x_multi(k, d, arr(w_hhs), arr(w_ihs), arr([buf[i] for i in range(k)]), _stream()),
+                   "temp_gru_chain_pack_x_multi")
+        return self._tagged([buf[i] for i in range(k)], _lib.CHAIN_PACK_HX_X)
+
+    def gru_chain_fwd_x(self, tabs, x, x_index, lam, variant, packs, b_hhs, b_ihs, h_out, saved_all):
+        d = saved_all.shape[2]
+        c, keep = self._chain_desc(tabs, d, variant, lam, saved_all.shape[1] * d, packs, b_hhs)
+        x = _f32(x, "x")
+        assert x.shape[1] == d and x_index.shape[0] == saved_all.shape[1]
+        b_ihs = [_f32(b, "b_ih") for b in b_ihs]
+        barr = (ctypes.c_void_p * len(b_ihs))(*[b.data_ptr() for b in b_ihs])
+        rc = self.lib.temp_gru_chain_fwd_x(ctypes.byref(c), _ptr(x), _ptr(_i32(x_index, "x_index")), barr, _ptr(h_out), _ptr(saved_all), _stream())
+        _lib.check(rc, "temp_gru_chain_fwd_x")
 
     def gru_chain_bwd(self, tabs, saved_all, ups, lam, variant, packs, b_hhs, dgi, dgh):
         d = saved_all.shape[2]
diff --git a/temp_amd/csrc/gru_chain.hip b/temp_amd/csrc/gru_chain.hip
--- a/temp_amd/csrc/gru_chain.hip
+++ b/temp_amd/csrc/gru_chain.hip
@@ -1,3 +1,4 @@
+#include <atomic>
 #include "common.hpp"
 #include "gru_math.hpp"
 #include "gemm_bx.hpp"
@@ -12,6 +13,7 @@
 struct ChainRnn { const float4* wf; const float4* wb; const float* b_hh; const unsigned* kf; const unsigned* kb; };
 struct ChainArgs {
   int D, n_panels, max_steps, dbg;
+  int layout;
   int n_rnn_keys;
   const int32_t* panel; const int32_t* rows; const int32_t* sinfo;
   const float* dt;
@@ -574,6 +576,7 @@
   }
 }
 
+static bool chain_layout_ok(int layout, int d);
 static int chain_check(const TempGruChain* c) {
   if (!c || c->d <= 0 || c->n_panels < 0 || c->n_steps < 0 || c->n_rnn <= 0 || c->n_rnn > TEMP_CHAIN_MAX_RNN) return TEMP_E_BADARG;
   if (c->variant != TEMP_GRU_TORCH && c->variant != TEMP_GRU_TYPE1) return TEMP_E_BADARG;
@@ -581,27 +584,37 @@
   for (int i = 0; i < c->n_rnn; ++i) if (!c->packed[i] || !c->b_hh[i]) return TEMP_E_BADARG;
   if (c->max_steps <= 0 || c->max_steps > CH_MAX_STEPS) return TEMP_E_BADARG;
   if (!temp_gru_chain_supported(c->d)) return TEMP_E_UNSUPPORTED;
+  if (!chain_layout_ok(c->pack_layout, c->d)) return TEMP_E_BADARG;
   return TEMP_OK;
 }
 
 static bool chain_bx(int d) { return bx_enabled() && d % 8 == 0; }
-static bool chain_hx(int d) {
-  if (!chain_bx(d) || !hx_enabled()) return false;
+static bool chain_hx_fits(int d) {
+  if (d % 8) return false;
   const ChainGeomHx g = chain_geom_hx(d);
   return chain_lds_fwd_hx(d, CH_MAX_STEPS) <= CH_LDS_LIMIT && chain_lds_bwd_hx(d, CH_MAX_STEPS) <= CH_LDS_LIMIT && g.NT <= 20 && g.NTb <= 8;
 }
+static bool chain_hx(int d) { return chain_bx(d) && hx_enabled() && chain_hx_fits(d); }
+static int chain_pack_layout(int d) { return chain_hx(d) ? TEMP_CHAIN_PACK_HX : chain_bx(d) ? TEMP_CHAIN_PACK_BX : TEMP_CHAIN_PACK_F32; }
+static bool chain_layout_ok(int layout, int d) {
+  if (layout == TEMP_CHAIN_PACK_F32) return true;
+  if (layout == TEMP_CHAIN_PACK_BX) return d % 8 == 0;
+  return (layout == TEMP_CHAIN_PACK_HX || layout == TEMP_CHAIN_PACK_HX_X) && chain_hx_fits(d);
+}
+static bool layout_hx(int layout) { return layout == TEMP_CHAIN_PACK_HX || layout == TEMP_CHAIN_PACK_HX_X; }
 
 static ChainArgs chain_args(const TempGruChain* c) {
   ChainArgs a = {};
   const ChainGeom g = chain_geom(c->d);
   a.D = c->d; a.n_panels = c->n_panels; a.max_steps = c->max_steps; a.panel = c->panel; a.rows = c->rows; a.sinfo = c->sinfo; a.dt = c->dt;
+  a.layout = c->pack_layout;
   a.n_rnn_keys = c->n_rnn; a.lambda = c->lambda; a.plane = c->saved_plane; a.gi_index = c->gi_index; a.dbg = option(TEMP_OPT_DEBUG) >> 8;
   for (int i = 0; i < c->n_rnn; ++i) {
     a.rnn[i].wf = (const float4*)c->packed[i];
-    a.rnn[i].wb = (const float4*)c->packed[i] + (chain_bx(c->d) ? (size_t)(g.NQ >> 1) * g.NT * 192 : (size_t)g.NT * g.NQ * 64);
+    a.rnn[i].wb = (const float4*)c->packed[i] + (a.layout == TEMP_CHAIN_PACK_BX ? (size_t)(g.NQ >> 1) * g.NT * 192 : (size_t)g.NT * g.NQ * 64);
     a.rnn[i].b_hh = c->b_hh[i];
     a.rnn[i].kf = a.rnn[i].kb = nullptr;
-    if (chain_hx(c->d)) {
+    if (layout_hx(a.layout)) {
       const ChainGeomHx gx = chain_geom_hx(c->d);
       a.rnn[i].wb = (const float4*)c->packed[i] + chain_hx_fwd_items(c->d);
       a.rnn[i].kf = (const unsigned*)((const float4*)c->packed[i] + chain_hx_fwd_items(c->d) + chain_hx_bwd_items(c->d));
@@ -625,7 +638,7 @@
   static bool attr = false;
   static bool attr_bx = false;
   static bool attr_hx = false;
-  if (chain_hx(a.D)) {
+  if (layout_hx(a.layout)) {
     const size_t lds_hx = chain_lds_fwd_hx(a.D, a.max_steps);
     constexpr int TPW8 = (TPW * 4 + 7) / 8 < 1 ? 1 : (TPW * 4 + 7) / 8;
     const int cfg = (a.dbg >> 4) & 3;
@@ -657,7 +670,7 @@
     return launch_status();
   }
   const size_t lds = chain_lds_fwd(a.D, a.max_steps);
-  if (chain_bx(a.D)) {
+  if (a.layout == TEMP_CHAIN_PACK_BX) {
     auto kernel = k_gru_chain_fwd<VARIANT, TPW, 4, 1>;
     int rc = chain_lds_attr(kernel, lds, &attr_bx);
     if (rc) return rc;
@@ -670,6 +683,15 @@
   TEMP_LAUNCH(K_GRU_CHAIN_FWD, kernel, dim3(a.n_panels), dim3(512), lds, st, a, gi, h, saved);
   return launch_status();
 }
+
+#define CH_FWD_X_OFF 0x400000
+static std::atomic<long long> g_fwd_x_launches{0};
+static size_t chain_x_ih_offset(int d) { return chain_hx_pack_floats(d); }
+static bool chain_fwd_x_fits(int d, int max_steps) {
+  return chain_hx_fits(d) && d / 4 <= 64 && max_steps > 0 && max_steps <= CH_MAX_STEPS && chain_lds_fwd_x(d, max_steps) <= CH_LDS_LIMIT &&
+         (chain_geom_hx(d).NT + 7) / 8 <= 3;
+}
+static bool chain_fwd_x_ok(int d, int max_steps) { return chain_hx(d) && !(option(TEMP_OPT_DEBUG) & CH_FWD_X_OFF) && chain_fwd_x_fits(d, max_steps); }
 
 template <int VARIANT, int TPWB, int G4 = 0>
 static int launch_chain_bwd(const ChainArgs& a, const ChainUps& ups, const float* saved, float* dgi, float* dgh, hipStream_t st,
@@ -677,7 +699,7 @@
   static bool attr = false;
   static bool attr_bx = false;
   static bool attr_hx = false;
-  if (chain_hx(a.D)) {
+  if (layout_hx(a.layout)) {
     const size_t lds_hx = chain_lds_bwd_hx(a.D, a.max_steps);
     constexpr int TPWB8 = (TPWB * 4 + 7) / 8 < 1 ? 1 : (TPWB * 4 + 7) / 8;
     const int cfg = (a.dbg >> 4) & 3;
@@ -705,7 +727,7 @@
   }
   if (row_keys || col_keys) return TEMP_E_UNSUPPORTED;
   const size_t lds = chain_lds_bwd(a.D, a.max_steps);
-  if (chain_bx(a.D)) {
+  if (a.layout == TEMP_CHAIN_PACK_BX) {
     auto kernel = k_gru_chain_bwd<VARIANT, TPWB, 8, 1, G4>;
     int rc = chain_lds_attr(kernel, lds, &attr_bx);
     if (rc) return rc;
@@ -818,6 +840,75 @@
 #undef TEMP_CHAIN_FWD
 }
 
+int temp_gru_chain_fwd_x_supported(int d, int variant, int max_steps) {
+  return d > 0 && d % 8 == 0 && variant == TEMP_GRU_TORCH && chain_fwd_x_ok(d, max_steps) ? 1 : 0;
+}
+
+size_t temp_gru_chain_pack_x_floats(int d) {
+  if (d <= 0) return 0;
+  return chain_x_ih_offset(d) + chain_hx_fwd_items(d) * 4;
+}
+
+int temp_gru_chain_pack_x_multi(int count, int d, const float* const* w_hh, const float* const* w_ih, float* const* packed, void* stream) {
+  if (count <= 0 || count > TEMP_CHAIN_MAX_RNN || d <= 0 || !w_hh || !w_ih || !packed) return TEMP_E_BADARG;
+  for (int i = 0; i < count; ++i) if (!w_hh[i] || !w_ih[i] || !packed[i]) return TEMP_E_BADARG;
+  if (d % 8 || !chain_hx(d)) return TEMP_E_UNSUPPORTED;
+  const ChainGeomHx gx = chain_geom_hx(d);
+  HxPackJobs jobs = {};
+  for (int i = 0; i < count; ++i) {
+    hx_u32x4* pf = reinterpret_cast<hx_u32x4*>(packed[i]);
+    hx_u32x4* pb = pf + chain_hx_fwd_items(d);
+    unsigned* kf = reinterpret_cast<unsigned*>(pb + chain_hx_bwd_items(d));
+    hx_u32x4* pi = reinterpret_cast<hx_u32x4*>(packed[i] + chain_x_ih_offset(d));
+    if (jobs.count + 2 > HX_PACK_JOBS) { hx_pack_launch(jobs, K_GRU_CHAIN_PACK, (hipStream_t)stream); jobs = HxPackJobs{}; }
+    hx_pack_jobs_add_joint(jobs, w_hh[i], pf, w_ih[i], pi, kf, d, 3 * d, d, 1);
+    hx_pack_jobs_add(jobs, w_hh[i], pb, kf + gx.NT * 32, 3 * d, d, d, 0, gx.NSb);
+  }
+  hx_pack_launch(jobs, K_GRU_CHAIN_PACK, (hipStream_t)stream);
+  return launch_status();
+}
+
+int temp_gru_chain_fwd_x(const TempGruChain* c, const float* x, const int32_t* x_index, const float* const* b_ih, float* h_out, float* saved, void* stream) {
+  int rc = chain_check(c);
+  if (rc) return rc;
+  if (c->pack_layout != TEMP_CHAIN_PACK_HX_X) return TEMP_E_BADARG;
+  if (c->variant != TEMP_GRU_TORCH || !chain_fwd_x_fits(c->d, c->max_steps)) return TEMP_E_UNSUPPORTED;
+  if (c->n_panels == 0) return TEMP_OK;
+  if (!x || !x_index || !b_ih || !h_out || !saved) return TEMP_E_BADARG;
+  for (int i = 0; i < c->n_rnn; ++i) if (!b_ih[i]) return TEMP_E_BADARG;
+  const ChainArgs a = chain_args(c);
+  ChainX X = {};
+  X.x = x; X.x_index = x_index;
+  const ChainGeomHx gx = chain_geom_hx(c->d);
+  for (int i = 0; i < c->n_rnn; ++i) {
+    X.b_ih[i] = b_ih[i];
+    X.wi[i] = reinterpret_cast<const hx_u32x4*>(c->packed[i] + chain_x_ih_offset(c->d));
+  }
+  static bool attr = false;
+  const size_t lds = chain_lds_fwd_x(c->d, c->max_steps);
+  hipStream_t st = (hipStream_t)stream;
+  if ((gx.NT + 7) / 8 == 3) {
+    auto kernel = k_gru_chain_fwd_x<3, 8, 8>;
+    if ((rc = chain_lds_attr(kernel, lds, &attr))) return rc;
+    TEMP_LAUNCH(K_GRU_CHAIN_FWD, kernel, dim3(a.n_panels), dim3(1024), lds, st, a, X, h_out, saved);
+  } else if ((gx.NT + 7) / 8 == 2) {
+    static bool attr2 = false;
+    auto kernel = k_gru_chain_fwd_x<2, 8, 8>;
+    if ((rc = chain_lds_attr(kernel, lds, &attr2))) return rc;
+    TEMP_LAUNCH(K_GRU_CHAIN_FWD, kernel, dim3(a.n_panels), dim3(1024), lds, st, a, X, h_out, saved);
+  } else {
+    static bool attr1 = false;
+    auto kernel = k_gru_chain_fwd_x<1, 8, 8>;
+    if ((rc = chain_lds_attr(kernel, lds, &attr1))) return rc;
+    TEMP_LAUNCH(K_GRU_CHAIN_FWD, kernel, dim3(a.n_panels), dim3(1024), lds, st, a, X, h_out, saved);
+  }
+  hx_count();
+  g_fwd_x_launches.fetch_add(1, std::memory_order_relaxed);
+  return launch_status();
+}
+
+long long temp_gru_chain_fwd_x_launches(void) { return g_fwd_x_launches.load(std::memory_order_relaxed); }
+
 int temp_gru_chain_bwd_g4(const TempGruChain* c, const float* saved, int n_up, const float* const* up, float* g4, void* stream) {
   int rc = chain_check(c);
   if (rc) return rc;
@@ -835,6 +926,8 @@
   return TEMP_E_UNSUPPORTED;
 }
 
+int temp_gru_chain_pack_layout(int d) { return d > 0 ? chain_pack_layout(d) : 0; }
+
 int temp_gru_chain_keys_supported(int d) { return d > 0 && chain_hx(d) ? 1 : 0; }
 
 int temp_gru_chain_bwd_g4_keys(const TempGruChain* c, const float* saved, int n_up, const float* const* up, float* g4, uint32_t* row_keys,
@@ -842,7 +935,7 @@
   int rc = chain_check(c);
   if (rc) return rc;
   if (n_up < 0 || n_up > TEMP_CHAIN_MAX_UP || (n_up > 0 && !up)) return TEMP_E_BADARG;
-  if (c->variant != TEMP_GRU_TORCH || !chain_hx(c->d)) return TEMP_E_UNSUPPORTED;
+  if (c->variant != TEMP_GRU_TORCH || !layout_hx(c->pack_layout)) return TEMP_E_UNSUPPORTED;
   if (c->n_panels == 0) return TEMP_OK;
   if (!saved || !g4) return TEMP_E_BADARG;
   const ChainArgs a = chain_args(c);
diff --git a/temp_amd/csrc/gru_chain_hx.hpp b/temp_amd/csrc/gru_chain_hx.hpp
--- a/temp_amd/csrc/gru_chain_hx.hpp
+++ b/temp_amd/csrc/gru_chain_hx.hpp
@@ -232,6 +232,283 @@
   }
 }
 
+struct ChainX {
+  const float* x;
+  const int32_t* x_index;
+  const float* b_ih[TEMP_CHAIN_MAX_RNN];
+  const hx_u32x4* wi[TEMP_CHAIN_MAX_RNN];
+};
+inline size_t chain_lds_fwd_x(int D, int ms) {
+  const ChainGeomHx g = chain_geom_hx(D);
+  return (size_t)CH_SLOTS * (3 * D + 4) * 4 + 4 * (size_t)CH_SLOTS * g.ldp + (size_t)CH_SLOTS * (D + 4) * 4 + CH_SLOTS * 4 + (2 * CH_SLOTS + 1) * (size_t)ms * 4;
+}
+template <int TPW, int MW, int NMW>
+__global__ void __launch_bounds__(64 * (NMW + MW)) k_gru_chain_fwd_x(ChainArgs a, ChainX X, float* __restrict__ H, float* __restrict__ saved) {
+  extern __shared__ __attribute__((aligned(16))) float lds[];
+  constexpr int PASSES = CH_SLOTS / MW;
+  const int D = a.D, D4 = D >> 2, G3 = 3 * D;
+  const ChainGeomHx g = chain_geom_hx(D);
+  const int NT = g.NT, NS = g.NS, ldp = g.ldp;
+  const int lda = G3 + 4, ldn = D + 4;
+  float* accb = lds;
+  char* hpl = (char*)(accb + CH_SLOTS * lda);
+  char* xpl = hpl + 2 * CH_SLOTS * ldp;
+  float* gin = (float*)(xpl + 2 * CH_SLOTS * ldp);
+  unsigned* xkey = (unsigned*)(gin + CH_SLOTS * ldn);
+  int* tabb = (int*)(xkey + CH_SLOTS);
+  float* decb = (float*)(tabb + CH_SLOTS * a.max_steps);
+  int* flagb = (int*)(decb + CH_SLOTS * a.max_steps);
+  const int tid = threadIdx.x, wave = __builtin_amdgcn_readfirstlane(tid >> 6), lane = tid & 63;
+  const size_t plane = a.plane;
+
+  if (wave < NMW) {
+  for (int p = blockIdx.x; p < a.n_panels; p += gridDim.x) {
+    const int rnn_id = a.panel[4 * p], s0 = a.panel[4 * p + 1], ns = a.panel[4 * p + 2];
+    const ChainRnn R = a.rnn[rnn_id];
+    for (int i = tid; i < 4 * CH_SLOTS * ldp / 16; i += blockDim.x) reinterpret_cast<hx_u32x4*>(hpl)[i] = hx_u32x4{0u, 0u, 0u, 0u};
+    for (int i = tid; i < ns * CH_SLOTS; i += blockDim.x) {
+      const int e = a.rows[(size_t)s0 * CH_SLOTS + i];
+      tabb[i] = e;
+      decb[i] = e >= 0 ? expf(-a.dt[e & CH_ROW_MASK] * a.lambda) : 0.f;
+    }
+    if (tid < ns) flagb[tid] = a.sinfo[4 * (size_t)(s0 + tid)];
+    __syncthreads();
+
+      const int li = lane & 31, hh = lane >> 5;
+      bool tval[TPW];
+      int tidx[TPW];
+#pragma unroll
+      for (int j = 0; j < TPW; ++j) { tidx[j] = wave + NMW * j; tval[j] = tidx[j] < NT; if (!tval[j]) tidx[j] = NT - 1; }
+      f32x16 acc[TPW];
+#pragma unroll
+      for (int j = 0; j < TPW; ++j)
+#pragma unroll
+        for (int r = 0; r < 16; ++r) acc[j][r] = 0.f;
+      const hx_u32x4* wph = reinterpret_cast<const hx_u32x4*>(R.wf);
+      const hx_u32x4* wpi = X.wi[rnn_id];
+      hx_u32x4 w[2][TPW] = {};
+      const std::integral_constant<int, 0> P0;
+      const std::integral_constant<int, 1> P1;
+      auto wload = [&](const hx_u32x4* wp, int sl, auto pl_c) __attribute__((always_inline)) {
+        constexpr int pl = decltype(pl_c)::value;
+#pragma unroll
+        for (int j = 0; j < TPW; ++j)
+          if (tval[j]) w[pl][j] = *reinterpret_cast<const hx_u32x4*>(reinterpret_cast<const char*>(wp) + (unsigned)((((sl * NT + tidx[j]) * 2 + pl) * 64 + lane) * 16));
+      };
+      const int rot = (a.dbg & 64) ? 0 : (int)(blockIdx.x >> 3) % NS;
+      auto at = [&](int j) { const int v = rot + j; return v < NS ? v : v - NS; };
+      const bool prio = !(a.dbg & 4096);
+      bool holds_ih = true;
+      wload(wpi, rot, P0); wload(wpi, rot, P1);
+      auto walk = [&](const bool prod, const char* pl0, const hx_u32x4* wcur, const hx_u32x4* wnext) __attribute__((always_inline)) {
+        const char* arow = pl0 + (size_t)li * ldp + 16 * hh;
+        const int pl1 = CH_SLOTS * ldp;
+        hx_u32x4 FH = *reinterpret_cast<const hx_u32x4*>(arow + 32 * rot), FL = *reinterpret_cast<const hx_u32x4*>(arow + pl1 + 32 * rot), NH, NL;
+        if (prio) __builtin_amdgcn_s_setprio(2);
+        for (int j = 0; j < NS; ++j) {
+          const bool last = j + 1 == NS;
+          const int sn = at(last ? 0 : j + 1);
+          const hx_u32x4* wn = last ? wnext : wcur;
+          NH = *reinterpret_cast<const hx_u32x4*>(arow + 32 * sn);
+          NL = *reinterpret_cast<const hx_u32x4*>(arow + pl1 + 32 * sn);
+          const hx_f16x8 ah = hx_frag(FH), al = hx_frag(FL);
+          __builtin_amdgcn_sched_barrier(0);
+#pragma unroll
+          for (int t = 0; t < TPW; ++t) {
+            if (prod) acc[t] = __builtin_amdgcn_mfma_f32_32x32x16_f16(hx_frag(w[1][t]), ah, acc[t], 0, 0, 0);
+            else asm volatile("" : : "v"(w[1][t]));
+          }
+          __builtin_amdgcn_sched_barrier(0);
+          wload(wn, sn, P1);
+          __builtin_amdgcn_sched_barrier(0);
+          if (prod) {
+#pragma unroll
+            for (int t = 0; t < TPW; ++t) acc[t] = __builtin_amdgcn_mfma_f32_32x32x16_f16(hx_frag(w[0][t]), al, acc[t], 0, 0, 0);
+#pragma unroll
+            for (int t = 0; t < TPW; ++t) acc[t] = __builtin_amdgcn_mfma_f32_32x32x16_f16(hx_frag(w[0][t]), ah, acc[t], 0, 0, 0);
+          } else {
+#pragma unroll
+            for (int t = 0; t < TPW; ++t) asm volatile("" : : "v"(w[0][t]));
+          }
+          __builtin_amdgcn_sched_barrier(0);
+          wload(wn, sn, P0);
+          FH = NH; FL = NL;
+        }
+        if (prio) __builtin_amdgcn_s_setprio(0);
+      };
+      auto xprod = [&]() __attribute__((always_inline)) {
+        if (!holds_ih) { wload(wpi, rot, P0); wload(wpi, rot, P1); }
+        walk(!(a.dbg & (1 | 2048)), xpl, wpi, wph);
+        holds_ih = false;
+        const float f = hx_inv_scale(xkey[li]) * CHX_STATE_SCALE;
+#pragma unroll
+        for (int j = 0; j < TPW; ++j)
+#pragma unroll
+          for (int r = 0; r < 16; ++r) acc[j][r] *= f;
+      };
+      if (ns > 0) {
+        __syncthreads();
+        xprod();
+        __syncthreads();
+      }
+      for (int s = 0; s < ns; ++s) {
+        const int flags = flagb[s];
+#pragma unroll
+        for (int j = 0; j < TPW; ++j) {
+          if (!tval[j]) continue;
+#pragma unroll
+          for (int qq = 0; qq < 4; ++qq) {
+            const int c = tidx[j] * 32 + 8 * qq + 4 * hh;
+            if (c < 2 * D || c >= G3) continue;
+            st4(gin + (size_t)li * ldn + (c - 2 * D), make_float4(acc[j][4 * qq], acc[j][4 * qq + 1], acc[j][4 * qq + 2], acc[j][4 * qq + 3]));
+            acc[j][4 * qq] = 0.f; acc[j][4 * qq + 1] = 0.f; acc[j][4 * qq + 2] = 0.f; acc[j][4 * qq + 3] = 0.f;
+          }
+        }
+        if ((flags & 1) && !(a.dbg & 1)) {
+          if (holds_ih) { wload(wph, rot, P0); wload(wph, rot, P1); }
+          walk(true, hpl, wph, wpi);
+          holds_ih = true;
+        }
+#pragma unroll
+        for (int j = 0; j < TPW; ++j) {
+          if (!tval[j]) continue;
+          float* dst = accb + (size_t)li * lda + tidx[j] * 32 + 4 * hh;
+#pragma unroll
+          for (int qq = 0; qq < 4; ++qq) {
+            if (tidx[j] * 32 + 8 * qq + 4 * hh < G3) st4(dst + 8 * qq, make_float4(acc[j][4 * qq], acc[j][4 * qq + 1], acc[j][4 * qq + 2], acc[j][4 * qq + 3]));
+            acc[j][4 * qq] = 0.f; acc[j][4 * qq + 1] = 0.f; acc[j][4 * qq + 2] = 0.f; acc[j][4 * qq + 3] = 0.f;
+          }
+        }
+        __syncthreads();
+        if (s + 1 < ns) xprod();
+        __syncthreads();
+      }
+    __syncthreads();
+  }
+  } else {
+  for (int p = blockIdx.x; p < a.n_panels; p += gridDim.x) {
+    const int rnn_id = a.panel[4 * p], s0 = a.panel[4 * p + 1], ns = a.panel[4 * p + 2];
+    const ChainRnn R = a.rnn[rnn_id];
+    for (int i = tid; i < 4 * CH_SLOTS * ldp / 16; i += blockDim.x) reinterpret_cast<hx_u32x4*>(hpl)[i] = hx_u32x4{0u, 0u, 0u, 0u};
+    for (int i = tid; i < ns * CH_SLOTS; i += blockDim.x) {
+      const int e = a.rows[(size_t)s0 * CH_SLOTS + i];
+      tabb[i] = e;
+      decb[i] = e >= 0 ? expf(-a.dt[e & CH_ROW_MASK] * a.lambda) : 0.f;
+    }
+    if (tid < ns) flagb[tid] = a.sinfo[4 * (size_t)(s0 + tid)];
+    __syncthreads();
+
+      const int mw = wave - NMW, c4 = lane, col = 4 * c4;
+      const bool cact = c4 < D4;
+      const int colc = cact ? col : 0;
+      const float* bih = X.b_ih[rnn_id];
+      const float4 br = add4(ld4(bih + colc), ld4(R.b_hh + colc)), bz = add4(ld4(bih + D + colc), ld4(R.b_hh + D + colc));
+      const float4 bhn = ld4(R.b_hh + 2 * D + colc), bin = ld4(bih + 2 * D + colc);
+      float4 ivr, ivz, ivn;
+      {
+        const hx_u32x4 kr = *reinterpret_cast<const hx_u32x4*>(R.kf + colc), kz = *reinterpret_cast<const hx_u32x4*>(R.kf + D + colc);
+        const hx_u32x4 kn = *reinterpret_cast<const hx_u32x4*>(R.kf + 2 * D + colc);
+        auto iv = [](const hx_u32x4 k) { return make_float4(hx_inv_scale(k[0]) * CHX_STATE_INV, hx_inv_scale(k[1]) * CHX_STATE_INV,
+                                                            hx_inv_scale(k[2]) * CHX_STATE_INV, hx_inv_scale(k[3]) * CHX_STATE_INV); };
+        ivr = iv(kr); ivz = iv(kz); ivn = iv(kn);
+      }
+      float4 hdr[PASSES];
+      float4 xr[PASSES];
+#pragma unroll
+      for (int ps = 0; ps < PASSES; ++ps) hdr[ps] = zero4();
+      auto xload = [&](int s) __attribute__((always_inline)) {
+#pragma unroll
+        for (int ps = 0; ps < PASSES; ++ps) {
+          const int e = tabb[s * CH_SLOTS + ps * MW + mw];
+          const bool ok = e >= 0 && cact && !(a.dbg & 4);
+          const size_t xrow = ok ? (size_t)X.x_index[e & CH_ROW_MASK] : 0;
+          xr[ps] = ok ? ld4(X.x + xrow * D + col) : zero4();
+        }
+      };
+      auto xsplit = [&]() __attribute__((always_inline)) {
+#pragma unroll
+        for (int ps = 0; ps < PASSES; ++ps) {
+          const int slot = ps * MW + mw;
+          const unsigned key = hx_wave_max(cact ? hx_abs_bits4(xr[ps]) : 0u);
+          if (cact) {
+            hx_u32x2 SH, SL;
+            hx_split4(xr[ps], hx_scale(key), SH, SL);
+            char* xd = xpl + (size_t)slot * ldp + 2 * col;
+            *reinterpret_cast<hx_u32x2*>(xd) = SH;
+            *reinterpret_cast<hx_u32x2*>(xd + CH_SLOTS * ldp) = SL;
+          }
+          if (lane == 0) xkey[slot] = key;
+        }
+      };
+      if (ns > 0) {
+        xload(0);
+        xsplit();
+        __syncthreads();
+        if (ns > 1) xload(1);
+        __syncthreads();
+      }
+      for (int s = 0; s < ns; ++s) {
+        const int flags = flagb[s];
+        if (s + 1 < ns) xsplit();
+        __syncthreads();
+        if (s + 2 < ns) xload(s + 2);
+#pragma unroll
+        for (int ps = 0; ps < PASSES; ++ps) {
+          const int slot = ps * MW + mw;
+          const int e = tabb[s * CH_SLOTS + slot];
+          if (!cact) continue;
+          int en = -1;
+          if (s + 1 < ns) en = tabb[(s + 1) * CH_SLOTS + slot];
+          const bool hpn = en >= 0 && (en & CH_HAS_PREV);
+          float4 h4 = zero4();
+          if (e >= 0) {
+            const size_t row = (size_t)(e & CH_ROW_MASK);
+            const bool hp = (e & CH_HAS_PREV) != 0;
+            const float* ab = accb + (size_t)slot * lda + col;
+            const float4 pr = ld4(ab), pz = ld4(ab + D), pn = ld4(ab + 2 * D), gn = ld4(gin + (size_t)slot * ldn + col);
+            const float4 hd = hp ? hdr[ps] : zero4();
+            float o_h[4], o_r[4], o_z[4], o_n[4], o_hn[4];
+            const float prv[4] = {pr.x, pr.y, pr.z, pr.w}, pzv[4] = {pz.x, pz.y, pz.z, pz.w}, pnv[4] = {pn.x, pn.y, pn.z, pn.w};
+            const float ivrv[4] = {ivr.x, ivr.y, ivr.z, ivr.w}, ivzv[4] = {ivz.x, ivz.y, ivz.z, ivz.w}, ivnv[4] = {ivn.x, ivn.y, ivn.z, ivn.w};
+            const float gnv[4] = {gn.x, gn.y, gn.z, gn.w}, hdv[4] = {hd.x, hd.y, hd.z, hd.w};
+            const float brv[4] = {br.x, br.y, br.z, br.w}, bzv[4] = {bz.x, bz.y, bz.z, bz.w}, bnv[4] = {bhn.x, bhn.y, bhn.z, bhn.w};
+            const float binv[4] = {bin.x, bin.y, bin.z, bin.w};
+#pragma unroll
+            for (int k = 0; k < 4; ++k) {
+              const float rg = gate_sigmoid(prv[k] * ivrv[k] + brv[k]);
+              const float zg = gate_sigmoid(pzv[k] * ivzv[k] + bzv[k]);
+              const float hn = pnv[k] * ivnv[k] + bnv[k];
+              const float ng = gate_tanh((gnv[k] * ivnv[k] + binv[k]) + rg * hn);
+              o_h[k] = (1.f - zg) * ng + zg * hdv[k];
+              o_r[k] = rg; o_z[k] = zg; o_n[k] = ng; o_hn[k] = hn;
+            }
+            h4 = make_float4(o_h[0], o_h[1], o_h[2], o_h[3]);
+            const size_t o = row * D + col;
+            if (!(a.dbg & 2)) {
+              if (flags & 2) st4(H + o, h4);
+              st4(saved + o, make_float4(o_r[0], o_r[1], o_r[2], o_r[3]));
+              st4(saved + plane + o, make_float4(o_z[0], o_z[1], o_z[2], o_z[3]));
+              st4(saved + 2 * plane + o, make_float4(o_n[0], o_n[1], o_n[2], o_n[3]));
+              st4(saved + 3 * plane + o, make_float4(o_hn[0], o_hn[1], o_hn[2], o_hn[3]));
+              st4(saved + 4 * plane + o, hd);
+            }
+          }
+          if (s + 1 < ns) {
+            hdr[ps] = hpn ? scale4(h4, decb[(s + 1) * CH_SLOTS + slot]) : zero4();
+            hx_u32x2 SH, SL;
+            hx_split4(hdr[ps], CHX_STATE_SCALE, SH, SL);
+            char* hdst = hpl + (size_t)slot * ldp + 2 * col;
+            *reinterpret_cast<hx_u32x2*>(hdst) = SH;
+            *reinterpret_cast<hx_u32x2*>(hdst + CH_SLOTS * ldp) = SL;
+          }
+        }
+        __syncthreads();
+      }
+    __syncthreads();
+  }
+  }
+}
+
 template <int VARIANT, int TPWB, int MW, int G4, int NMW = 4, int RING = 4>
 __global__ void __launch_bounds__(64 * (NMW + MW)) k_gru_chain_bwd_hx(ChainArgs a, ChainUps ups, const float* __restrict__ saved,
                                                                      float* __restrict__ dgi, float* __restrict__ dgh,
diff --git a/temp_amd/csrc/hx_pack.hpp b/temp_amd/csrc/hx_pack.hpp
--- a/temp_amd/csrc/hx_pack.hpp
+++ b/temp_amd/csrc/hx_pack.hpp
@@ -5,7 +5,7 @@
 namespace temp {
 
 #define HX_PACK_JOBS 8
-struct HxPackJob { const float* B; hx_u32x4* out; unsigned* keys; int K, N, n_tiles, n_slabs, ldb, trans, unit0, kblock0; };
+struct HxPackJob { const float* B; hx_u32x4* out; unsigned* keys; int K, N, n_tiles, n_slabs, ldb, trans, unit0, kblock0; const float* B2; hx_u32x4* out2; };
 struct HxPackJobs { HxPackJob j[HX_PACK_JOBS]; int count, total_units, total_kblocks; };
 
 inline size_t hx_packed_items(int N, int K) { return (size_t)ceil_div(K, 16) * ceil_div(N, 32) * 128; }
@@ -18,6 +18,11 @@
   jobs.total_kblocks += j.n_tiles;
 }
 
+inline void hx_pack_jobs_add_joint(HxPackJobs& jobs, const float* B, hx_u32x4* out, const float* B2, hx_u32x4* out2, unsigned* keys, int K, int N, int ldb, int trans) {
+  hx_pack_jobs_add(jobs, B, out, keys, K, N, ldb, trans);
+  jobs.j[jobs.count - 1].B2 = B2; jobs.j[jobs.count - 1].out2 = out2;
+}
+
 __device__ __forceinline__ const HxPackJob& hx_job_of(const HxPackJobs& jobs, int idx, bool by_kblock, int& local) {
   int ji = 0;
 #pragma unroll
@@ -33,9 +38,10 @@
   int t;
   const HxPackJob& jb = hx_job_of(jobs, blockIdx.x, true, t);
   const int K = jb.K, N = jb.N, ldb = jb.ldb;
-  const float* __restrict__ B = jb.B;
   unsigned key = 0;
   int c, g;
+  for (int m = 0; m < (jb.B2 ? 2 : 1); ++m) {
+  const float* __restrict__ B = m ? jb.B2 : jb.B;
   if (jb.trans) {
     c = threadIdx.x >> 5; g = threadIdx.x & 31;
     const int n = 32 * t + c;
@@ -67,6 +73,7 @@
       }
     }
   }
+  }
   sm[g][c] = key;
   __syncthreads();
   if (threadIdx.x < 32) {
@@ -80,6 +87,8 @@
   const int lane = threadIdx.x & 63, hh = lane >> 5, li = lane & 31, wave = threadIdx.x >> 6;
   const int n = 32 * t + li;
   const float sc = scale_l[li];
+  for (int m = 0; m < (jb.B2 ? 2 : 1); ++m) {
+  const float* __restrict__ B = m ? jb.B2 : jb.B;
   for (int s0 = wave; s0 < jb.n_slabs; s0 += 16) {
     const int k = 16 * s0 + 8 * hh;
     float4 v0 = zero4(), v1 = zero4();
@@ -98,8 +107,9 @@
     }
     hx_u32x4 H, L;
     hx_split8(v0, v1, sc, H, L);
-    hx_u32x4* d = jb.out + ((size_t)s0 * jb.n_tiles + t) * 128 + lane;
+    hx_u32x4* d = (m ? jb.out2 : jb.out) + ((size_t)s0 * jb.n_tiles + t) * 128 + lane;
     d[0] = H; d[64] = L;
+  }
   }
 }
 
diff --git a/temp_amd/gru_chain.py b/temp_amd/gru_chain.py
--- a/temp_amd/gru_chain.py
+++ b/temp_amd/gru_chain.py
@@ -9,6 +9,7 @@
 WEIGHT_GRADS_MULTI = True
 KEYED_GRADS = True
 GATE_GRADS_ONCE = True
+FUSED_INPUT_GATES = True
 
 
 class GruInstance:
@@ -213,6 +214,15 @@
         self._gi_shared = (str(device), res)
         return res
 
+    def x_index(self, device):
+        c = getattr(self, "_x_index", None)
+        if c is None or c[0] != str(device):
+            idx = np.zeros(self.n_total, dtype=np.int32)
+            for it in self.inst:
+                idx[it.h0:it.h0 + it.n] = it.x0 + np.arange(it.n, dtype=np.int32)
+            c = self._x_index = (str(device), _lib.to_device(idx, device))
+        return c[1]
+
     def constants(self, device, d):
         key = (str(device), int(d))
         c = getattr(self, "_const", None)
@@ -256,11 +266,15 @@
         tabs = None
         if CHAIN_KERNELS and hasattr(be, "gru_chain_fwd") and n_rnn <= _lib.CHAIN_MAX_RNN and be.gru_chain_supported(d):
             tabs = prog.chain_tables(dev, want)
-        share = prog.gi_shared(dev) if tabs is not None else None
+        fused = bool(tabs is not None and FUSED_INPUT_GATES and variant == _lib.GRU_TORCH and hasattr(be, "gru_chain_fwd_x")
+                     and be.gru_chain_fwd_x_supported(d, variant, tabs["max_steps"]))
+        share = prog.gi_shared(dev) if (tabs is not None and not fused) else None
         ctx.x_keys = x_keys if (x_keys is not None and tabs is not None) else None
         gk = (lambda: dict(x_keys=[ctx.x_keys[0][g["x0"]:g["x1"]] for g in prog.groups])) if ctx.x_keys is not None else dict
         gi_index = None
-        if share is not None:
+        if fused:
+            gi = None
+        elif share is not None:
             gi_index = share["gi_index"]
             gi = torch.empty(share["rows"], G, dtype=torch.float32, device=dev)
             cut = share["g0"] + [share["rows"]]
@@ -269,7 +283,7 @@
                                      x_idx=share["rep"], **gk())
         else:
             gi = torch.empty(N, G, dtype=torch.float32, device=dev)
-        if share is not None:
+        if share is not None or fused:
             pass
         elif len(prog.groups) > 1 and hasattr(be, "gru_input_gates_multi"):
             be.gru_input_gates_multi([x_all[g["x0"]:g["x1"]] for g in prog.groups], [W[g["rnn"]][0] for g in prog.groups],
@@ -281,7 +295,11 @@
         H = torch.empty(N, d, dtype=torch.float32, device=dev)
         saved = torch.empty(5, N, d, dtype=torch.float32, device=dev)
         packs = None
-        if tabs is not None:
+        if fused:
+            packs = be.gru_chain_pack_x_multi([W[r][1] for r in range(n_rnn)], [W[r][0] for r in range(n_rnn)])
+            be.gru_chain_fwd_x(tabs, x_all, prog.x_index(dev), lam, variant, packs, [W[r][3] for r in range(n_rnn)], [W[r][2] for r in range(n_rnn)],
+                               H, saved)
+        elif tabs is not None:
             packs = be.gru_chain_pack_multi([W[r][1] for r in range(n_rnn)]) if hasattr(be, "gru_chain_pack_multi") else \
                 [be.gru_chain_pack(W[r][1]) for r in range(n_rnn)]
             be.gru_chain_fwd(tabs, gi, lam, variant, packs, [W[r][3] for r in range(n_rnn)], H, saved, gi_index=gi_index)
@@ -415,6 +433,7 @@
     if chain_kernels_usable(d, n_rnn) and prog.chain_tables(device, tuple(want) if want is not None else None) is not None:
         _lib.pause_point()
         prog.gi_shared(device)
+        prog.x_index(device)
         return
     prog.upload(device)
 
```

Result: faster. 911.3 million, median of 6 (+4.1%).
